# lukifer23/Matrix0

Measured on AMD Instinct MI355X. Metric: self-play games/sec at 800 sims/move, ResNet-24 53M; 1/2/4/8 MI355X, higher is better.
Workload: dtype f16

## Files before the change

include/m0_engine.h:

```cpp
#ifndef M0_ENGINE_H
#define M0_ENGINE_H

#include <stddef.h>
#include <stdint.h>

#ifdef __cplusplus
extern "C" {
#endif

#define M0_OK 0
#define M0_ERR_INVALID (-1)
#define M0_ERR_UNSUPPORTED (-2)
#define M0_ERR_HIP (-3)
#define M0_ERR_STATE (-4)
#define M0_ERR_NONFINITE (-5)

#define M0_POLICY_SIZE 4672
#define M0_PLANES 19

#define M0_ACT_RELU 1
#define M0_ACT_SILU 2
#define M0_ACT_LEAKY 3

#define M0_SSL_PIECE 1
// ... 203 lines not shown
#define M0_DECODE_FULLMOVE_SATURATED 2
#define M0_DECODE_EP_FROM_MASK 4
#define M0_DECODE_NO_MASK 8
int m0_decode_planes(int hip_device, const float* planes, const uint8_t* mask, int n, int32_t* status, int32_t* flags,
                     int32_t* nlegal, char* fens, int fen_stride);
int m0_analysis_submit_planes(m0_selfplay* sp, const float* planes, const uint8_t* mask, int n, int sims, const int64_t* ids,
                              int32_t* status, int32_t* flags);
int m0_analysis_keep_visits(m0_selfplay* sp, int on);
int m0_analysis_poll_visits(m0_selfplay* sp, m0_analysis_result* out, int32_t* nchild, int32_t* policy_idx, int32_t* visits,
                            int cap);

typedef struct m0_tb m0_tb;
m0_tb* m0_tb_build(int hip_device, int max_men);
m0_tb* m0_tb_build_signatures(int hip_device, const char* const* sigs, int n);
m0_tb* m0_tb_load(const char* path);
int m0_tb_save(const m0_tb* tb, const char* path);
void m0_tb_destroy(m0_tb* tb);
int m0_tb_max_men(const m0_tb* tb);
int m0_tb_table(const m0_tb* tb, const char* sig, const uint8_t** bytes, size_t* n);
int m0_tb_table_info(const m0_tb* tb, int i, char* sig8, int* maxd, int* sweeps, double* build_ms);
int m0_tb_probe_fens(const m0_tb* tb, const char* const* fens, int n, uint8_t* hit, int8_t* wdl, int16_t* dtm);
int m0_selfplay_set_tablebase(m0_selfplay* sp, const m0_tb* tb, int max_pieces);
uint64_t m0_selfplay_tb_adjudications(m0_selfplay* sp);
int m0_selfplay_set_search_tablebase(m0_selfplay* sp, const m0_tb* tb, int max_pieces);
uint64_t m0_selfplay_tb_leaves(m0_selfplay* sp);
int m0_tb_root_lines(const m0_tb* tb, const char* fen, int multipv, int pv_len, m0_analysis_result* out);

int m0_sample_move_index(const int32_t* visits, int n, double temperature, double u);
int m0_playout_cap(int sims, double frac, double u);
double m0_temperature_for(int fullmove_number, double t_start, double t_end, int t_moves);
int m0_rules_probe(const m0_selfplay_cfg* cfg, const char* fen, const char* const* ucis, int n, int* flags, float* result);

int m0_san_pattern(const char* token, uint32_t* pattern);
#define M0_MOVE_UCI 0
#define M0_MOVE_RAW 1
int m0_move_pattern(int kind, const char* uci, uint32_t raw, uint32_t* pattern);
#define M0_REPLAY_OK 0
#define M0_REPLAY_ILLEGAL 1
#define M0_REPLAY_AMBIGUOUS 2
#define M0_REPLAY_TOO_LONG 3
#define M0_REPLAY_END_CHECKMATE 1
#define M0_REPLAY_END_STALEMATE 2
#define M0_REPLAY_END_INSUFFICIENT 4
#define M0_REPLAY_END_WHITE_TO_MOVE 8
int m0_replay_games(int hip_device, const char* const* start_fens, const uint32_t* patterns, const int32_t* offsets, int n_games,
                    int max_plies, int max_positions_per_launch, int32_t* plies, int32_t* status, int32_t* end_flags,
                    uint16_t* moves, int32_t* policy_idx, int32_t* nlegal, int8_t* turn, float* planes, uint8_t* mask, float* ssl);

#ifdef __cplusplus
}
#endif
#include "m0_analysis_live.h"
#include "m0_score.h"
#endif
```

matrix0_amd/_abi.py:

```python
from __future__ import annotations

import ctypes as C
from ctypes import POINTER as P

M0_OK = 0
M0_ERR_INVALID = -1
M0_ERR_UNSUPPORTED = -2
M0_ERR_HIP = -3
M0_ERR_STATE = -4
M0_ERR_NONFINITE = -5
POLICY_SIZE = 4672
ACT = {"relu": 1, "silu": 2, "leaky_relu": 3}
SSL_BITS = {"piece": 1, "threat": 2, "pin": 4, "fork": 8, "control": 16}
AN_MAX_LINES, AN_MAX_PV = 8, 16
DECODE_STATUS = {0: "ok", 1: "piece_value", 2: "square_clash", 3: "kings", 4: "pawn_rank", 5: "not_uniform", 6: "flag_value",
                 7: "castling", 8: "counter", 9: "opponent_in_check", 10: "too_many_moves", 11: "mask_mismatch"}
DECODE_OK, DECODE_MASK_MISMATCH = 0, 11
HALFMOVE_SATURATED, FULLMOVE_SATURATED, EP_FROM_MASK, NO_MASK = 1, 2, 4, 8
REPLAY_STATUS = {0: "ok", 1: "illegal", 2: "ambiguous", 3: "too_long"}
REPLAY_END_BITS = {"checkmate": 1, "stalemate": 2, "insufficient": 4, "white_to_move": 8}
MOVE_UCI, MOVE_RAW = 0, 1
SCORE_MASK = {"legal": 0, "target": 1, "none": 2}
SCORE_COLS = 8
SCORE_COLUMNS = ("policy_loss", "entropy", "value_loss", "rank", "support_mass", "support_size", "value", "flags")
# ... 139 lines not shown
    "m0_search_advance": (i32, [vp, i32, i32, i32, i32]),
    "m0_analysis_create": (vp, [vp, _cfg, P(AnalysisOpts)]),
    "m0_analysis_create_ext": (vp, [_cfg, P(AnalysisOpts)]),
    "m0_analysis_submit": (i32, [vp, cstr, cstrs, i32, i32, i64]),
    "m0_analysis_step": (i32, [vp, i32]),
    "m0_analysis_ext_select": _select,
    "m0_analysis_ext_expand": _expand,
    "m0_analysis_poll": (i32, [vp, _res]),
    "m0_analysis_pending": (i32, [vp]),
    "m0_analysis_result_size": (C.c_size_t, []),
    "m0_decode_planes": (i32, [i32, vp, vp, i32, vp, vp, vp, cstr, i32]),
    "m0_analysis_submit_planes": (i32, [vp, vp, vp, i32, i32, vp, vp, vp]),
    "m0_analysis_keep_visits": (i32, [vp, i32]),
    "m0_analysis_poll_visits": (i32, [vp, _res, _pi32, vp, vp, i32]),
    "m0_tb_build": (vp, [i32, i32]),
    "m0_tb_build_signatures": (vp, [i32, cstrs, i32]),
    "m0_tb_load": (vp, [cstr]),
    "m0_tb_save": (i32, [vp, cstr]),
    "m0_tb_destroy": (None, [vp]),
    "m0_tb_max_men": (i32, [vp]),
    "m0_tb_table": (i32, [vp, cstr, P(P(u8)), P(C.c_size_t)]),
    "m0_tb_table_info": (i32, [vp, i32, cstr, _pi32, _pi32, P(f64)]),
    "m0_tb_probe_fens": (i32, [vp, cstrs, i32, vp, vp, vp]),
    "m0_selfplay_set_tablebase": _attach,
    "m0_selfplay_tb_adjudications": (u64, [vp]),
    "m0_selfplay_set_search_tablebase": _attach,
    "m0_selfplay_tb_leaves": (u64, [vp]),
    "m0_tb_root_lines": (i32, [vp, cstr, i32, i32, _res]),
    "m0_sample_move_index": (i32, [vp, i32, f64, f64]),
    "m0_playout_cap": (i32, [i32, f64, f64]),
    "m0_temperature_for": (f64, [i32, f64, f64, i32]),
    "m0_rules_probe": (i32, [_cfg, cstr, cstrs, i32, _pi32, P(f32)]),
    "m0_san_pattern": (i32, [cstr, P(u32)]),
    "m0_move_pattern": (i32, [i32, cstr, u32, P(u32)]),
    "m0_replay_games": (i32, [i32, cstrs, vp, vp, i32, i32, i32] + [vp] * 10),
}

LIVE_FUNCTIONS = {
    "m0_analysis_submit_keep": (i32, [vp, cstr, cstrs, i32, i32, i64]),
    "m0_analysis_peek": (i32, [vp, i64, _res]),
    "m0_analysis_stop": (i32, [vp, i64]),
    "m0_analysis_continue": (i32, [vp, i64, cstrs, i32, i32, i64, i32, _pi32]),
    "m0_analysis_release": (i32, [vp, i64]),
    "m0_analysis_held": (i32, [vp]),
}

SCORE_STRUCTS = {"m0_score_opts": ScoreOpts}
SCORE_FUNCTIONS = {
    "m0_score_rows": (i32, [i32, vp, vp, vp, vp, vp, i32, P(ScoreOpts), vp]),
    "m0_net_score": (i32, [vp, vp, vp, vp, vp, i32, P(ScoreOpts), vp]),
    "m0_score_bench": (i32, [i32, i32, i32, P(f32), P(f64)]),
}


def bind(L) -> list:
    missing = []
    for name, (restype, argtypes) in list(FUNCTIONS.items()) + list(LIVE_FUNCTIONS.items()) + list(SCORE_FUNCTIONS.items()):
        fn = getattr(L, name, None)
        if fn is None:
            missing.append(name)
        else:
            fn.restype, fn.argtypes = restype, argtypes
    return missing
```

matrix0_amd/backend.py:

```python
from __future__ import annotations

import ctypes as C
import threading
from typing import Dict, Optional, Tuple

import numpy as np

from . import _abi, _lib


def resolve_mask_mode(pi: np.ndarray, legal_mask, mask_mode: Optional[str]) -> str:
    if mask_mode is not None:
        if mask_mode not in _abi.SCORE_MASK:
            raise ValueError(f"mask_mode must be one of {sorted(_abi.SCORE_MASK)} or None, got {mask_mode!r}")
        return mask_mode
    if legal_mask is not None:
        return "legal"
    return "none" if bool(((np.asarray(pi) > 0).sum(axis=1) == 1).all()) else "target"


class NonFiniteScore(ValueError):

    def __init__(self, msg: str, rows: np.ndarray):
        super().__init__(msg)
        self.rows = rows


def score_opts(mask_mode: str, label_smoothing: float, value_loss: str, huber_delta: float) -> "_abi.ScoreOpts":
    if value_loss not in ("mse", "huber"):
        raise ValueError(f"value_loss must be 'mse' or 'huber', got {value_loss!r}")
    return _abi.ScoreOpts(_abi.SCORE_MASK[mask_mode], float(label_smoothing), int(value_loss == "huber"), float(huber_delta))


class M0Backend:
    def __init__(self, model_cfg: dict, device_index: int = 0):
        self._L = _lib.lib()
        self.model_cfg = dict(model_cfg)
        self._cfg = _lib.net_cfg_from_dict(model_cfg)
        self._h = self._L.m0_net_create(C.byref(self._cfg), int(device_index))
        if not self._h:
            raise RuntimeError(f"m0_net_create failed: {_lib.last_error()}")
        self._finalized = False
        self.ssl_tasks = [t for t in _lib.SSL_ORDER if self._cfg.ssl_tasks & _lib.SSL_BITS[t]] \
            if self._cfg.self_supervised else []

    def load_state_dict(self, sd: Dict[str, "np.ndarray"]) -> None:
        for k, v in sd.items():
            if hasattr(v, "detach"):
                v = v.detach().cpu().float().numpy()
            a = np.ascontiguousarray(np.asarray(v), dtype=np.float32)
            shape = (C.c_int64 * max(1, a.ndim))(*a.shape)
            _lib.check(self._L.m0_net_load_weight(self._h, k.encode(), _lib.ptr(a), 0, shape, a.ndim),
                       f"m0_net_load_weight({k})")
        _lib.check(self._L.m0_net_finalize(self._h), "m0_net_finalize")
        self._finalized = True

    @classmethod
    def from_state_dict(cls, model_cfg: dict, sd, device_index: int = 0) -> "M0Backend":
        b = cls(model_cfg, device_index)
        b.load_state_dict(sd)
        return b

    @classmethod
    def from_checkpoint(cls, model_cfg: dict, ckpt_path: str, device_index: int = 0) -> "M0Backend":
        import torch
        state = torch.load(ckpt_path, map_location="cpu", weights_only=False)
        sd = state
        if isinstance(state, dict):
            for key in ("model_ema", "model", "model_state_dict"):
                if key in state and isinstance(state[key], dict):
                    sd = state[key]
                    break
        return cls.from_state_dict(model_cfg, sd, device_index)

    def infer_np(self, arr: np.ndarray) -> Tuple[np.ndarray, np.ndarray]:
        p, v, _ = self._infer(arr, False)
        return p, v

    def infer_np_ssl(self, arr: np.ndarray):
        return self._infer(arr, True)

    def tap_info(self) -> Tuple[int, int]:
        steps, width = C.c_int(0), C.c_int(0)
        _lib.check(self._L.m0_net_tap_info(self._h, C.byref(steps), C.byref(width)), "m0_net_tap_info")
        return steps.value, width.value

    def infer_tap(self, arr: np.ndarray, step: int):
        return self._infer(arr, True, int(step))

    def _infer(self, arr: np.ndarray, want_ssl: bool, tap_step: Optional[int] = None):
        if not self._finalized:
            raise RuntimeError("weights not loaded")
        a = np.asarray(arr)
        if a.ndim == 3:
            a = a[None]
        if a.ndim != 4 or a.shape[1:] != (self._cfg.planes, 8, 8):
            raise ValueError(f"expected input [B,{self._cfg.planes},8,8], got {a.shape}")
        a = np.ascontiguousarray(a, dtype=np.float32)
        B = a.shape[0]
        pol = np.empty((B, _lib.POLICY_SIZE), dtype=np.float32)
        val = np.empty((B,), dtype=np.float32)
        sslc = self._L.m0_net_ssl_channels(self._h)
        ssl = np.empty((B, sslc, 8, 8), dtype=np.float32) if (want_ssl and sslc > 0) else None
        if tap_step is None:
            _lib.check(self._L.m0_net_infer(self._h, _lib.ptr(a), B, _lib.ptr(pol), _lib.ptr(val), _lib.ptr(ssl)), "m0_net_infer")
        else:
            width = self.tap_info()[1]
            stream = np.empty((B, 64, width), dtype=np.float32)
            second = np.empty((B, 64, width), dtype=np.float32)
            has_second = C.c_int(0)
            _lib.check(self._L.m0_net_infer_tap(self._h, _lib.ptr(a), B, tap_step, _lib.ptr(pol), _lib.ptr(val), _lib.ptr(ssl),
                                                _lib.ptr(stream), _lib.ptr(second), C.byref(has_second)), "m0_net_infer_tap")
        out = None
        if ssl is not None:
            out, off = {}, 0
            for t in self.ssl_tasks:
                n = _lib.SSL_CH[t]
                out[t] = ssl[:, off:off + n]
                off += n
        if tap_step is not None:
            return pol, val, out, stream, (second if has_second.value else None)
        return pol, val, out

    def score(self, s: np.ndarray, pi: np.ndarray, z: np.ndarray, legal_mask: Optional[np.ndarray] = None, *,
              mask_mode: Optional[str] = None, label_smoothing: float = 0.0, value_loss: str = "mse",
              huber_delta: float = 1.0) -> np.ndarray:
        if not self._finalized:
            raise RuntimeError("weights not loaded")
        a = np.ascontiguousarray(s, dtype=np.float32)
        if a.ndim != 4 or a.shape[1:] != (self._cfg.planes, 8, 8):
            raise ValueError(f"expected input [B,{self._cfg.planes},8,8], got {a.shape}")
        B = a.shape[0]
        pi = np.ascontiguousarray(pi, dtype=np.float32)
        z = np.ascontiguousarray(np.asarray(z).reshape(-1), dtype=np.float32)
        if pi.shape != (B, _lib.POLICY_SIZE) or z.shape != (B,):
            raise ValueError(f"expected pi [{B},{_lib.POLICY_SIZE}] and z [{B}], got {pi.shape} and {z.shape}")
        if legal_mask is not None:
            legal_mask = np.ascontiguousarray(np.asarray(legal_mask).reshape(B, -1), dtype=np.uint8)
            if legal_mask.shape != pi.shape:
                raise ValueError(f"expected legal_mask [{B},{_lib.POLICY_SIZE}], got {legal_mask.shape}")
        opts = score_opts(resolve_mask_mode(pi, legal_mask, mask_mode), label_smoothing, value_loss, huber_delta)
        rows = np.empty((B, _abi.SCORE_COLS), dtype=np.float32)
        rc = self._L.m0_net_score(self._h, _lib.ptr(a), _lib.ptr(pi), _lib.ptr(z), _lib.ptr(legal_mask), B, C.byref(opts),
                                  _lib.ptr(rows))
        if rc == _lib.M0_ERR_NONFINITE:
            raise NonFiniteScore(f"m0_net_score failed ({rc}): {_lib.last_error()}", rows)
        _lib.check(rc, "m0_net_score")
        return rows

    def param_count(self) -> int:
        return int(self._L.m0_net_param_count(self._h))

# ... 35 lines not shown
```

matrix0_amd/csrc/capi_analysis.hip:

```cpp
#include <string.h>
#include <algorithm>
#include <string>
#include <memory>
#include "selfplay_engine.h"
#include "planes_decode.h"
#include "tb.h"

using namespace m0;

namespace m0 {

static int searches_pending(const m0_selfplay* sp) {
    int n = (int)sp->an->queue.size();
    for (int s = 0; s < sp->G; ++s) n += sp->games[s].in_use && !sp->an->held[s] ? 1 : 0;
    return n;
}
static int pending_count(const m0_selfplay* sp) { return searches_pending(sp) + (int)sp->an->policy_queue.size(); }

static m0_analysis_result blank_result(const AnalysisJob& job) {
    m0_analysis_result r;
    memset(&r, 0, sizeof(r));
    r.id = job.id; r.nlegal = job.nlegal; r.sims = job.sims;
    return r;
}
// ... 54 lines not shown
    a.finished.clear();
    for (int s = 0; s < sp->G; ++s)
        if (sp->hg[s].active && sp->hg[s].finished) a.finished.push_back(s);
    const int nf = (int)a.finished.size();
    if (nf == 0) return M0_OK;
    HipStatus& hs = sp->hip;
    M0_HIP(hs, hipMemcpyAsync(sp->ids_dev, a.finished.data(), (size_t)nf * 4, hipMemcpyHostToDevice, sp->stream));
    M0_HIP(hs, launch_analysis_lines(sp->d, sp->ids_dev, nf, a.opts.multipv, a.opts.pv_len, a.lines_dev, a.nlines_dev, sp->stream));
    M0_HIP(hs, hipMemcpyAsync(a.hlines.data(), a.lines_dev, sizeof(m0_analysis_line) * M0_AN_MAX_LINES * nf, hipMemcpyDeviceToHost, sp->stream));
    M0_HIP(hs, hipMemcpyAsync(a.hnlines.data(), a.nlines_dev, (size_t)nf * 4, hipMemcpyDeviceToHost, sp->stream));
    if (a.keep_visits) {
        M0_HIP(hs, launch_root_children(sp->d, sp->ids_dev, nf, a.child_idx_dev, a.child_n_dev, a.nchild_dev, sp->stream));
        M0_HIP(hs, hipMemcpyAsync(a.hchild_idx.data(), a.child_idx_dev, (size_t)nf * M0_MAX_CHILDREN * 4, hipMemcpyDeviceToHost, sp->stream));
        M0_HIP(hs, hipMemcpyAsync(a.hchild_n.data(), a.child_n_dev, (size_t)nf * M0_MAX_CHILDREN * 4, hipMemcpyDeviceToHost, sp->stream));
        M0_HIP(hs, hipMemcpyAsync(a.hnchild.data(), a.nchild_dev, (size_t)nf * 4, hipMemcpyDeviceToHost, sp->stream));
    }
    if (!M0_HIP(hs, hipStreamSynchronize(sp->stream))) return m0_hip_error(hs, "analysis harvest failed");
    for (int j = 0; j < nf; ++j) {
        const int s = a.finished[j];
        GameDev& g = sp->hg[s];
        m0_analysis_result r = blank_result(a.slot_job[s]);
        r.overflow = g.overflow; r.root_n = g.root_n; r.evals = g.evals;
        r.value = (float)g.root_v;
        r.root_q = g.root_n > 0 ? g.root_q : g.root_v;
        copy_lines(a, j, r);
        if (g.overflow) sp->stats.arena_overflows++;
        std::vector<int32_t> children;
        if (a.keep_visits) {
            const int k = a.hnchild[j] < 0 ? 0 : (a.hnchild[j] > M0_MAX_CHILDREN ? M0_MAX_CHILDREN : a.hnchild[j]);
            const int32_t* ci = a.hchild_idx.data() + (size_t)j * M0_MAX_CHILDREN;
            const int32_t* cn = a.hchild_n.data() + (size_t)j * M0_MAX_CHILDREN;
            children.assign(ci, ci + k);
            children.insert(children.end(), cn, cn + k);
        }
        answer(a, r, std::move(children));
        g.active = 0; g.finished = 0;
        leave_slot(sp, s);
    }
    return sync_games_h2d(sp) ? M0_OK : m0_hip_error(hs, "releasing the slots failed");
}

static int policy_pass(m0_selfplay* sp) {
    Analysis& a = *sp->an;
    const int n = (int)std::min<size_t>(a.policy_queue.size(), (size_t)sp->rows_max);
    if (n <= 0) return M0_OK;
    const double t0 = now_ms();
    for (int i = 0; i < n; ++i) a.hpos[i] = a.policy_queue[i].line.pos;
    HipStatus& hs = sp->hip;
    M0_HIP(hs, hipMemcpyAsync(a.pos_dev, a.hpos.data(), sizeof(Pos) * n, hipMemcpyHostToDevice, sp->stream));
    if (!M0_HIP(hs, launch_encode_positions(a.pos_dev, n, nullptr, sp->d.x0, nullptr, a.nlegal_dev, a.moves_dev, a.idx_dev, sp->stream)))
        return m0_hip_error(hs, "position encode failed");
    std::string err;
    m0_net_lock(sp->nethandle);
    const int rc = sp->net->forward(nullptr, sp->d.x0, n, sp->logits_dev, sp->values_dev, nullptr, sp->stream, err);
    m0_net_unlock(sp->nethandle);
    if (rc != M0_OK) { hs.check(sp->net->hip()); m0_set_error(err); return rc; }
    M0_HIP(hs, launch_policy_lines(sp->logits_dev, sp->values_dev, a.nlegal_dev, a.moves_dev, a.idx_dev, n, a.opts.multipv, a.lines_dev,
                                   a.nlines_dev, a.value_out_dev, sp->stream));
    M0_HIP(hs, hipMemcpyAsync(a.hlines.data(), a.lines_dev, sizeof(m0_analysis_line) * M0_AN_MAX_LINES * n, hipMemcpyDeviceToHost, sp->stream));
    M0_HIP(hs, hipMemcpyAsync(a.hnlines.data(), a.nlines_dev, (size_t)n * 4, hipMemcpyDeviceToHost, sp->stream));
    M0_HIP(hs, hipMemcpyAsync(a.hvalues.data(), a.value_out_dev, (size_t)n * 4, hipMemcpyDeviceToHost, sp->stream));
    if (!M0_HIP(hs, hipStreamSynchronize(sp->stream))) return m0_hip_error(hs, "policy pass failed");
    for (int i = 0; i < n; ++i) {
        m0_analysis_result r = blank_result(a.policy_queue.front());
        r.evals = 1;
        r.value = a.hvalues[i];
        r.root_q = (double)r.value;
        copy_lines(a, i, r);
        answer(a, r);
        a.policy_queue.pop_front();
    }
    sp->stats.evals += (uint64_t)n;
    sp->stats.ms_total += now_ms() - t0;
    return M0_OK;
}

static bool blocked_by_held(const m0_selfplay* sp) {
    if (sp->an->queue.empty()) return false;
    for (int s = 0; s < sp->G; ++s) if (!sp->games[s].in_use || !sp->an->held[s]) return false;
    m0_set_error("searches are queued but every slot is held: m0_analysis_release or m0_analysis_continue one");
    return true;
}

static bool live_call_ok(const m0_selfplay* sp, const char* what) {
    if (!sp->ext_pending) return true;
    m0_set_error(std::string(what) + ": m0_analysis_ext_expand outstanding");
    return false;
}
static int slot_of(const m0_selfplay* sp, int64_t id, bool held) {
    for (int s = 0; s < sp->G; ++s)
        if (sp->games[s].in_use && (sp->an->held[s] != 0) == held && sp->an->slot_job[s].id == id) return s;
    return -1;
}
template <typename Q> static typename Q::iterator queued(Q& q, int64_t id) {
    return std::find_if(q.begin(), q.end(), [id](const AnalysisJob& j) { return j.id == id; });
}

static int live_result(m0_selfplay* sp, int s, m0_analysis_result& r) {
    Analysis& a = *sp->an;
    HipStatus& hs = sp->hip;
    M0_HIP(hs, hipMemcpyAsync(sp->ids_dev, &s, 4, hipMemcpyHostToDevice, sp->stream));
    M0_HIP(hs, launch_analysis_lines(sp->d, sp->ids_dev, 1, a.opts.multipv, a.opts.pv_len, a.lines_dev, a.nlines_dev, sp->stream));
    M0_HIP(hs, hipMemcpyAsync(a.hlines.data(), a.lines_dev, sizeof(m0_analysis_line) * M0_AN_MAX_LINES, hipMemcpyDeviceToHost, sp->stream));
    M0_HIP(hs, hipMemcpyAsync(a.hnlines.data(), a.nlines_dev, 4, hipMemcpyDeviceToHost, sp->stream));
    if (!sync_games_d2h(sp)) return m0_hip_error(hs, "reading a running search failed");
    const GameDev& g = sp->hg[s];
    r = blank_result(a.slot_job[s]);
// ... 309 lines not shown
```

matrix0_amd/csrc/capi_net.hip:

```cpp
#include <hip/hip_runtime.h>
#include <math.h>
#include <string.h>
#include <mutex>
#include <string>
#include <vector>
#include "../../include/m0_engine.h"
#include "net.h"
#include "capi_common.h"
#include "score_core.h"
#include "score_kernels.h"

thread_local std::string g_m0_last_error;

void m0_set_error(const std::string& s) { g_m0_last_error = s; }

struct m0_net {
    Net* net = nullptr;
    int device = 0;
    hipStream_t stream = nullptr;
    std::mutex mu;
    float* planes_dev = nullptr;
    float* logits_dev = nullptr;
    float* value_dev = nullptr;
    float* ssl_dev = nullptr;
    int cap = 0;
    float* score_pi_dev = nullptr;
    float* score_z_dev = nullptr;
    uint8_t* score_mask_dev = nullptr;
    float* score_rows_dev = nullptr;
    int score_cap = 0;
};

Net* m0_net_impl(m0_net* n) { return n ? n->net : nullptr; }
hipStream_t m0_net_stream(m0_net* n) { return n ? n->stream : nullptr; }
int m0_net_device(m0_net* n) { return n ? n->device : 0; }
void m0_net_lock(m0_net* n) { if (n) n->mu.lock(); }
void m0_net_unlock(m0_net* n) { if (n) n->mu.unlock(); }

hipError_t create_stream_cu_mask_env(const char* env_name, hipStream_t* stream) {
    const char* mk = getenv(env_name);
    if (!mk || !*mk) return hipStreamCreateWithFlags(stream, hipStreamNonBlocking);
    uint32_t words[8] = {0, 0, 0, 0, 0, 0, 0, 0};
    int nw = 0;
    for (const char* q = mk; *q && nw < 8; ++nw) {
        char* end = nullptr;
        words[nw] = (uint32_t)strtoul(q, &end, 16);
        if (end == q) break;
        q = (*end == ',') ? end + 1 : end;
    }
    return hipExtStreamCreateWithCUMask(stream, 8, words);
}

extern "C" {

const char* m0_last_error(void) { return g_m0_last_error.c_str(); }
const char* m0_version(void) { return "m0engine 0.2 (gfx950)"; }
int m0_device_count(void) {
    int n = 0;
    if (hipGetDeviceCount(&n) != hipSuccess) { (void)hipGetLastError(); return 0; }
    return n;
}

m0_net* m0_net_create(const m0_net_cfg* cfg, int hip_device) {
    if (!cfg) { m0_set_error("cfg is null"); return nullptr; }
    const char* why = Net::check_supported(*cfg);
    if (why) { m0_set_error(std::string("unsupported network config: ") + why); return nullptr; }
    int ndev = 0;
    if (hipGetDeviceCount(&ndev) != hipSuccess || ndev <= 0) {
        m0_set_error("no HIP device available (the engine has no CPU fallback)");
        return nullptr;
    }
    if (hip_device < 0 || hip_device >= ndev) { m0_set_error("hip_device out of range"); return nullptr; }
    if (hipSetDevice(hip_device) != hipSuccess) { m0_set_error("hipSetDevice failed"); return nullptr; }
    m0_net* h = new m0_net();
    h->device = hip_device;
    const hipError_t se = create_stream_cu_mask_env("M0_NET_CU_MASK", &h->stream);
    if (se != hipSuccess) {
        m0_set_error("hipStreamCreate failed");
        delete h;
        return nullptr;
    }
    h->net = new Net(*cfg, hip_device, h->stream);
    return h;
}

void m0_net_destroy(m0_net* n) {
    if (!n) return;
    (void)hipSetDevice(n->device);
    if (n->stream) { (void)hipStreamSynchronize(n->stream); }
    if (n->planes_dev) (void)hipFree(n->planes_dev);
    if (n->logits_dev) (void)hipFree(n->logits_dev);
    if (n->value_dev) (void)hipFree(n->value_dev);
    if (n->ssl_dev) (void)hipFree(n->ssl_dev);
    if (n->score_pi_dev) (void)hipFree(n->score_pi_dev);
    if (n->score_z_dev) (void)hipFree(n->score_z_dev);
    if (n->score_mask_dev) (void)hipFree(n->score_mask_dev);
    if (n->score_rows_dev) (void)hipFree(n->score_rows_dev);
    delete n->net;
    if (n->stream) (void)hipStreamDestroy(n->stream);
    delete n;
}

int m0_net_load_weight(m0_net* n, const char* name, const void* data, int dtype, const int64_t* shape, int ndim) {
    if (!n) { m0_set_error("net is null"); return M0_ERR_INVALID; }
    std::lock_guard<std::mutex> lk(n->mu);
    std::string err;
    int rc = n->net->load(name, data, dtype, shape, ndim, err);
    if (rc != M0_OK) m0_set_error(err);
    return rc;
}

int m0_net_finalize(m0_net* n) {
    if (!n) { m0_set_error("net is null"); return M0_ERR_INVALID; }
    std::lock_guard<std::mutex> lk(n->mu);
    if (!n->net->hip().ok()) return m0_hip_error(n->net->hip());
    std::string err;
    int rc = n->net->finalize(err);
    if (rc != M0_OK) m0_set_error(err);
    return rc;
}

static int ensure_io(m0_net* n, int B) {
    if (B <= n->cap) return M0_OK;
    HipStatus& hs = n->net->hip();
    for (float** p : {&n->planes_dev, &n->logits_dev, &n->value_dev, &n->ssl_dev}) {
        if (*p) M0_HIP(hs, hipFree(*p));
        *p = nullptr;
    }
    n->cap = 0;
    int cap = B < 64 ? 64 : B;
    const int P = n->net->cfg().planes;
    int sslc = n->net->ssl_channels_total();
    M0_HIP(hs, hipMalloc((void**)&n->planes_dev, (size_t)cap * P * 64 * 4));
    M0_HIP(hs, hipMalloc((void**)&n->logits_dev, (size_t)cap * M0_POLICY_SIZE * 4));
    M0_HIP(hs, hipMalloc((void**)&n->value_dev, (size_t)cap * 4));
    M0_HIP(hs, hipMalloc((void**)&n->ssl_dev, (size_t)cap * (sslc > 0 ? sslc : 1) * 64 * 4));
    if (!hs.ok()) return m0_hip_error(hs, "hipMalloc failed for I/O staging");
    n->cap = cap;
    return M0_OK;
}

static int ensure_score_io(m0_net* n, int B) {
    if (B <= n->score_cap) return M0_OK;
    HipStatus& hs = n->net->hip();
    if (n->score_pi_dev) M0_HIP(hs, hipFree(n->score_pi_dev));
    if (n->score_z_dev) M0_HIP(hs, hipFree(n->score_z_dev));
    if (n->score_mask_dev) M0_HIP(hs, hipFree(n->score_mask_dev));
    if (n->score_rows_dev) M0_HIP(hs, hipFree(n->score_rows_dev));
    n->score_pi_dev = n->score_z_dev = n->score_rows_dev = nullptr;
    n->score_mask_dev = nullptr;
    n->score_cap = 0;
    const int cap = B < 64 ? 64 : B;
    M0_HIP(hs, hipMalloc((void**)&n->score_pi_dev, (size_t)cap * M0_POLICY_SIZE * 4));
    M0_HIP(hs, hipMalloc((void**)&n->score_z_dev, (size_t)cap * 4));
    M0_HIP(hs, hipMalloc((void**)&n->score_mask_dev, (size_t)cap * M0_POLICY_SIZE));
    M0_HIP(hs, hipMalloc((void**)&n->score_rows_dev, (size_t)cap * M0_SCORE_COLS * 4));
    if (!hs.ok()) return m0_hip_error(hs, "hipMalloc failed for score staging");
    n->score_cap = cap;
    return M0_OK;
}

static int infer_locked(m0_net* n, const float* planes, int B, float* policy, float* value, float* ssl,
                        float* tap_stream = nullptr, float* tap_second = nullptr, int* has_second = nullptr) {
    HipStatus& hs = n->net->hip();
    if (!M0_HIP(hs, hipSetDevice(n->device))) return m0_hip_error(hs);
    int rc = ensure_io(n, B);
    if (rc != M0_OK) return rc;
    const int P = n->net->cfg().planes;
    const int sslc = n->net->ssl_channels_total();
    if (ssl && sslc == 0) { m0_set_error("ssl output requested but the net has no SSL heads"); return M0_ERR_INVALID; }
    std::string err;
    if (!M0_HIP(hs, hipMemcpyAsync(n->planes_dev, planes, (size_t)B * P * 64 * 4, hipMemcpyHostToDevice, n->stream)))
        return m0_hip_error(hs, "H2D copy");
    rc = n->net->forward(n->planes_dev, nullptr, B, n->logits_dev, n->value_dev, ssl ? n->ssl_dev : nullptr, n->stream, err);
    if (rc != M0_OK) { m0_set_error(err); return rc; }
    M0_HIP(hs, hipMemcpyAsync(policy, n->logits_dev, (size_t)B * M0_POLICY_SIZE * 4, hipMemcpyDeviceToHost, n->stream));
    M0_HIP(hs, hipMemcpyAsync(value, n->value_dev, (size_t)B * 4, hipMemcpyDeviceToHost, n->stream));
    if (ssl) M0_HIP(hs, hipMemcpyAsync(ssl, n->ssl_dev, (size_t)B * sslc * 64 * 4, hipMemcpyDeviceToHost, n->stream));
    std::vector<_Float16> th, ta;
    const size_t tn = tap_stream ? (size_t)B * 64 * n->net->trunk_width() : 0;
    if (tap_stream) {
        th.resize(tn);
        M0_HIP(hs, hipMemcpyAsync(th.data(), n->net->tap_stream(), tn * 2, hipMemcpyDeviceToHost, n->stream));
        if (n->net->tap_has_second()) {
            ta.resize(tn);
            M0_HIP(hs, hipMemcpyAsync(ta.data(), n->net->tap_second(), tn * 2, hipMemcpyDeviceToHost, n->stream));
        }
    }
    if (!M0_HIP(hs, hipStreamSynchronize(n->stream))) return m0_hip_error(hs, "forward failed");
    if (tap_stream) {
        for (size_t i = 0; i < tn; ++i) tap_stream[i] = (float)th[i];
        for (size_t i = 0; i < tn; ++i) tap_second[i] = ta.empty() ? 0.f : (float)ta[i];
        *has_second = ta.empty() ? 0 : 1;
    }
    for (size_t i = 0, nn = (size_t)B * M0_POLICY_SIZE; i < nn; ++i)
        if (!isfinite(policy[i])) { m0_set_error("network produced non-finite policy logits"); return M0_ERR_NONFINITE; }
    for (int i = 0; i < B; ++i)
        if (!isfinite(value[i])) { m0_set_error("network produced non-finite value"); return M0_ERR_NONFINITE; }
    return M0_OK;
}

int m0_net_infer(m0_net* n, const float* planes, int B, float* policy, float* value, float* ssl) {
    if (!n || !planes || !policy || !value) { m0_set_error("null argument"); return M0_ERR_INVALID; }
    if (B <= 0) { m0_set_error("batch must be positive"); return M0_ERR_INVALID; }
    std::lock_guard<std::mutex> lk(n->mu);
    return infer_locked(n, planes, B, policy, value, ssl);
}

int m0_net_score(m0_net* n, const float* planes, const float* pi, const float* z, const uint8_t* legal_mask, int B,
                 const m0_score_opts* opts, float* rows) {
    if (!n || !planes || !pi || !z || !rows) { m0_set_error("null argument"); return M0_ERR_INVALID; }
    if (B <= 0) { m0_set_error("batch must be positive"); return M0_ERR_INVALID; }
    if (const char* why = m0score::bad_opts(opts, legal_mask != nullptr)) { m0_set_error(why); return M0_ERR_INVALID; }
    std::lock_guard<std::mutex> lk(n->mu);
    HipStatus& hs = n->net->hip();
    if (!M0_HIP(hs, hipSetDevice(n->device))) return m0_hip_error(hs);
    int rc = ensure_io(n, B);
    if (rc == M0_OK) rc = ensure_score_io(n, B);
    if (rc != M0_OK) return rc;
    const bool masked = opts->mask_mode == M0_SCORE_MASK_LEGAL;
    const size_t cells = (size_t)B * M0_POLICY_SIZE;
    M0_HIP(hs, hipMemcpyAsync(n->planes_dev, planes, (size_t)B * n->net->cfg().planes * 64 * 4, hipMemcpyHostToDevice, n->stream));
    M0_HIP(hs, hipMemcpyAsync(n->score_pi_dev, pi, cells * 4, hipMemcpyHostToDevice, n->stream));
    M0_HIP(hs, hipMemcpyAsync(n->score_z_dev, z, (size_t)B * 4, hipMemcpyHostToDevice, n->stream));
    if (masked) M0_HIP(hs, hipMemcpyAsync(n->score_mask_dev, legal_mask, cells, hipMemcpyHostToDevice, n->stream));
    if (!hs.ok()) return m0_hip_error(hs, "H2D copy");
    std::string err;
    rc = n->net->forward(n->planes_dev, nullptr, B, n->logits_dev, n->value_dev, nullptr, n->stream, err);
    if (rc != M0_OK) { m0_set_error(err); return rc; }
    M0_HIP(hs, launch_score_rows(n->logits_dev, n->value_dev, n->score_pi_dev, n->score_z_dev, masked ? n->score_mask_dev : nullptr,
                                 B, *opts, n->score_rows_dev, n->stream));
    M0_HIP(hs, hipMemcpyAsync(rows, n->score_rows_dev, (size_t)B * M0_SCORE_COLS * 4, hipMemcpyDeviceToHost, n->stream));
    if (!M0_HIP(hs, hipStreamSynchronize(n->stream))) return m0_hip_error(hs, "forward and score failed");
    for (int b = 0; b < B; ++b)
        if ((int)rows[(size_t)b * M0_SCORE_COLS + 7] & M0_SCORE_FLAG_NONFINITE) {
            m0_set_error("network produced non-finite outputs (row " + std::to_string(b) + ")");
            return M0_ERR_NONFINITE;
        }
    return M0_OK;
}

int m0_net_tap_info(const m0_net* n, int* steps, int* width) {
    if (!n || !steps || !width) { m0_set_error("null argument"); return M0_ERR_INVALID; }
    *steps = n->net->tap_steps();
    *width = n->net->trunk_width();
    return M0_OK;
}

int m0_net_infer_tap(m0_net* n, const float* planes, int B, int step, float* policy, float* value, float* ssl, float* stream,
                     float* second, int* has_second) {
    if (!n || !planes || !policy || !value || !stream || !second || !has_second) {
        m0_set_error("null argument");
        return M0_ERR_INVALID;
    }
    if (B <= 0) { m0_set_error("batch must be positive"); return M0_ERR_INVALID; }
    if (step < 0 || step >= n->net->tap_steps()) { m0_set_error("tap step out of range"); return M0_ERR_INVALID; }
    std::lock_guard<std::mutex> lk(n->mu);
    n->net->set_tap(step);
    const int rc = infer_locked(n, planes, B, policy, value, ssl, stream, second, has_second);
    n->net->set_tap(-1);
    return rc;
}

int m0_net_ssl_channels(const m0_net* n) { return n ? n->net->ssl_channels_total() : 0; }
int64_t m0_net_param_count(const m0_net* n) { return n ? (int64_t)n->net->param_count() : 0; }
double m0_net_flops_per_position(const m0_net* n, int with_ssl) { return n ? n->net->flops_per_position(with_ssl != 0) : 0.0; }

int m0_net_profile_enable(m0_net* n, int on) {
    if (!n) { m0_set_error("net is null"); return M0_ERR_INVALID; }
    std::lock_guard<std::mutex> lk(n->mu);
    n->net->set_profile(on != 0);
    return M0_OK;
}

int m0_net_profile_get(m0_net* n, double* conv_ms, double* conv_flop, int64_t* launches, int reset) {
    if (!n) { m0_set_error("net is null"); return M0_ERR_INVALID; }
    std::lock_guard<std::mutex> lk(n->mu);
    if (conv_ms) *conv_ms = n->net->prof_conv_ms();
    if (conv_flop) *conv_flop = n->net->prof_conv_flop();
    if (launches) *launches = n->net->prof_conv_launches();
    if (reset) n->net->reset_profile();
    return M0_OK;
}

int m0_net_profile_get_tail(m0_net* n, double* tail_ms, int64_t* tail_launches) {
    if (!n) { m0_set_error("net is null"); return M0_ERR_INVALID; }
    std::lock_guard<std::mutex> lk(n->mu);
    if (tail_ms) *tail_ms = n->net->prof_tail_ms();
    if (tail_launches) *tail_launches = n->net->prof_tail_launches();
    return M0_OK;
}

int m0_net_bench_forward(m0_net* n, int B, int iters, int with_ssl, float* ms_per_forward) {
    if (!n || !ms_per_forward || B <= 0 || iters <= 0) { m0_set_error("invalid argument"); return M0_ERR_INVALID; }
    std::lock_guard<std::mutex> lk(n->mu);
    HipStatus& hs = n->net->hip();
    if (!M0_HIP(hs, hipSetDevice(n->device))) return m0_hip_error(hs);
    int rc = ensure_io(n, B);
    if (rc != M0_OK) return rc;
    std::string err;
    if (!(with_ssl & 2)) {
        const int P = n->net->cfg().planes;
        std::vector<float> h((size_t)B * P * 64, 0.f);
        uint64_t s = 0x9E3779B97F4A7C15ull;
        for (size_t i = 0; i < h.size(); ++i) {
            s ^= s << 13; s ^= s >> 7; s ^= s << 17;
            int p = (int)((i / 64) % P);
            if (p < 12) h[i] = ((s >> 20) % 100) < 8 ? 1.f : 0.f;
            else h[i] = (float)((((i / 64 / P) * 7 + p) % 10) / 10.0);
        }
        if (!M0_HIP(hs, hipMemcpy(n->planes_dev, h.data(), h.size() * 4, hipMemcpyHostToDevice))) return m0_hip_error(hs, "H2D copy");
    }
    float* ssl = ((with_ssl & 1) && n->net->ssl_channels_total() > 0) ? n->ssl_dev : nullptr;
    rc = n->net->forward(n->planes_dev, nullptr, B, n->logits_dev, n->value_dev, ssl, n->stream, err);
    if (rc != M0_OK) { m0_set_error(err); return rc; }
    struct Events {
        hipEvent_t e0 = nullptr, e1 = nullptr;
        ~Events() { if (e0) (void)hipEventDestroy(e0); if (e1) (void)hipEventDestroy(e1); }
    } ev;
    M0_HIP(hs, hipEventCreate(&ev.e0)); M0_HIP(hs, hipEventCreate(&ev.e1));
    M0_HIP(hs, hipEventRecord(ev.e0, n->stream));
    for (int i = 0; i < iters && hs.ok(); ++i) {
        rc = n->net->forward(n->planes_dev, nullptr, B, n->logits_dev, n->value_dev, ssl, n->stream, err);
        if (rc != M0_OK) { m0_set_error(err); return rc; }
    }
    M0_HIP(hs, hipEventRecord(ev.e1, n->stream));
    M0_HIP(hs, hipEventSynchronize(ev.e1));
    float ms = 0.f;
    if (!M0_HIP(hs, hipEventElapsedTime(&ms, ev.e0, ev.e1))) return m0_hip_error(hs, "bench forward failed");
    *ms_per_forward = ms / iters;
    n->net->harvest_profile();
    return M0_OK;
}

}
```

matrix0_amd/csrc/capi_selfplay.hip:

```cpp
#include <string.h>
#include <algorithm>
#include <memory>
#include "selfplay_engine.h"

using namespace m0;

static void fill_tree_cfg(const m0_selfplay_cfg& c, bool match, TreeCfg& t) {
    t.fpu_reduction = c.fpu_reduction; t.draw_penalty = c.draw_penalty; t.virtual_loss = c.virtual_loss;
    t.selection_jitter = c.selection_jitter; t.cpuct = c.cpuct; t.cpuct_start = c.cpuct_start; t.cpuct_end = c.cpuct_end;
    t.cpuct_plies = c.cpuct_plies; t.use_c_base = c.use_c_base; t.cpuct_c_base = c.cpuct_c_base; t.cpuct_c_init = c.cpuct_c_init;
    t.dirichlet_alpha = c.dirichlet_alpha; t.dirichlet_frac = c.dirichlet_frac; t.legal_softmax = c.legal_softmax;
    t.enable_entropy_noise = c.enable_entropy_noise; t.no_instant_backtrack = c.no_instant_backtrack;
    t.virtual_loss_active = c.virtual_loss_active; t.leaves_per_step = c.inference_batch_size;
    t.tt_merge = c.tt_merge; t.raw_legal_priors = c.raw_legal_priors; t.max_children = c.max_children;
    t.min_child_prior = c.min_child_prior;
    t.eval_cache = ((match ? c.arena_eval_cache : c.eval_cache) && c.legal_softmax && !c.raw_legal_priors && !c.tt_merge) ? 1 : 0;
}

static bool alloc_tree_arenas(m0_selfplay* sp) {
    const m0_selfplay_cfg& c = sp->cfg;
    long want = c.arena_nodes > 0 ? c.arena_nodes : (long)(c.num_simulations * 1.3 + 64) * 96;
    if (want < 4096) want = 4096;
    sp->cap = (int)want;
    const size_t N = (size_t)sp->G * 2 * sp->cap;
    TreeArrays& t = sp->d.t;
    t.cap = sp->cap;
    t.prior = dalloc<double>(sp, N); t.w = dalloc<double>(sp, N); t.q = dalloc<double>(sp, N);
    t.n = dalloc<int>(sp, N); t.vl = dalloc<int>(sp, N); t.cbase = dalloc<int>(sp, N);
    t.nch = dalloc<int16_t>(sp, N); t.mv = dalloc<uint16_t>(sp, N); t.midx = dalloc<uint16_t>(sp, N);
    sp->d.games = dalloc<GameDev>(sp, sp->G);
    const size_t LS = (size_t)sp->L + 1;
    sp->d.samples = dalloc<Sample>(sp, (size_t)sp->G * LS);
    sp->d.paths = dalloc<int>(sp, (size_t)sp->G * LS * M0_MAX_DEPTH);
    sp->d.leaf_moves = dalloc<uint16_t>(sp, (size_t)sp->G * LS * M0_MAX_CHILDREN);
    return hip_ok(sp, "hipMalloc failed for the search arenas (lower concurrent_games or arena_nodes)");
}

static bool alloc_position_tables(m0_selfplay* sp) {
    sp->d.tt_sides = 1;
    if (!sp->cfg.tt_merge) return true;
    const size_t LS = (size_t)sp->L + 1;
    int tc = 1024;
    while (tc < 2 * sp->cap) tc <<= 1;
    sp->d.tt_cap = tc;
    sp->d.tt_sides = sp->kind == EngineKind::Match ? 2 : 1;
    sp->d.search_nodes = (int)std::min<long>((long)sp->cfg.num_simulations * 48 + 4 * M0_MAX_CHILDREN, (long)sp->cap / 2);
    sp->d.epaths = dalloc<int>(sp, (size_t)sp->G * LS * M0_MAX_DEPTH);
    sp->d.tt_keys = dalloc<uint64_t>(sp, (size_t)sp->G * sp->d.tt_sides * tc);
    sp->d.tt_nodes = dalloc<int>(sp, (size_t)sp->G * sp->d.tt_sides * tc);
    return hip_ok(sp, "hipMalloc failed for the position tables (tt_merge): lower concurrent_games or arena_nodes");
}

static bool alloc_eval_cache(m0_selfplay* sp) {
    if (!sp->tc.eval_cache) return true;
    const size_t LS = (size_t)sp->L + 1;
    int entries = sp->cfg.eval_cache_entries > 0 ? sp->cfg.eval_cache_entries : 16384;
    int sets = 64;
    while (sets * 4 < entries) sets <<= 1;
    EvalCache& ec = sp->d.ec;
    ec.sets = sets;
    ec.sides = sp->kind == EngineKind::Match ? 2 : 1;
    const size_t entries_all = (size_t)sp->G * ec.sides * sets * 4;
    ec.keys = dalloc<uint64_t>(sp, entries_all);
    ec.stamps = dalloc<uint32_t>(sp, entries_all);
    ec.payload = dalloc<float>(sp, entries_all * M0_EC_WORDS);
    ec.hit_stage = dalloc<float>(sp, (size_t)sp->G * LS * M0_EC_WORDS);
    return hip_ok(sp, "hipMalloc failed for the evaluation cache: lower eval_cache_entries or concurrent_games");
}

static bool alloc_batch_buffers(m0_selfplay* sp) {
    const int nreg = sp->kind == EngineKind::Match ? 2 : 1;
    sp->d.hist = dalloc<uint64_t>(sp, (size_t)sp->G * M0_HIST_CAP);
    sp->d.results = dalloc<RootResult>(sp, sp->G);
    sp->d.row_counter = dalloc<int>(sp, 4);
    sp->d.x0 = dalloc<_Float16>(sp, (size_t)(nreg * sp->rows_max + 4) * 64 * 32);
    sp->logits_dev = dalloc<float>(sp, (size_t)nreg * sp->rows_max * 4672);
    sp->values_dev = dalloc<float>(sp, (size_t)nreg * sp->rows_max + 4);
    sp->d.net_row_base = sp->rows_max;
    if (sp->cfg.ssl_in_forward && sp->net && sp->net->ssl_channels_total() > 0)
        sp->ssl_dev = dalloc<float>(sp, (size_t)sp->rows_max * sp->net->ssl_channels_total() * 64);
    if (sp->cfg.ssl_targets) {
        sp->ssl_cap = sp->cfg.max_game_len > 0 ? sp->cfg.max_game_len + 1 : 513;
        sp->ssl_pos_dev = dalloc<Pos>(sp, sp->ssl_cap);
        sp->ssl_out_dev = dalloc<float>(sp, (size_t)sp->ssl_cap * 17 * 64);
        if (!hip_ok(sp, "hipMalloc failed for the SSL target staging buffers")) return false;
    }
    sp->ids_dev = dalloc<int>(sp, sp->G);
    sp->roots_dev = dalloc<int>(sp, sp->G);
    sp->d.logits = sp->logits_dev; sp->d.values = sp->values_dev;
    sp->d.G = sp->G; sp->d.L = sp->L;
    return hip_ok(sp, "hipMalloc failed for the batch buffers (lower concurrent_games or inference_batch_size)");
}

static bool make_tail_view(m0_selfplay* sp) {
    if (!(sp->cfg.tail_split && sp->net && sp->kind != EngineKind::Match && sp->net->cfg().channels > 256 && sp->net->cfg().channels <= 320 &&
          sp->rows_max >= 2048)) return true;
    M0_HIP(sp->hip, create_stream_cu_mask_env("M0_TAIL_CU_MASK", &sp->stream_tail));
    M0_HIP(sp->hip, hipEventCreateWithFlags(&sp->ev_sel, hipEventDisableTiming));
    M0_HIP(sp->hip, hipEventCreateWithFlags(&sp->ev_tail, hipEventDisableTiming));
    if (!hip_ok(sp, "hipStreamCreate / hipEventCreate failed (tail split)")) return false;
    sp->net_tail = sp->net->shared_view(sp->stream_tail);
    std::string werr;
    sp->half_split = sp->cfg.tail_split == 2;
    if (sp->net_tail->ensure_workspace(sp->half_split ? sp->rows_max / 2 + 1024 : 1023, werr) != M0_OK) {
        m0_set_error("tail split: " + werr);
        return false;
    }
    return true;
}

static bool build_engine(m0_selfplay* sp) {
    if (!alloc_tree_arenas(sp) || !alloc_position_tables(sp) || !alloc_eval_cache(sp) || !alloc_batch_buffers(sp)) return false;
    sp->hg.assign(sp->G, GameDev());
    for (auto& g : sp->hg) memset(&g, 0, sizeof(GameDev));
    sp->games.assign(sp->G, HostGame());
    sp->hres.resize(sp->G);
    sp->hsamples.resize((size_t)sp->G * (sp->L + 1));
    sp->prev_done.assign(sp->G, 0);
    for (hipEvent_t* e : {&sp->ev0, &sp->ev1, &sp->ev2, &sp->ev3}) M0_HIP(sp->hip, hipEventCreate(e));
    if (!hip_ok(sp, "hipEventCreate failed") || !make_tail_view(sp)) return false;
    std::string err;
    if (sp->net && sp->net->ensure_workspace(sp->rows_max, err) != M0_OK) { m0_set_error(err); return false; }
    if (sp->net && sp->net_b && sp->net_b->ensure_workspace(sp->rows_max, err) != M0_OK) { m0_set_error(err); return false; }
    M0_HIP(sp->hip, hipStreamSynchronize(sp->stream));
    return hip_ok(sp, "clearing the search arenas failed");
}

m0_selfplay* m0::engine_create(m0_net* nh, m0_net* nh_b, const m0_selfplay_cfg* cfg, EngineKind kind) {
    if (!cfg) { m0_set_error("cfg is null"); return nullptr; }
    if (cfg->concurrent_games <= 0 || cfg->inference_batch_size <= 0 || cfg->num_simulations <= 0) {
// ... 31 lines not shown
static int leaf_planes(m0_selfplay* sp, int rows_a, float* planes_a, int rows_b, float* planes_b) {
    sync_games_d2h(sp);
    if (!M0_HIP(sp->hip, hipMemcpy(sp->hsamples.data(), sp->d.samples, sizeof(Sample) * (size_t)sp->G * (sp->L + 1), hipMemcpyDeviceToHost)))
        return m0_hip_error(sp->hip, "device sync failed");
    const int base = sp->d.net_row_base;
    for (int g = 0; g < sp->G; ++g) {
        if (!sp->hg[g].active) continue;
        for (int s = 0; s < sp->hg[g].nsamples; ++s) {
            const Sample& smp = sp->hsamples[(size_t)g * (sp->L + 1) + s];
            if (!sample_owns_row(smp.kind) || smp.row < 0) continue;
            if (smp.row < rows_a) encode_planes_f32(smp.pos, planes_a + (size_t)smp.row * 19 * 64);
            else if (smp.row >= base && smp.row < base + rows_b) encode_planes_f32(smp.pos, planes_b + (size_t)(smp.row - base) * 19 * 64);
        }
    }
    return M0_OK;
}

static void upload_eval(m0_selfplay* sp, size_t row_base, const float* logits, const float* values, int rows) {
    if (rows <= 0) return;
    M0_HIP(sp->hip, hipMemcpyAsync(sp->logits_dev + row_base * 4672, logits, (size_t)rows * 4672 * 4, hipMemcpyHostToDevice, sp->stream));
    M0_HIP(sp->hip, hipMemcpyAsync(sp->values_dev + row_base, values, (size_t)rows * 4, hipMemcpyHostToDevice, sp->stream));
}

int m0::ext_select_impl(m0_selfplay* sp, int* rows_a, int* rows_b, float* planes_a, float* planes_b, int max_rows) {
    if (sp->ext_pending) { m0_set_error("m0_selfplay_ext_expand outstanding"); return M0_ERR_STATE; }
    if (!planes_a || (sp->kind == EngineKind::Match && !planes_b) || max_rows < sp->G * (sp->L + 1)) {
        m0_set_error("planes buffer too small: concurrent_games * (inference_batch_size + 1) rows are required");
        return M0_ERR_INVALID;
    }
    int rc = refill(sp);
    if (rc != M0_OK) return rc;
    int r = 0;
    if ((rc = run_select(sp, &r)) != M0_OK) return rc;
    const int rb = sp->kind == EngineKind::Match ? sp->rows2[1] : 0;
    if (r > sp->rows_max || rb > sp->rows_max) { m0_set_error("row counter overflow"); return M0_ERR_STATE; }
    *rows_a = r;
    if (rows_b) *rows_b = rb;
    sp->last_rows = r;
    sp->last_rows_b = rb;
    sp->ext_pending = true;
    if (r + rb > 0) return leaf_planes(sp, r, planes_a, rb, planes_b);
    return M0_OK;
}

int m0::ext_expand_impl(m0_selfplay* sp, const float* logits_a, const float* values_a, int rows_a, const float* logits_b,
                           const float* values_b, int rows_b) {
    if (!sp->ext_pending) { m0_set_error("no m0_selfplay_ext_select outstanding"); return M0_ERR_STATE; }
    if (rows_a != sp->last_rows || rows_b != sp->last_rows_b) { m0_set_error("rows does not match the last select"); return M0_ERR_INVALID; }
    if ((rows_a > 0 && (!logits_a || !values_a)) || (rows_b > 0 && (!logits_b || !values_b))) { m0_set_error("null argument"); return M0_ERR_INVALID; }
    upload_eval(sp, 0, logits_a, values_a, rows_a);
    upload_eval(sp, (size_t)sp->d.net_row_base, logits_b, values_b, rows_b);
    sp->ext_pending = false;
    M0_HIP(sp->hip, hipEventRecord(sp->ev0, sp->stream)); M0_HIP(sp->hip, hipEventRecord(sp->ev1, sp->stream));
    return finish_step(sp, rows_a + rows_b, now_ms());
}

bool m0::kind_accepted(const m0_selfplay* sp, const char* what, unsigned kinds) {
    if (kinds & (1u << (int)sp->kind)) return true;
    static const char* const is_a[] = {"a self-play engine", "a match engine", "an analysis engine"};
    const char* only = kinds == KIND_SELFPLAY ? "self-play engines" : kinds == KIND_MATCH ? "match engines"
                     : kinds == KIND_ANALYSIS ? "analysis engines" : "self-play and match engines";
    m0_set_error(std::string(what) + ": " + only + " only, this is " + is_a[(int)sp->kind]);
    return false;
}

extern "C" {

m0_selfplay* m0_selfplay_create(m0_net* nh, const m0_selfplay_cfg* cfg) { return engine_create(nh, nullptr, cfg, EngineKind::SelfPlay); }

m0_selfplay* m0_arena_create(m0_net* net_a, m0_net* net_b, const m0_selfplay_cfg* cfg) {
    if (!net_a || !net_b) { m0_set_error("m0_arena_create needs two networks"); return nullptr; }
    if (m0_net_device(net_a) != m0_net_device(net_b)) { m0_set_error("both networks must live on the same HIP device"); return nullptr; }
    if (cfg && (cfg->ssl_in_forward || cfg->ssl_targets)) { m0_set_error("arena games carry no SSL outputs"); return nullptr; }
    return engine_create(net_a, net_b, cfg, EngineKind::Match);
}

m0_selfplay* m0_arena_create_ext(const m0_selfplay_cfg* cfg) {
    if (cfg && (cfg->ssl_in_forward || cfg->ssl_targets)) { m0_set_error("arena games carry no SSL outputs"); return nullptr; }
    return engine_create(nullptr, nullptr, cfg, EngineKind::Match);
}

void m0_selfplay_destroy(m0_selfplay* sp) {
    if (!sp) return;
    forward_gate_leave(sp);
    (void)hipSetDevice(sp->device);
    if (sp->stream) (void)hipStreamSynchronize(sp->stream);
    if (sp->stream_tail) (void)hipStreamSynchronize(sp->stream_tail);
    delete sp->net_tail;
    if (sp->ev_sel) (void)hipEventDestroy(sp->ev_sel);
    if (sp->ev_tail) (void)hipEventDestroy(sp->ev_tail);
    if (sp->stream_tail) (void)hipStreamDestroy(sp->stream_tail);
    for (void* p : sp->allocs) (void)hipFree(p);
    for (auto& r : sp->done_meta) delete (GameRecordOwner*)r.owner;
    delete sp->an;
    if (sp->ev0) { (void)hipEventDestroy(sp->ev0); (void)hipEventDestroy(sp->ev1); (void)hipEventDestroy(sp->ev2); (void)hipEventDestroy(sp->ev3); }
    if (sp->own_stream && sp->stream) (void)hipStreamDestroy(sp->stream);
    delete sp;
}

int m0_selfplay_set_openings(m0_selfplay* sp, const char* const* fens, int n) {
    if (!sp || n < 0 || (n > 0 && !fens)) { m0_set_error("invalid argument"); return M0_ERR_INVALID; }
    M0_ENGINE_CALL(sp, "m0_selfplay_set_openings", KIND_GAMES, false);
    if (sp->stats.games_started != 0) { m0_set_error("set the opening book before the first step"); return M0_ERR_STATE; }
    std::vector<Pos> book(n);
    for (int i = 0; i < n; ++i)
        if (!fens[i] || parse_fen(fens[i], book[i]) != 0) { m0_set_error(std::string("bad FEN at index ") + std::to_string(i)); return M0_ERR_INVALID; }
    sp->book.swap(book);
// ... 154 lines not shown
```

matrix0_amd/csrc/conv_epilogue.h:

```cpp
#pragma once
#include "kernel_common.h"

typedef _Float16 half2v __attribute__((ext_vector_type(2)));

template <int ACT>
__device__ __forceinline__ float act_fast(float v) {
    if constexpr (ACT == ACT_RELU) return v > 0.f ? v : 0.f;
    else if constexpr (ACT == ACT_SILU) return v * __builtin_amdgcn_rcpf(1.f + __expf(-v));
    else if constexpr (ACT == ACT_LEAKY) return v > 0.f ? v : 0.05f * v;
    else if constexpr (ACT == ACT_SIGMOID) return __builtin_amdgcn_rcpf(1.f + __expf(-v));
    else if constexpr (ACT == ACT_TANH) return tanhf(v);
    else return v;
}
template <int NT>
__device__ __forceinline__ char* conv_stage_base(char* lds_wave, int lane) {
    return lds_wave + (4 * (lane >> 5) + (lane & 1)) * (NT * 64) + ((lane & 31) >> 1) * 4;
}

template <int NT, int MI, int NI>
__device__ __forceinline__ void conv_stage_tile(const float (&v)[16], char* wbase, int lane) {
    constexpr int ROWB = NT * 64;
    const bool odd = (lane & 1) != 0;
    static_for<0, 8>([&](auto rp_) __attribute__((always_inline)) {
        constexpr int r0 = 2 * decltype(rp_)::value;
// ... 2 lines not shown
        const float recv = __builtin_bit_cast(
            float, __builtin_amdgcn_update_dpp(0, __builtin_bit_cast(int, send), 0xB1, 0xF, 0xF, true));
        const half2v h = {(_Float16)(odd ? recv : v0), (_Float16)(odd ? v1 : recv)};
        *reinterpret_cast<half2v*>(wbase + (MI * 32 + (r0 & 3) + 8 * (r0 >> 2)) * ROWB + NI * 64) = h;
    });
}

template <int NT, int FENCE_EVERY = 0>
__device__ __forceinline__ void conv_stage_flush(const GemmArgs& a, const char* lds_wave, int m0, int n0, int wm, int wn,
                                                 int lane) {
    constexpr int NCH = NT * 4;
    const uint32_t ldo2 = (uint32_t)a.ldo * 2u;
    char* out = reinterpret_cast<char*>(a.out) + ((size_t)(m0 + wm * 64) * a.ldo + n0 + wn * NT * 32) * 2;
    const int rows_valid = a.Mvalid - (m0 + wm * 64);
    int row = lane / NCH, ch = lane - row * NCH;
#pragma unroll
    for (int it = 0; it < NCH; ++it) {
        if (FENCE_EVERY > 0 && it % (FENCE_EVERY > 0 ? FENCE_EVERY : 1) == 0) asm volatile("" ::: "memory");
        const uint4 v = *reinterpret_cast<const uint4*>(lds_wave + (it * 64 + lane) * 16);
        if (row < rows_valid) *reinterpret_cast<uint4*>(out + ((uint32_t)row * ldo2 + (uint32_t)ch * 16u)) = v;
        ch += 64 % NCH; row += 64 / NCH;
        if (ch >= NCH) { ch -= NCH; row += 1; }
    }
}

__device__ __forceinline__ void gn16_mean_rstd(float s, float ss, float& mean, float& rstd) {
    mean = s * (1.f / 1024.f);
    float var = ss * (1.f / 1024.f) - mean * mean;
    var = var > 0.f ? var : 0.f;
    rstd = rsqrtf(var + 1e-5f);
}
__device__ __forceinline__ void gn16_affine(float mean, float rstd, const float& gamma, const float& beta, float& scale,
                                            float& shift) {
    scale = gamma * rstd;
    shift = beta - mean * scale;
}

template <int NI, int NT>
__device__ __forceinline__ void conv_gn_column(const float16v (&acc)[2][NT], const float* gamma, const float* beta, int col,
                                               float& scale, float& shift) {
    float s = 0.f, ss = 0.f;
    static_for<0, 2>([&](auto mi_) __attribute__((always_inline)) {
        const float16v av = acc[decltype(mi_)::value][NI];
        static_for<0, 16>([&](auto r_) __attribute__((always_inline)) { const float v = av[decltype(r_)::value]; s += v; ss += v * v; });
    });
#pragma unroll
    for (int o = 1; o <= 8; o <<= 1) { s += __shfl_xor(s, o); ss += __shfl_xor(ss, o); }
    s += __shfl_xor(s, 32); ss += __shfl_xor(ss, 32);
    float mean, rstd;
    gn16_mean_rstd(s, ss, mean, rstd);
    gn16_affine(mean, rstd, gamma[col], beta[col], scale, shift);
}

template <ConvEpi EPI, int ACT, int NT>
__device__ __forceinline__ void conv_tile_epilogue(float16v (&acc)[2][NT], const GemmArgs& a, char* lds_wave, int m0,
                                                   int n0, int wm, int wn, int lane, int out_col0 = 0) {
    const int half = lane >> 5;
    const int r31 = lane & 31;
    const int colbase = n0 + wn * NT * 32 + r31;
    char* wbase = conv_stage_base<NT>(lds_wave, lane);
    if constexpr (EPI == EPI_GN) {
        static_for<0, NT>([&](auto ni_) __attribute__((always_inline)) {
            constexpr int ni = decltype(ni_)::value;
            const int col = colbase + ni * 32;
            float g, sh;
            conv_gn_column<ni>(acc, a.gn_gamma, a.gn_beta, col, g, sh);
            static_for<0, 2>([&](auto mi_) __attribute__((always_inline)) {
                constexpr int mi = decltype(mi_)::value;
                float v[16];
                static_for<0, 16>([&](auto r_) __attribute__((always_inline)) {
                    constexpr int r = decltype(r_)::value;
                    v[r] = act_fast<ACT>(acc[mi][ni][r] * g + sh);
                });
                if (a.posenc != nullptr) {
                    static_for<0, 16>([&](auto r_) __attribute__((always_inline)) {
                        constexpr int r = decltype(r_)::value;
                        const int sq = mi * 32 + (r & 3) + 8 * (r >> 2) + 4 * half;
                        v[r] += a.posenc[(size_t)sq * a.N + col];
                    });
                }
                conv_stage_tile<NT, mi, ni>(v, wbase, lane);
            });
        });
        conv_stage_flush<NT>(a, lds_wave, m0, n0 - out_col0, wm, wn, lane);
    }
    if constexpr (EPI == EPI_PLAIN) {
        const float oscale = a.out_scale;
        const bool want_stats = a.out_stats != nullptr;
        float* stats = a.out_stats + ((size_t)(m0 / 64 + wm) * a.N + colbase) * 2;
        static_for<0, NT>([&](auto ni_) __attribute__((always_inline)) {
            constexpr int ni = decltype(ni_)::value;
            const float bias = a.bias != nullptr ? a.bias[colbase + ni * 32] : 0.f;
            float s = 0.f, ss = 0.f;
            static_for<0, 2>([&](auto mi_) __attribute__((always_inline)) {
                constexpr int mi = decltype(mi_)::value;
                float v[16];
                static_for<0, 16>([&](auto r_) __attribute__((always_inline)) {
                    constexpr int r = decltype(r_)::value;
                    v[r] = act_fast<ACT>(acc[mi][ni][r] + bias) * oscale;
                    s += v[r]; ss += v[r] * v[r];
                });
                conv_stage_tile<NT, mi, ni>(v, wbase, lane);
            });
            if (want_stats) {
                s += __shfl_xor(s, 32);
                ss += __shfl_xor(ss, 32);
                if (lane < 32) { stats[ni * 64] = s; stats[ni * 64 + 1] = ss; }
            }
        });
        conv_stage_flush<NT>(a, lds_wave, m0, n0, wm, wn, lane);
    }
    if constexpr (EPI == EPI_ELEMENT) {
        const int ldo = a.ldo;
        const int rowbase = m0 + wm * 64 + 4 * half;
        const int epi_act = a.epi_act;
        const float oscale = a.out_scale;
        const bool want_stats = a.out_stats != nullptr;
        const bool has_mul = a.mul != nullptr;
        const bool f32out = a.out_f32 != 0;
        static_for<0, NT>([&](auto ni_) __attribute__((always_inline)) {
            constexpr int ni = decltype(ni_)::value;
            const int col = colbase + ni * 32;
            const float bias = a.bias != nullptr ? a.bias[col] : 0.f;
            float s = 0.f, ss = 0.f;
            static_for<0, 2>([&](auto mi_) __attribute__((always_inline)) {
                constexpr int mi = decltype(mi_)::value;
                const float16v av = acc[mi][ni];
                static_for<0, 16>([&](auto r_) __attribute__((always_inline)) {
                    constexpr int r = decltype(r_)::value;
                    const int row = rowbase + mi * 32 + (r & 3) + 8 * (r >> 2);
                    float v = av[r] + bias;
                    if (epi_act != ACT_NONE) v = act_apply(v, epi_act);
                    if (has_mul) v *= (float)a.mul[(size_t)row * ldo + col];
                    v *= oscale;
                    s += v; ss += v * v;
                    if (row < a.Mvalid) {
                        if (f32out) reinterpret_cast<float*>(a.out)[(size_t)row * ldo + col] = v;
                        else reinterpret_cast<_Float16*>(a.out)[(size_t)row * ldo + col] = (_Float16)v;
                    }
                });
            });
            if (want_stats) {
                s += __shfl_xor(s, 32);
                ss += __shfl_xor(ss, 32);
                if (lane < 32) {
                    float* st = a.out_stats + ((size_t)(m0 / 64 + wm) * a.N + col) * 2;
                    st[0] = s; st[1] = ss;
                }
            }
        });
    }
}
```

matrix0_amd/csrc/conv_gemm.hip:

```cpp
#include "kernel_common.h"
#include "conv_epilogue.h"

template <int TAPS, int WN, int NT, int KC, ConvEpi EPI = EPI_ELEMENT, int ACT = ACT_NONE>
__global__ __launch_bounds__(256 * WN) void conv_gemm_kernel(GemmArgs a) {
    constexpr int NB = WN * NT * 32;
    constexpr int NTHR = 256 * WN;
    constexpr int AST = KC + 8;
    constexpr int APIX = (TAPS == 9) ? 100 : 64;
    constexpr int A_ELEMS = 4 * APIX * AST;
    constexpr int W_ELEMS = NB * AST;
    constexpr int A_PIECES = 4 * 64 * KC / 8;
    constexpr int W_PIECES = NB * KC / 8;
    constexpr int A_PER = (A_PIECES + NTHR - 1) / NTHR;
    constexpr int W_PER = (W_PIECES + NTHR - 1) / NTHR;
    constexpr int K8 = KC / 8;

    extern __shared__ __attribute__((aligned(16))) char smem[];
    _Float16* A_lds = reinterpret_cast<_Float16*>(smem);
    _Float16* W_lds = A_lds + A_ELEMS;

    const int tid = threadIdx.x;
    const int lane = tid & 63;
    const int wave = tid >> 6;
    const int wm = wave % 4;
    const int wn = wave / 4;
    const int m0 = blockIdx.x * 256;
    const int n0 = blockIdx.y * NB;
    const int Cin = a.Cin;
    const int nchunk = Cin / KC;
    const int Npad = a.Npad;

    if (TAPS == 9) {
        for (int i = tid; i < A_ELEMS / 8; i += NTHR)
            reinterpret_cast<uint4*>(A_lds)[i] = make_uint4(0, 0, 0, 0);
    }
    __syncthreads();

    float16v acc[2][NT];
    static_for<0, 2>([&](auto mi) __attribute__((always_inline)) {
        static_for<0, NT>([&](auto ni) __attribute__((always_inline)) {
            acc[decltype(mi)::value][decltype(ni)::value] = float16v{0.f, 0.f, 0.f, 0.f, 0.f, 0.f, 0.f, 0.f,
                                                                      0.f, 0.f, 0.f, 0.f, 0.f, 0.f, 0.f, 0.f};
        });
    });

    int apix[2];
#pragma unroll
    for (int mi = 0; mi < 2; ++mi) {
        int px = mi * 32 + (lane & 31);
        if (TAPS == 9) apix[mi] = wm * 100 + ((px >> 3) + 1) * 10 + (px & 7) + 1;
        else apix[mi] = wm * 64 + px;
    }
    const int khalf = 8 * (lane >> 5);

    uint4 areg[A_PER];
    uint4 wreg[W_PER];
// ... 29 lines not shown
            int p = tid + i * NTHR;
            if (W_PIECES % NTHR == 0 || p < W_PIECES)
                wreg[i] = *reinterpret_cast<const uint4*>(src + (size_t)p * 8);
        }
    };
    auto store_W = [&](int buf) {
#pragma unroll
        for (int i = 0; i < W_PER; ++i) {
            int p = tid + i * NTHR;
            if (W_PIECES % NTHR == 0 || p < W_PIECES) {
                int n = p / K8, k8 = p % K8;
                *reinterpret_cast<uint4*>(W_lds + buf * W_ELEMS + n * AST + k8 * 8) = wreg[i];
            }
        }
    };

    const int nsteps = nchunk * TAPS;
    load_A(0);
    load_W(0);
    for (int s = 0; s < nsteps; ++s) {
        const int chunk = s / TAPS, tap = s % TAPS;
        if (tap == 0) {
            if (s > 0) __syncthreads();
            store_A(chunk);
        }
        store_W(s & 1);
        __syncthreads();
        if (s + 1 < nsteps) {
            load_W(s + 1);
            if ((s + 1) % TAPS == 0) load_A((s + 1) / TAPS);
        }
        const int tapoff = (TAPS == 9) ? ((tap / 3 - 1) * 10 + (tap % 3 - 1)) : 0;
        const _Float16* Wb = W_lds + (s & 1) * W_ELEMS + (wn * NT * 32 + (lane & 31)) * AST + khalf;
        static_for<0, KC / 16>([&](auto kk_) __attribute__((always_inline)) {
            constexpr int kk = decltype(kk_)::value;
            half8 af0 = *reinterpret_cast<const half8*>(A_lds + (apix[0] + tapoff) * AST + kk * 16 + khalf);
            half8 af1 = *reinterpret_cast<const half8*>(A_lds + (apix[1] + tapoff) * AST + kk * 16 + khalf);
            static_for<0, NT>([&](auto ni_) __attribute__((always_inline)) {
                constexpr int ni = decltype(ni_)::value;
                half8 bf = *reinterpret_cast<const half8*>(Wb + ni * 32 * AST + kk * 16);
                acc[0][ni] = __builtin_amdgcn_mfma_f32_32x32x16_f16(af0, bf, acc[0][ni], 0, 0, 0);
                acc[1][ni] = __builtin_amdgcn_mfma_f32_32x32x16_f16(af1, bf, acc[1][ni], 0, 0, 0);
            });
        });
    }

    if constexpr (EPI == EPI_GN) {
        __syncthreads();
        GemmArgs o = a;
        int out_col0 = 0;
        if (a.out2 != nullptr && n0 + wn * NT * 32 >= a.nsplit) { o.out = a.out2; o.ldo = a.ldo2; out_col0 = a.nsplit; }
        conv_tile_epilogue<EPI_GN, ACT, NT>(acc, o, smem + wave * (64 * 64 * NT), m0, n0, wm, wn, lane, out_col0);
    } else {
        conv_tile_epilogue<EPI_ELEMENT, ACT_NONE, NT>(acc, a, smem, m0, n0, wm, wn, lane);
    }
}

template <int TAPS, int WN, int NT, int KC>
static size_t conv_gemm_lds() {
    constexpr int NB = WN * NT * 32;
    constexpr int AST = KC + 8;
    constexpr int APIX = (TAPS == 9) ? 100 : 64;
    const size_t main_loop = (size_t)(4 * APIX * AST + 2 * NB * AST) * 2 + 64;
    const size_t staging = (size_t)WN * 4 * 64 * 64 * NT;
    return main_loop > staging ? main_loop : staging;
}

template <int TAPS, int WN, int NT, int KC, ConvEpi EPI = EPI_ELEMENT, int ACT = ACT_NONE>
static hipError_t launch_conv_gemm_t(const GemmArgs& a, hipStream_t st) {
    constexpr int NB = WN * NT * 32;
    size_t lds = conv_gemm_lds<TAPS, WN, NT, KC>();
    static DeviceOnce once;
    hipError_t e = once.run([] {
        return hipFuncSetAttribute(reinterpret_cast<const void*>(&conv_gemm_kernel<TAPS, WN, NT, KC, EPI, ACT>),
                                   hipFuncAttributeMaxDynamicSharedMemorySize, 160 * 1024);
    });
    if (e != hipSuccess) return e;
    dim3 grid(a.Mrows / 256, a.Npad / NB);
    hipLaunchKernelGGL((conv_gemm_kernel<TAPS, WN, NT, KC, EPI, ACT>), grid, dim3(256 * WN), lds, st, a);
    return hipGetLastError();
}
template <int ACT>
static hipError_t launch_conv_gemm_gn(const GemmArgs& a, int taps, hipStream_t st) {
    if (a.bias != nullptr || a.mul != nullptr || a.out_stats != nullptr || a.out_f32 || a.out_scale != 1.f || a.Npad != a.N)
        return hipErrorInvalidValue;
    if (taps == 9) return a.Npad % 64 == 0 && a.out2 == nullptr ? launch_conv_gemm_t<9, 1, 2, 32, EPI_GN, ACT>(a, st) : hipErrorInvalidValue;
    if (a.posenc != nullptr) return hipErrorInvalidValue;
    if (a.out2 != nullptr) return a.Npad == 192 && a.nsplit == 64 ? launch_conv_gemm_t<1, 3, 2, 32, EPI_GN, ACT>(a, st) : hipErrorInvalidValue;
    if (a.Npad == 160) return launch_conv_gemm_t<1, 1, 5, 32, EPI_GN, ACT>(a, st);
    if (a.Npad == 128) return launch_conv_gemm_t<1, 2, 2, 32, EPI_GN, ACT>(a, st);
    if (a.Npad == 64) return launch_conv_gemm_t<1, 1, 2, 32, EPI_GN, ACT>(a, st);
    if (a.Npad == 32) return launch_conv_gemm_t<1, 1, 1, 32, EPI_GN, ACT>(a, st);
    return hipErrorInvalidValue;
}

hipError_t launch_conv_big(const GemmArgs& a, int taps, hipStream_t st);
hipError_t launch_conv_zs(const GemmArgs& a, hipStream_t st);

int conv_gemm_tile_n(int Cin, int Npad) {
    return (Npad % 320 == 0 && Cin % 64 == 0) ? 320 : 32;
}
int conv_gemm_kc(int Cin, int Npad) {
    return (Npad % 320 == 0 && Cin % 64 == 0) ? 64 : 32;
}

hipError_t launch_conv_gemm(const GemmArgs& a, int taps, hipStream_t st) {
    if (a.Mrows % 256 != 0 || a.Cin % 32 != 0 || a.Npad % 32 != 0) return hipErrorInvalidValue;
    const bool big = conv_gemm_tile_n(a.Cin, a.Npad) == 320;
    if (a.gn_gamma != nullptr && !big) {
        if (a.epi_act == ACT_SILU) return launch_conv_gemm_gn<ACT_SILU>(a, taps, st);
        if (a.epi_act == ACT_RELU) return launch_conv_gemm_gn<ACT_RELU>(a, taps, st);
        return hipErrorInvalidValue;
    }
    if (taps == 9) {
        if (big) {
            if (!a.w_pp) return hipErrorInvalidValue;
            return launch_conv_zs(a, st);
        }
        return launch_conv_gemm_t<9, 1, 1, 32>(a, st);
    } else if (taps == 1) {
        if (big) return a.w_pp ? hipErrorInvalidValue : launch_conv_big(a, 1, st);
        if (a.Mrows / 256 >= 256 && a.Npad % 64 == 0) return launch_conv_gemm_t<1, 1, 2, 32>(a, st);
        return launch_conv_gemm_t<1, 1, 1, 32>(a, st);
    }
    return hipErrorInvalidValue;
}
```

matrix0_amd/csrc/net.h:

```cpp
#pragma once
#include <hip/hip_runtime.h>
#include <stdint.h>
#include <map>
#include <string>
#include <vector>
#include "../../include/m0_engine.h"
#include "hip_check.h"
#include "net_kernels.h"

namespace net_pack { struct GemmShape; }

inline int ceil_to(int v, int m) { return (v + m - 1) / m * m; }

struct HostTensor {
    std::vector<float> data;
    std::vector<int64_t> shape;
};

struct PackedGemm {
    _Float16* w = nullptr;
    float* bias = nullptr;
    int taps = 1, Cin = 0, N = 0;
    bool pp = false;
};
// ... 4 lines not shown
};

struct HostNorm { std::vector<float> gamma, beta; };

struct ResBlockW {
    PackedGemm conv1, conv2;
    NormParams bn1, bn2;
    float *se_w1 = nullptr, *se_b1 = nullptr, *se_w2 = nullptr, *se_b2 = nullptr;
    void* se_wf = nullptr;
    int se_hidden = 0;
};

struct AttnW {
    PackedGemm qkv, proj;
    NormParams ln;
    float* rel_bias = nullptr;
    void* blk_w = nullptr;
    _Float16* blk_bias = nullptr;
};

struct TowerLayer {
    int kind;
    int index;
    bool skip;
    int next_bn1 = -1;
};

struct SslHeadW {
    PackedGemm c0, c1;
    NormParams n;
    int out_ch = 0;
};

struct ConvNormOpts {
    const float* posenc = nullptr;
    const _Float16* res = nullptr;
    const NormParams* next_bn1 = nullptr;
};

class Net {
public:
    explicit Net(const m0_net_cfg& cfg, int device, hipStream_t stream);
    ~Net();
    Net* shared_view(hipStream_t stream) const;
    static const char* check_supported(const m0_net_cfg& cfg);
    int load(const char* name, const void* data, int dtype, const int64_t* shape, int ndim, std::string& err);
    int finalize(std::string& err);
    bool ready() const { return finalized_; }
    HipStatus& hip() { return *hip_; }
    const std::vector<void*>& device_buffers() const { return dev_allocs_; }
    const std::vector<size_t>& device_buffer_bytes() const { return dev_sizes_; }

    int forward(const float* planes_dev, const _Float16* nhwc_dev, int B, float* logits_dev, float* value_dev,
                float* ssl_dev, hipStream_t st, std::string& err);
    int ensure_workspace(int B, std::string& err);
    int ssl_channels_total() const;
    const m0_net_cfg& cfg() const { return cfg_; }
    size_t param_count() const { return nparams_; }
    double flops_per_position(bool with_ssl) const;
    _Float16* input_nhwc() { return X0_; }
    int tap_steps() const { return 3 + (int)tower_.size(); }
    int trunk_width() const { return Cp_; }
    void set_tap(int step) { tap_step_ = step; }
    const _Float16* tap_stream() const { return TAPX_; }
    const _Float16* tap_second() const { return TAPA_; }
    bool tap_has_second() const { return tap_second_; }
    void set_profile(bool on) { profile_ = on; }
    void harvest_profile();
    double prof_conv_ms() const { return prof_ms_; }
    double prof_conv_flop() const { return prof_flop_; }
    long prof_conv_launches() const { return prof_launches_; }
    void reset_profile() { prof_ms_ = 0; prof_flop_ = 0; prof_launches_ = 0; prof_tail_ms_ = 0; prof_tail_launches_ = 0; }
    double prof_tail_ms() const { return prof_tail_ms_; }
    long prof_tail_launches() const { return prof_tail_launches_; }

private:
    m0_net_cfg cfg_;
    int device_;
    hipStream_t stream_ = nullptr;
    HipStatus own_hip_, *hip_ = &own_hip_;
    struct Switches { bool fuse_tail = true, fuse_attn = true; int attn_grid = 0; } sw_;
    struct Plan {
        bool fuse_tail = false;
        bool fuse_attn = false;
        bool gn_small = false;
        int act = 0, vact = 0;
        int first_bn1 = -1;
    } plan_;
    bool finalized_ = false;
    size_t nparams_ = 0;
    std::map<std::string, HostTensor> sd_;
    std::vector<void*> dev_allocs_;
    std::vector<size_t> dev_sizes_;
    std::vector<void*> ws_allocs_;

    int C_ = 0, Cs_ = 0 ;
    int Cp_ = 0;
    PackedGemm stem_;
    NormParams stem_n_;
    float* posenc_ = nullptr;
    PackedGemm pst_, inter_;
    NormParams pst_n_, inter_n_;
    std::vector<ResBlockW> res_;
    std::vector<AttnW> att_;
    std::vector<TowerLayer> tower_;
    PackedGemm ph_conv_, pfc1_, pfc2_;
    PackedGemm hv_;
    NormParams hv_n_;
    NormParams ph_n_;
    float logit_scale_ = 1.f;
    PackedGemm vh0_, vh3_, vfc1_, vfc2_, vgate_, vfc3_;
    NormParams vh1_n_, vh4_n_;
    std::vector<SslHeadW> ssl_;
    uint64_t* mask_dev_ = nullptr;

    bool profile_ = false;
    std::vector<hipEvent_t> pev_;
    std::vector<double> pflop_;
    std::vector<char> ptail_;
    size_t pev_used_ = 0;
    double prof_ms_ = 0, prof_flop_ = 0, prof_tail_ms_ = 0;
    long prof_launches_ = 0, prof_tail_launches_ = 0;

    int wsB_ = 0, wsM_ = 0;
    _Float16 *X0_ = nullptr, *XA_ = nullptr, *XB_ = nullptr, *T1_ = nullptr, *T2_ = nullptr, *QKV_ = nullptr,
             *O_ = nullptr, *AA_ = nullptr;
    float *S1_ = nullptr, *S2_ = nullptr, *G_ = nullptr;
    _Float16 *PH_ = nullptr, *PH2_ = nullptr, *VH_ = nullptr, *VH2_ = nullptr, *F1_ = nullptr, *F2_ = nullptr,
             *F3_ = nullptr, *F4_ = nullptr, *SH_ = nullptr, *SH2_ = nullptr, *SO_ = nullptr;
    float* VAL_ = nullptr;
    float* SPK_ = nullptr;
    int tap_step_ = -1;
    bool tap_second_ = false;
    _Float16 *TAPX_ = nullptr, *TAPA_ = nullptr;
// ... 26 lines not shown
```

matrix0_amd/csrc/net.hip:

```cpp
#include "net.h"
#include <math.h>
#include <string.h>
#include <algorithm>
#include <stdlib.h>

const char* Net::check_supported(const m0_net_cfg& c) {
    if (!c.norm_group) return "HIP path supports norm='group' only (BatchNorm configs are not built)";
    if (!c.preact) return "HIP path supports preact=true only";
    if (c.channels % 32 != 0 || c.channels < 32 || c.channels > 384) return "channels must be a multiple of 32 in [32,384]";
    if (c.planes < 1 || c.planes > 32) return "planes must be in [1,32]";
    if (c.attention && (c.attention_heads <= 0 || c.channels % c.attention_heads != 0 ||
                        c.channels / c.attention_heads != 16))
        return "attention head_dim (channels/attention_heads) must be 16";
    if (c.activation != M0_ACT_SILU && c.activation != M0_ACT_RELU) return "activation must be silu or relu";
    if (c.blocks < 1) return "blocks must be >= 1";
    if (c.policy_factor_rank < 0) return "policy_factor_rank must be >= 0";
    if (c.self_supervised && c.ssl_tasks && (c.channels / 2) % 16 != 0) return "ssl heads need channels/2 % 16 == 0";
    return nullptr;
}

Net::Net(const m0_net_cfg& cfg, int device, hipStream_t stream) : cfg_(cfg), device_(device), stream_(stream) {
    auto off = [](const char* name) { const char* e = getenv(name); return e && e[0] == '0'; };
    sw_.fuse_tail = !off("M0_FUSE_TAIL");
    sw_.fuse_attn = !off("M0_FUSE_ATTN");
    if (const char* e = getenv("M0_ATTN_GRID")) sw_.attn_grid = std::max(0, atoi(e));
    C_ = cfg.channels;
    Cp_ = (C_ > 256 && C_ < 320) ? 320 : C_;
    Cs_ = ceil_to(std::max(16, C_ / 2), 32);
    int k = cfg.attention_every_k;
    int stride = std::max(1, cfg.infer_attention_stride);
    int att_seen = 0;
    for (int i = 0; i < cfg.blocks; ++i) {
        tower_.push_back({0, (int)res_.size(), false});
        res_.emplace_back();
        if (cfg.attention && k > 0 && (i % k) == (k - 1)) {
            ++att_seen;
            bool skip = stride > 1 && (att_seen % stride) != 0;
            tower_.push_back({1, (int)att_.size(), skip});
            att_.emplace_back();
        }
    }
}

Net* Net::shared_view(hipStream_t stream) const {
    Net* v = new Net(*this);
    v->stream_ = stream;
    v->dev_allocs_.clear(); v->dev_sizes_.clear();
    v->ws_allocs_.clear(); v->wsB_ = 0; v->wsM_ = 0;
    v->tap_step_ = -1; v->TAPX_ = v->TAPA_ = nullptr;
    v->sd_.clear();
    v->pev_.clear(); v->pflop_.clear(); v->ptail_.clear(); v->pev_used_ = 0; v->profile_ = false;
    v->prof_ms_ = v->prof_flop_ = v->prof_tail_ms_ = 0; v->prof_launches_ = v->prof_tail_launches_ = 0;
    return v;
}

Net::~Net() {
    for (hipEvent_t e : pev_) (void)hipEventDestroy(e);
    for (void* p : dev_allocs_) (void)hipFree(p);
    for (void* p : ws_allocs_) (void)hipFree(p);
}

void* Net::dalloc(size_t bytes, bool ws) {
    void* p = nullptr;
    if (bytes == 0) bytes = 16;
    if (!M0_HIP(*hip_, hipMalloc(&p, bytes))) return nullptr;
    (ws ? ws_allocs_ : dev_allocs_).push_back(p);
    if (!ws) dev_sizes_.push_back(bytes);
    M0_HIP(*hip_, hipMemsetAsync(p, 0, bytes, stream_));
    if (!ws) M0_HIP(*hip_, hipStreamSynchronize(stream_));
    return hip_->ok() ? p : nullptr;
}

int Net::ssl_channels_total() const {
    int n = 0;
    for (auto& h : ssl_) n += h.out_ch;
    return n;
}
// ... 78 lines not shown

static double conv3x3_flop(const PackedGemm& g, int rows) { return 2.0 * (double)rows * (double)g.N * (double)g.Cin * 9.0; }

template <class Launch>
hipError_t Net::profiled(bool on, hipStream_t st, double flop, bool tail, Launch&& launch) {
    if (!on) return launch();
    if (pev_used_ + 2 > pev_.size()) {
        for (int i = 0; i < 2; ++i) { hipEvent_t e; if (!M0_HIP(*hip_, hipEventCreate(&e))) return hip_->code(); pev_.push_back(e); }
    }
    M0_HIP(*hip_, hipEventRecord(pev_[pev_used_], st));
    hipError_t rc = hip_->ok() ? launch() : hip_->code();
    if (rc == hipSuccess && !M0_HIP(*hip_, hipEventRecord(pev_[pev_used_ + 1], st))) rc = hip_->code();
    pev_used_ += 2;
    pflop_.push_back(flop);
    ptail_.push_back(tail ? 1 : 0);
    return rc;
}

hipError_t Net::run_gemm(const PackedGemm& g, GemmArgs a, hipStream_t st) {
    const bool big = conv_gemm_tile_n(g.Cin, g.N) == 320;
    const bool splitk = g.taps == 1 && big && g.Cin >= 4096 && (g.Cin >> 6) % 8 == 0 && !a.gn_gamma && !a.mul && !a.out_stats &&
                        !a.out_f32 && a.out_scale == 1.f && SPK_ != nullptr && (size_t)g.N <= (size_t)ceil_to(2 * C_, 32) &&
                        a.Mrows <= wsM_;
    return profiled(profile_ && g.taps == 9 && big, st, conv3x3_flop(g, a.Mvalid), false, [&]() -> hipError_t {
        if (!splitk) return launch_conv_gemm(a, g.taps, st);
        _Float16* out = (_Float16*)a.out;
        const int act = a.epi_act;
        a.out = SPK_; a.bias = nullptr; a.epi_act = ACT_NONE; a.out_f32 = 1; a.ksplit = 8;
        hipError_t rc = launch_conv_gemm(a, g.taps, st);
        return rc != hipSuccess ? rc : launch_splitk_reduce(SPK_, 8, a.Mrows, g.N, g.bias, act, out, st);
    });
}

hipError_t Net::se_gate(const ResBlockW& r, const float* stats, int boards, hipStream_t st) {
    SeGateArgs g;
    g.t_stats = stats; g.w1 = r.se_w1; g.b1 = r.se_b1; g.w2 = r.se_w2; g.b2 = r.se_b2;
    g.gate = G_; g.B = boards; g.C = Cp_; g.hidden = r.se_hidden; g.act = plan_.act;
    return launch_se_gate(g, st);
}

hipError_t Net::conv_norm_act(const PackedGemm& g, const NormParams& n, const _Float16* in, _Float16* out, _Float16* scratch,
                              int Mrows, hipStream_t st, const ConvNormOpts& o) {
    const bool big = conv_gemm_tile_n(g.Cin, g.N) == 320;
    GemmArgs a = gemm_args(g, in, out, Mrows);
    if (big && o.res && plan_.fuse_tail) {
        a.epi_act = plan_.act; a.res = o.res; a.pre_gamma = n.gamma; a.pre_beta = n.beta;
        if (o.next_bn1) { a.y2 = AA_; a.gn_gamma = o.next_bn1->gamma; a.gn_beta = o.next_bn1->beta; }
        return launch_conv_gemm(a, g.taps, st);
    }
    const bool epilogue = big ? g.taps == 9
                              : plan_.gn_small && (g.taps == 9 ? g.Cin == 32 : g.N == 32 || g.N == 64 || g.N == 128 || g.N == 160);
    if (epilogue && !o.res && !o.next_bn1) {
        a.gn_gamma = n.gamma; a.gn_beta = n.beta; a.epi_act = plan_.act; a.posenc = o.posenc;
        return run_gemm(g, a, st);
    }
    a.out = scratch; a.out_stats = S1_;
    hipError_t rc = run_gemm(g, a, st);
    if (rc != hipSuccess) return rc;
    EwArgs e = ew_args(scratch, out, g.N, plan_.act);
    e.t_stats = S1_; e.gn_gamma = n.gamma; e.gn_beta = n.beta; e.res = o.res; e.posenc = o.posenc;
    ew_next_bn1(e, o.next_bn1, AA_);
    return launch_ew_board(e, Mrows / 64, st);
}

void Net::harvest_profile() {
    for (size_t i = 0; i + 1 < pev_used_; i += 2) {
        float ms = 0.f;
        if (hipEventElapsedTime(&ms, pev_[i], pev_[i + 1]) == hipSuccess) {
            prof_ms_ += ms; prof_flop_ += pflop_[i / 2]; prof_launches_++;
            if (ptail_[i / 2]) { prof_tail_ms_ += ms; prof_tail_launches_++; }
        }
    }
    pev_used_ = 0;
    pflop_.clear();
    ptail_.clear();
}

int Net::forward(const float* planes_dev, const _Float16* nhwc_dev, int B, float* logits_dev, float* value_dev,
                 float* ssl_dev, hipStream_t st, std::string& err) {
    if (!finalized_) { err = "weights not finalized"; return M0_ERR_STATE; }
    if (B <= 0) { err = "batch must be positive"; return M0_ERR_INVALID; }
    if (int rc = ensure_workspace(B, err)) return rc;
    HipStatus& hs = *hip_;
    const int Bp = ceil_to(B, 4);
    const int Mc = Bp * 64;
    const int Mfc = ceil_to(B, 256);
    const int act = plan_.act, vact = plan_.vact;
    const int C = Cp_;

    const _Float16* x0 = nhwc_dev;
    if (!x0) {
        if (!planes_dev) { err = "no input"; return M0_ERR_INVALID; }
        M0_HIP(hs, launch_planes_to_nhwc(planes_dev, X0_, B, cfg_.planes, st));
        x0 = X0_;
    }
    _Float16* xa = XA_;
    _Float16* xb = XB_;
    const NormParams* first_bn1 = bn1(plan_.first_bn1);
    auto tap = [&](int step, const _Float16* stream, bool second) {
        if (step != tap_step_) return;
        const size_t bytes = (size_t)Mc * C * sizeof(_Float16);
        M0_HIP(hs, hipMemcpyAsync(TAPX_, stream, bytes, hipMemcpyDeviceToDevice, st));
        if (second) M0_HIP(hs, hipMemcpyAsync(TAPA_, AA_, bytes, hipMemcpyDeviceToDevice, st));
        tap_second_ = second;
    };
    ConvNormOpts so;
    if (cfg_.chess_features) so.posenc = posenc_; else so.next_bn1 = first_bn1;
    M0_HIP(hs, conv_norm_act(stem_, stem_n_, x0, xa, T1_, Mc, st, so));
    tap(0, xa, so.next_bn1 != nullptr);
    if (cfg_.chess_features) {
        if (cfg_.piece_square_tables) {
            ConvNormOpts po;
            po.res = xa;
            M0_HIP(hs, conv_norm_act(pst_, pst_n_, xa, xb, T1_, Mc, st, po));
            std::swap(xa, xb);
        }
        tap(1, xa, false);
        ConvNormOpts io;
        io.res = xa; io.next_bn1 = first_bn1;
        M0_HIP(hs, conv_norm_act(inter_, inter_n_, xa, xb, T1_, Mc, st, io));
        std::swap(xa, xb);
        tap(2, xa, first_bn1 != nullptr);
    } else {
        tap(1, xa, false);
        tap(2, xa, false);
    }
    for (size_t li = 0; li < tower_.size(); ++li) {
        const TowerLayer& L = tower_[li];
        const NormParams* next_bn1 = bn1(L.next_bn1);
        if (L.kind == 0) {
            const ResBlockW& r = res_[L.index];
            M0_HIP(hs, conv_norm_act(r.conv1, r.bn2, AA_, T1_, T2_, Mc, st));
// ... 7 lines not shown
            } else {
                GemmArgs a = gemm_args(r.conv2, T1_, T2_, Mc);
                a.out_stats = S2_;
                M0_HIP(hs, run_gemm(r.conv2, a, st));
                EwArgs e = ew_args(T2_, xb, C, act);
                e.t_stats = S2_; e.res = xa;
                if (cfg_.se) { M0_HIP(hs, se_gate(r, S2_, Bp, st)); e.gate = G_; }
                ew_next_bn1(e, next_bn1, AA_);
                M0_HIP(hs, launch_ew_board(e, Bp, st));
            }
        } else {
            if (L.skip) { tap(3 + (int)li, xa, false); continue; }
            const AttnW& w = att_[L.index];
            const float inv_sqrt_d = 1.f / sqrtf((float)(C_ / cfg_.attention_heads));
            if (plan_.fuse_attn && w.blk_w != nullptr) {
                AttnBlockArgs ab;
                memset(&ab, 0, sizeof(ab));
                ab.x = xa; ab.wpack = w.blk_w; ab.bias = w.blk_bias; ab.mask = mask_dev_;
                ab.ln_g = w.ln.gamma; ab.ln_b = w.ln.beta; ab.y = xb;
                if (next_bn1) { ab.y2 = AA_; ab.gn2_gamma = next_bn1->gamma; ab.gn2_beta = next_bn1->beta; }
                ab.B = Bp; ab.ln_count = C_; ab.act = act; ab.grid_cap = sw_.attn_grid; ab.mix = cfg_.attention_unmasked_mix; ab.inv_sqrt_d = inv_sqrt_d;
                M0_HIP(hs, launch_attn_block(ab, st));
            } else {
                M0_HIP(hs, run_gemm(w.qkv, gemm_args(w.qkv, xa, QKV_, Mc), st));
                AttnArgs aa;
                aa.qkv = QKV_; aa.rel_bias = w.rel_bias; aa.mask = mask_dev_; aa.o = O_;
                aa.B = Bp; aa.H = C / 16; aa.C = C; aa.mix = cfg_.attention_unmasked_mix;
                aa.inv_sqrt_d = inv_sqrt_d;
                M0_HIP(hs, launch_attn_core(aa, st));
                M0_HIP(hs, run_gemm(w.proj, gemm_args(w.proj, O_, T1_, Mc), st));
                EwArgs e = ew_args(T1_, xb, C, act);
                e.res = xa; e.ln_g = w.ln.gamma; e.ln_b = w.ln.beta; e.ln_count = C_;
                ew_next_bn1(e, next_bn1, AA_);
                M0_HIP(hs, launch_ew_board(e, Bp, st));
            }
        }
        std::swap(xa, xb);
        tap(3 + (int)li, xa, next_bn1 != nullptr);
    }
    const bool joint = plan_.gn_small;
    if (joint) {
        GemmArgs a = gemm_args(hv_, xa, PH2_, Mc, act);
        a.gn_gamma = hv_n_.gamma; a.gn_beta = hv_n_.beta;
        a.ldo = 64; a.out2 = VH2_; a.ldo2 = 128; a.nsplit = 64;
        M0_HIP(hs, launch_conv_gemm(a, 1, st));
    } else {
        M0_HIP(hs, conv_norm_act(ph_conv_, ph_n_, xa, PH2_, PH_, Mc, st));
    }
    const bool factored = cfg_.policy_factor_rank > 0;
    if (factored) M0_HIP(hs, run_gemm(pfc1_, gemm_args(pfc1_, PH2_, F1_, Mfc, ACT_RELU), st));
    const PackedGemm& plast = factored ? pfc2_ : pfc1_;
    GemmArgs pl = gemm_args(plast, factored ? F1_ : PH2_, logits_dev, Mfc);
    pl.Mvalid = B; pl.out_f32 = 1; pl.out_scale = logit_scale_;
    M0_HIP(hs, run_gemm(plast, pl, st));
    if (!joint) M0_HIP(hs, conv_norm_act(vh0_, vh1_n_, xa, VH2_, VH_, Mc, st));
    _Float16* vflat = joint ? VH_ : VH2_;
    M0_HIP(hs, conv_norm_act(vh3_, vh4_n_, VH2_, vflat, VH_, Mc, st));
    M0_HIP(hs, run_gemm(vfc1_, gemm_args(vfc1_, vflat, F2_, Mfc, vact), st));
    M0_HIP(hs, run_gemm(vfc2_, gemm_args(vfc2_, F2_, F3_, Mfc, vact), st));
    GemmArgs vg = gemm_args(vgate_, F3_, F4_, Mfc, ACT_SIGMOID);
    vg.mul = F3_;
    M0_HIP(hs, run_gemm(vgate_, vg, st));
    GemmArgs v3 = gemm_args(vfc3_, F4_, VAL_, Mfc, ACT_TANH);
    v3.out_f32 = 1;
    M0_HIP(hs, run_gemm(vfc3_, v3, st));
    M0_HIP(hs, hipMemcpy2DAsync(value_dev, 4, VAL_, 32 * 4, 4, B, hipMemcpyDeviceToDevice, st));
    if (ssl_dev && !ssl_.empty()) {
        const int ctot = ssl_channels_total();
        int coff = 0;
        for (auto& h : ssl_) {
            M0_HIP(hs, conv_norm_act(h.c0, h.n, xa, SH2_, SH_, Mc, st));
            M0_HIP(hs, run_gemm(h.c1, gemm_args(h.c1, SH2_, SO_, Mc), st));
            M0_HIP(hs, launch_nhwc_to_nchw_f32(SO_, ssl_dev, B, 32, h.out_ch, ctot, coff, st));
            coff += h.out_ch;
        }
    }
    if (!hs.ok()) { err = "kernel launch failed: " + hs.message(); return M0_ERR_HIP; }
    return M0_OK;
}
```

matrix0_amd/csrc/net_kernels.h:

```cpp
#pragma once
#include <hip/hip_runtime.h>
#include <stdint.h>

enum { ACT_NONE = 0, ACT_RELU = 1, ACT_SILU = 2, ACT_LEAKY = 3, ACT_SIGMOID = 4, ACT_TANH = 5 };

enum ConvEpi {
    EPI_PLAIN,
    EPI_GN,
    EPI_ELEMENT,
    EPI_TAIL,
    EPI_TAIL_PRE,
};

constexpr int TAIL_SE_HMAX = 96;

struct GemmArgs {
    const _Float16* in;
    const _Float16* w;
    void* out;
    const float* gn_gamma;
    const float* gn_beta;
    const float* bias;
    const _Float16* mul;
    float* out_stats;
    int Mrows;
    int Mvalid;
    int Cin;
    int N;
    int Npad;
    int ldo;
    int epi_act;
    int out_f32;
    float out_scale;
    int ksplit;
    int w_pp;
    const _Float16* res;
    const float* pre_gamma;
    const float* pre_beta;
    _Float16* y2;
    const float* se_w1;
    const float* se_b1;
    const float* se_w2;
    const float* se_b2;
    int se_hidden;
    const void* se_wf;
    const float* posenc;
    void* out2;
    int ldo2;
    int nsplit;
};

struct EwArgs {
    const _Float16* t;
    const float* t_stats;
    const float* gn_gamma;
    const float* gn_beta;
    const float* gate;
    const _Float16* res;
    const float* posenc;
    const float* ln_g;
    const float* ln_b;
    int ln_count;
    _Float16* y;
    float* out_stats;
    _Float16* y2;
    const float* gn2_gamma;
    const float* gn2_beta;
    int C;
    int act;
};

struct SeGateArgs {
    const float* t_stats;
    const float* w1;
    const float* b1;
    const float* w2;
    const float* b2;
    float* gate;
    int B, C, hidden, act;
};

struct AttnArgs {
    const _Float16* qkv;
    const float* rel_bias;
    const uint64_t* mask;
    _Float16* o;
    int B, H, C;
    float mix;
    float inv_sqrt_d;
};

struct AttnBlockArgs {
    const _Float16* x;
    const void* wpack;
    const _Float16* bias;
    const uint64_t* mask;
    const float* ln_g;
    const float* ln_b;
    const float* gn2_gamma;
    const float* gn2_beta;
    _Float16* y;
    _Float16* y2;
// ... 21 lines not shown
```

matrix0_amd/csrc/selfplay.hip:

```cpp
#include <math.h>
#include <string.h>
#include <atomic>
#include "selfplay_engine.h"
#include "tb.h"

namespace m0 {

static bool nn_cache_miss(m0_selfplay* sp, uint64_t key) {
    auto it = sp->nn_map.find(key);
    if (it != sp->nn_map.end()) {
        sp->nn_lru.splice(sp->nn_lru.end(), sp->nn_lru, it->second);
        return false;
    }
    sp->nn_lru.push_back(key);
    sp->nn_map[key] = std::prev(sp->nn_lru.end());
    if (sp->nn_lru.size() > 10000) { sp->nn_map.erase(sp->nn_lru.front()); sp->nn_lru.pop_front(); }
    return true;
}

static void seed_game_dev(GameDev& g, uint64_t base, int uid) {
    g.seed_jitter = derive_seed(base, uid, PURPOSE_JITTER);
    g.seed_noise = derive_seed(base, uid, PURPOSE_NOISE);
    g.seed_dir = derive_seed(base, uid, PURPOSE_DIRICHLET);
    g.ctr_jitter = g.ctr_noise = g.ctr_dir = 0;
// ... 309 lines not shown
    }
}

static int harvest_games(m0_selfplay* sp) {
    if (!M0_HIP(sp->hip, hipMemcpy(sp->hres.data(), sp->d.results, sizeof(RootResult) * sp->G, hipMemcpyDeviceToHost)))
        return m0_hip_error(sp->hip, "harvest failed");
    for (int s = 0; s < sp->G; ++s) {
        if (!(sp->hg[s].active && sp->hg[s].finished)) continue;
        if (sp->hg[s].overflow) sp->stats.arena_overflows++;
        finish_search(sp, s);
    }
    start_games(sp);
    return apply_advances(sp);
}

static int harvest(m0_selfplay* sp) {
    switch (sp->kind) {
    case EngineKind::Analysis: return analysis_harvest(sp);
    default: return harvest_games(sp);
    }
}

static constexpr int M0_MAX_DEVICES = 16;
static std::mutex g_forward_gate[M0_MAX_DEVICES];
static std::atomic<int> g_engines_with_net[M0_MAX_DEVICES];
static bool forward_gate_enabled() {
    static const bool on = [] { const char* v = getenv("M0_FORWARD_GATE"); return v && v[0] == '1'; }();
    return on;
}

struct ForwardGate {
    std::mutex* m = nullptr;
    hipStream_t st = nullptr;
    ForwardGate(int device, hipStream_t stream, bool has_rows) : st(stream) {
        if (has_rows && forward_gate_enabled() && (unsigned)device < (unsigned)M0_MAX_DEVICES &&
            g_engines_with_net[device].load(std::memory_order_relaxed) > 1) {
            m = &g_forward_gate[device];
            m->lock();
        }
    }
    void release() {
        if (m) { (void)hipStreamSynchronize(st); m->unlock(); m = nullptr; }
    }
    ~ForwardGate() { release(); }
};

void forward_gate_join(m0_selfplay* sp) {
    if ((unsigned)sp->device < (unsigned)M0_MAX_DEVICES) { g_engines_with_net[sp->device].fetch_add(1); sp->counted = true; }
}
void forward_gate_leave(m0_selfplay* sp) {
    if (sp->counted) g_engines_with_net[sp->device].fetch_sub(1);
}

int finish_step(m0_selfplay* sp, int rows, double t0) {
    M0_HIP(sp->hip, hipEventRecord(sp->ev2, sp->stream));
    M0_HIP(sp->hip, launch_expand(sp->d, sp->tc, sp->stream));
    M0_HIP(sp->hip, hipEventRecord(sp->ev3, sp->stream));
    if (!sync_games_d2h(sp)) return m0_hip_error(sp->hip, "step failed");
    if (sp->net) sp->net->harvest_profile();
    if (sp->net_b) sp->net_b->harvest_profile();
    float ms_sel = 0, ms_net = 0, ms_exp = 0;
    M0_HIP(sp->hip, hipEventElapsedTime(&ms_sel, sp->ev0, sp->ev1));
    M0_HIP(sp->hip, hipEventElapsedTime(&ms_net, sp->ev1, sp->ev2));
    if (!M0_HIP(sp->hip, hipEventElapsedTime(&ms_exp, sp->ev2, sp->ev3))) return m0_hip_error(sp->hip, "step failed");
    sp->stats.ms_net += ms_net; sp->stats.ms_tree += ms_sel + ms_exp;
    sp->stats.steps++; sp->stats.evals += (uint64_t)rows;
    const double t1 = now_ms();
    bool any = false;
    if (sp->tc.eval_cache) {
        uint64_t h = 0;
        for (int s = 0; s < sp->G; ++s) h += sp->hg[s].cache_hits;
        sp->stats.evals_cached = h;
    }
    for (int s = 0; s < sp->G; ++s) {
        if (!sp->hg[s].active) continue;
        const int delta = sp->hg[s].sims_done - sp->prev_done[s];
        if (delta > 0) { sp->stats.sims += (uint64_t)delta; sp->prev_done[s] = sp->hg[s].sims_done; }
        if (sp->hg[s].finished) any = true;
    }
    if (any) { const int rc = harvest(sp); if (rc != M0_OK) return rc; }
    count_active_games(sp);
    const double t2 = now_ms();
    sp->stats.ms_host += t2 - t1;
    sp->stats.ms_total += t2 - t0;
    return M0_OK;
}

struct RowSplit { int main_rows, tail_rows; };
static RowSplit split_rows(int rows, bool have_tail, bool half_split) {
    int main_rows = rows;
    if (have_tail && rows >= 2048 && (rows & 1023) != 0) main_rows = rows & ~1023;
    if (have_tail && half_split && rows >= 4096) main_rows = ((rows / 2) + 1023) & ~1023;
    return {main_rows, rows - main_rows};
}

int one_step(m0_selfplay* sp) {
    std::string err;
    const double t0 = now_ms();
    M0_HIP(sp->hip, hipEventRecord(sp->ev0, sp->stream));
    int rows = 0;
    if (run_select(sp, &rows) != M0_OK) return M0_ERR_HIP;
    if (!M0_HIP(sp->hip, hipEventRecord(sp->ev1, sp->stream))) return m0_hip_error(sp->hip, "step failed");
    if (rows > sp->rows_max || sp->rows2[1] > sp->rows_max) { m0_set_error("row counter overflow"); return M0_ERR_STATE; }
    ForwardGate gate(sp->device, sp->stream, rows > 0 || sp->rows2[1] > 0);
    if (rows > 0) {
        if (!sp->net) { m0_set_error("m0_selfplay_step needs a network (use the split-step API without one)"); return M0_ERR_STATE; }
        const auto [main_rows, tail_rows] = split_rows(rows, sp->net_tail != nullptr, sp->half_split);
        float* ssl = sp->cfg.ssl_in_forward ? sp->ssl_dev : nullptr;
        if (tail_rows > 0 && !M0_HIP(sp->hip, hipEventRecord(sp->ev_sel, sp->stream)))
            return m0_hip_error(sp->hip, "step failed");
        m0_net_lock(sp->nethandle);
        int rc = sp->net->forward(nullptr, sp->d.x0, main_rows, sp->logits_dev, sp->values_dev, ssl, sp->stream, err);
        if (rc == M0_OK && tail_rows > 0 && M0_HIP(sp->hip, hipStreamWaitEvent(sp->stream_tail, sp->ev_sel, 0))) {
            const size_t sslw = ssl ? (size_t)sp->net->ssl_channels_total() * 64 : 0;
            rc = sp->net_tail->forward(nullptr, sp->d.x0 + (size_t)main_rows * 64 * 32, tail_rows, sp->logits_dev + (size_t)main_rows * 4672,
                                       sp->values_dev + main_rows, ssl ? ssl + (size_t)main_rows * sslw : nullptr, sp->stream_tail, err);
            M0_HIP(sp->hip, hipEventRecord(sp->ev_tail, sp->stream_tail));
            M0_HIP(sp->hip, hipStreamWaitEvent(sp->stream, sp->ev_tail, 0));
        }
        m0_net_unlock(sp->nethandle);
        if (rc != M0_OK) { sp->hip.check(sp->net->hip()); m0_set_error(err); return rc; }
        if (!sp->hip.ok()) return m0_hip_error(sp->hip, "step failed");
        sp->stats.rows_tail += (uint64_t)tail_rows;
    }
    if (sp->rows2[1] > 0) {
        if (!sp->net_b) { m0_set_error("rows for a second network without one"); return M0_ERR_STATE; }
        const size_t b = (size_t)sp->d.net_row_base;
        m0_net_lock(sp->nethandle_b);
        int rc = sp->net_b->forward(nullptr, sp->d.x0 + b * 64 * 32, sp->rows2[1], sp->logits_dev + b * 4672,
                                    sp->values_dev + b, nullptr, sp->stream, err);
        m0_net_unlock(sp->nethandle_b);
        if (rc != M0_OK) { sp->hip.check(sp->net_b->hip()); m0_set_error(err); return rc; }
        rows += sp->rows2[1];
    }
    gate.release();
    return finish_step(sp, rows, t0);
}

}
```

matrix0_amd/csrc/selfplay_engine.h:

```cpp
#pragma once
#include <hip/hip_runtime.h>
#include <chrono>
#include <deque>
#include <list>
#include <mutex>
#include <string>
#include <unordered_map>
#include <vector>
#include "../../include/m0_engine.h"
#include "capi_common.h"
#include "chess_core.h"
#include "host_rules.h"
#include "net.h"
#include "tree.h"

namespace m0 {

inline double now_ms() {
    return std::chrono::duration<double, std::milli>(std::chrono::steady_clock::now().time_since_epoch()).count();
}

struct GameRecordOwner {
    std::vector<float> s, pi, z, search_values, ssl;
    std::vector<uint8_t> legal_mask;
// ... 38 lines not shown
    std::deque<AnalysisJob> queue;
    std::deque<AnalysisJob> policy_queue;
    std::deque<m0_analysis_result> done;
    std::deque<std::vector<int32_t>> done_children;
    std::vector<AnalysisJob> slot_job;
    std::vector<uint8_t> held;
    int* reroot_in_dev = nullptr;
    RerootOut* reroot_out_dev = nullptr;
    std::vector<int> finished;
    std::vector<m0_analysis_line> hlines;
    std::vector<int> hnlines;
    std::vector<float> hvalues;
    std::vector<Pos> hpos;
    m0_analysis_line* lines_dev = nullptr;
    int* nlines_dev = nullptr;
    float* value_out_dev = nullptr;
    Pos* pos_dev = nullptr;
    int32_t* nlegal_dev = nullptr;
    uint16_t* moves_dev = nullptr;
    int32_t* idx_dev = nullptr;
    bool keep_visits = false;
    int32_t* child_idx_dev = nullptr;
    int32_t* child_n_dev = nullptr;
    int32_t* nchild_dev = nullptr;
    std::vector<int32_t> hchild_idx, hchild_n, hnchild;
};

}

struct m0_selfplay {
    m0::EngineKind kind = m0::EngineKind::SelfPlay;
    m0_selfplay_cfg cfg;
    TreeCfg tc;
    m0_net* nethandle = nullptr;
    m0_net* nethandle_b = nullptr;
    Net* net = nullptr;
    Net* net_b = nullptr;
    Net* net_tail = nullptr;
    hipStream_t stream_tail = nullptr;
    hipEvent_t ev_sel = nullptr, ev_tail = nullptr;
    bool half_split = false;
    int device = 0;
    hipStream_t stream = nullptr;
    bool own_stream = false;
    int G = 0, L = 0, cap = 0, rows_max = 0;
    TreeDev d;
    std::vector<void*> allocs;
    HipStatus hip;
    std::vector<GameDev> hg;
    std::vector<m0::HostGame> games;
    std::vector<RootResult> hres;
    float* logits_dev = nullptr;
    float* values_dev = nullptr;
    float* ssl_dev = nullptr;
    m0::Pos* ssl_pos_dev = nullptr;
    float* ssl_out_dev = nullptr;
    int ssl_cap = 0;
    m0::AdvanceList adv;
    int* ids_dev = nullptr;
    int* roots_dev = nullptr;
    std::deque<m0_game_record> done_meta;
    m0_selfplay_stats stats;
    int next_game = 0;
    hipEvent_t ev0 = nullptr, ev1 = nullptr, ev2 = nullptr, ev3 = nullptr;
    std::mutex mu;
    std::vector<Sample> hsamples;
    std::vector<int> prev_done;
    int last_rows = 0, last_rows_b = 0;
    int rows2[2] = {0, 0};
    std::vector<m0::Pos> book;
    std::vector<std::string> book_fens;
    std::list<uint64_t> nn_lru;
    std::unordered_map<uint64_t, std::list<uint64_t>::iterator> nn_map;
    bool ext_pending = false;
    bool counted = false;
    m0::Analysis* an = nullptr;
    const m0_tb* tb = nullptr;
    int tb_max_pieces = 0;
    uint64_t tb_adjudications = 0;
};

namespace m0 {

template <typename T>
T* dalloc(m0_selfplay* sp, size_t count) {
    void* p = nullptr;
    size_t bytes = count * sizeof(T);
    if (bytes == 0) bytes = 16;
    if (!M0_HIP(sp->hip, hipMalloc(&p, bytes))) return nullptr;
    sp->allocs.push_back(p);
    M0_HIP(sp->hip, hipMemsetAsync(p, 0, bytes, sp->stream));
    return (T*)p;
}
inline bool hip_ok(m0_selfplay* sp, const char* context) {
    if (!sp->hip.ok()) m0_hip_error(sp->hip, context);
    return sp->hip.ok();
}

bool kind_accepted(const m0_selfplay* sp, const char* what, unsigned kinds);
#define M0_ENGINE_CALL_OR(null_result, sp, what, kinds, on_device)                    \
    if (!(sp)) { m0_set_error(what ": sp is null"); return null_result; }             \
    std::lock_guard<std::mutex> lk((sp)->mu);                                         \
    if (!m0::kind_accepted(sp, what, kinds)) return M0_ERR_STATE;                     \
    if ((on_device) && !M0_HIP((sp)->hip, hipSetDevice((sp)->device))) return m0_hip_error((sp)->hip)
#define M0_ENGINE_CALL(sp, what, kinds, on_device) M0_ENGINE_CALL_OR(M0_ERR_INVALID, sp, what, kinds, on_device)

void forward_gate_join(m0_selfplay* sp);
void forward_gate_leave(m0_selfplay* sp);
bool sync_games_d2h(m0_selfplay* sp);
bool sync_games_h2d(m0_selfplay* sp);
HostGame& occupy_slot(m0_selfplay* sp, int slot, Line&& line, int uid);
void begin_search(m0_selfplay* sp, int slot, int sims, bool dirichlet, int root);
void arm_slot_search(m0_selfplay* sp, int slot, int sims, bool dirichlet, bool fresh);
int apply_advances(m0_selfplay* sp);
int run_select(m0_selfplay* sp, int* rows_out);
int refill(m0_selfplay* sp);
int one_step(m0_selfplay* sp);
int finish_step(m0_selfplay* sp, int rows, double t0);

m0_selfplay* engine_create(m0_net* nh, m0_net* nh_b, const m0_selfplay_cfg* cfg, EngineKind kind);
int ext_select_impl(m0_selfplay* sp, int* rows_a, int* rows_b, float* planes_a, float* planes_b, int max_rows);
int ext_expand_impl(m0_selfplay* sp, const float* logits_a, const float* values_a, int rows_a, const float* logits_b,
                    const float* values_b, int rows_b);

int analysis_refill(m0_selfplay* sp);
int analysis_harvest(m0_selfplay* sp);

}
```

matrix0_amd/csrc/tree.h:

```cpp
#pragma once
#include <hip/hip_runtime.h>
#include <stdint.h>
#include "chess_core.h"
namespace m0 { struct TbSet; }
#include "../../include/m0_engine.h"

#define M0_MAX_DEPTH 256
#define M0_HIST_CAP 192
#define M0_MAX_CHILDREN 256
constexpr int M0_NHWC_C = 32;

struct TreeCfg {
    double fpu_reduction;
    double draw_penalty;
    double virtual_loss;
    double selection_jitter;
    double cpuct;
    double cpuct_start, cpuct_end;
    int cpuct_plies;
    int use_c_base;
    double cpuct_c_base, cpuct_c_init;
    double dirichlet_alpha, dirichlet_frac;
    int legal_softmax;
    int enable_entropy_noise;
    int no_instant_backtrack;
    int virtual_loss_active;
    int leaves_per_step;
    int tt_merge;
    int raw_legal_priors;
    int max_children;
    double min_child_prior;
    int eval_cache;
};

#define M0_EC_MAXLEGAL 64
#define M0_EC_WORDS 66
struct EvalCache {
    uint64_t* keys;
    uint32_t* stamps;
    float* payload;
    float* hit_stage;
    int sets;
    int sides;
};

struct GameDev {
    m0::Pos root_pos;
    int root;
    int next;
    int arena;
    int active;
    int sims_done, sims_target;
    int need_dirichlet;
    int root_q_from_v;
    int flip_root_v;
    int root_fresh;
    int hist_len;
    int nsamples;
    int overflow;
    int finished;
    int root_n;
    double root_q;
    double root_v;
    uint64_t seed_jitter, seed_noise, seed_dir;
    uint64_t ctr_jitter, ctr_noise, ctr_dir;
    uint64_t evals;
    int net_id;
    int reinfer;
    uint64_t cache_hits;
    uint32_t cache_clock[2];
    int ec_clear;
    int side_next[2];
    int root_found;
    uint64_t tb_leaves;
};

enum SampleKind : int {
    SK_NONE = 0,
    SK_EVAL = 1,
    SK_ROOT_INIT = 2,
    SK_TERMINAL = 3,
    SK_ROOT_VALUE = 4,
    SK_CACHED = 5,
    SK_SHARED = 6,
};
// ... 6 lines not shown
    uint64_t ckey;
    int leaf;
    int depth;
    int row;
    int nlegal;
};
static_assert(sizeof(Sample) == 104, "the host copies Sample arrays device-to-host: the layout must not move");

struct TreeArrays {
    double* prior;
    double* w;
    double* q;
    int* n;
    int* vl;
    int* cbase;
    int16_t* nch;
    uint16_t* mv;
    uint16_t* midx;
    int cap;
};

struct RootResult {
    int nchild;
    int root_n;
    double root_q;
    int child_node[M0_MAX_CHILDREN];
    int child_n[M0_MAX_CHILDREN];
    uint16_t child_mv[M0_MAX_CHILDREN];
    uint16_t child_idx[M0_MAX_CHILDREN];
    double child_prior[M0_MAX_CHILDREN];
    double child_q[M0_MAX_CHILDREN];
};

struct TreeDev {
    TreeArrays t;
    GameDev* games;
    Sample* samples;
    int* paths;
    int* epaths;
    uint64_t* tt_keys;
    int* tt_nodes;
    int tt_cap;
    EvalCache ec;
    int search_nodes;
    int tt_sides;
    uint16_t* leaf_moves;
    uint64_t* hist;
    RootResult* results;
    int* row_counter;
    int net_row_base;
    _Float16* x0;
    const float* logits;
    const float* values;
    int G;
    int L;
    const m0::TbSet* tb_set;
    int tb_max_pieces;
};

hipError_t launch_select(const TreeDev& d, const TreeCfg& c, hipStream_t st);
hipError_t launch_expand(const TreeDev& d, const TreeCfg& c, hipStream_t st);
enum RootMode : int {
    ROOT_FRESH = -1,
    ROOT_FROM_SIDE_TABLE = -2,
    ROOT_FIRST_OF_GAME = -3,
};
hipError_t launch_advance(const TreeDev& d, const int* game_ids_dev, const int* child_slots_dev, int count, hipStream_t st);
#define M0_REROOT_MAX_MOVES 8
struct RerootOut { int32_t kept, n; double q; };
hipError_t launch_reroot_moves(const TreeDev& d, const int* slots_dev, const int* nmoves_dev, const int* moves_dev ,
                               int count, RerootOut* out_dev, hipStream_t st);

hipError_t launch_encode_positions(const m0::Pos* pos_dev, int n, float* planes_f32_dev ,
                                   _Float16* nhwc_dev , uint8_t* mask_dev ,
                                   int32_t* nlegal_dev, uint16_t* moves_dev , int32_t* idx_dev ,
                                   hipStream_t st);

hipError_t launch_decode_planes(const float* planes_dev, const uint8_t* mask_dev, int n, m0::Pos* pos_dev, int32_t* status_dev,
                                int32_t* flags_dev, int32_t* nlegal_dev, hipStream_t st);

hipError_t launch_analysis_lines(const TreeDev& d, const int* slots_dev, int count, int multipv, int pv_len,
                                 m0_analysis_line* lines_dev, int* nlines_dev, hipStream_t st);
hipError_t launch_root_children(const TreeDev& d, const int* slots_dev, int count, int32_t* policy_idx_dev, int32_t* visits_dev,
                                int32_t* nchild_dev, hipStream_t st);
hipError_t launch_policy_lines(const float* logits_dev, const float* values_dev, const int32_t* nlegal_dev, const uint16_t* moves_dev,
                               const int32_t* idx_dev, int rows, int multipv, m0_analysis_line* lines_dev, int* nlines_dev,
                               float* value_out_dev, hipStream_t st);

hipError_t launch_ssl_targets(const m0::Pos* pos_dev, int n, float* out_dev, hipStream_t st);

hipError_t launch_replay_games(const m0::Pos* start_dev, const uint32_t* patterns_dev, const int32_t* offsets_dev ,
                               int n_games, int max_plies, m0::Pos* pos_dev, uint16_t* moves_dev, int32_t* policy_idx_dev,
                               int32_t* nlegal_dev, int8_t* turn_dev, int32_t* plies_dev, int32_t* status_dev,
                               int32_t* end_flags_dev, hipStream_t st);
```

matrix0_amd/csrc/tree_device.h:

```cpp
#pragma once
#include <hip/hip_runtime.h>
#include <math.h>
#include "tree.h"

using namespace m0;

#define GOLDEN64 0x9E3779B97F4A7C15ull

__device__ __forceinline__ double u01(uint64_t seed, uint64_t k) {
    return (double)(mix64(seed + (k + 1) * GOLDEN64) >> 11) * (1.0 / 9007199254740992.0);
}
__device__ __forceinline__ double normal_at(uint64_t seed, uint64_t k) {
    double u1 = u01(seed, k), u2 = u01(seed, k + 1);
    if (u1 < 1e-300) u1 = 1e-300;
    return sqrt(-2.0 * log(u1)) * cos(2.0 * 3.141592653589793 * u2);
}
static __device__ double gamma_draw(uint64_t seed, uint64_t& ctr, double a) {
    double boost = 1.0;
    if (a < 1.0) {
        double u = u01(seed, ctr++);
        boost = pow(u, 1.0 / a);
        a += 1.0;
    }
    const double d = a - 1.0 / 3.0, c = 1.0 / sqrt(9.0 * d);
    for (int it = 0; it < 1000; ++it) {
        double x = normal_at(seed, ctr); ctr += 2;
        double v = 1.0 + c * x;
        if (v <= 0.0) continue;
        v = v * v * v;
        double u = u01(seed, ctr++);
        if (u < 1e-300) u = 1e-300;
        if (log(u) < 0.5 * x * x + d - d * v + d * log(v)) return d * v * boost;
    }
    return d * boost;
}

struct Arena {
    double* prior; double* w; double* q; int* n; int* vl; int* cbase; int16_t* nch; uint16_t* mv; uint16_t* midx;
};
__device__ __forceinline__ Arena arena_of(const TreeArrays& t, int g, int half) {
    size_t b = ((size_t)g * 2 + half) * (size_t)t.cap;
    Arena a;
    a.prior = t.prior + b; a.w = t.w + b; a.q = t.q + b; a.n = t.n + b; a.vl = t.vl + b;
    a.cbase = t.cbase + b; a.nch = t.nch + b; a.mv = t.mv + b; a.midx = t.midx + b;
    return a;
}
__device__ __forceinline__ void node_reset(const Arena& A, int i, double prior, Move mv, uint16_t midx) {
    A.prior[i] = prior; A.w[i] = 0.0; A.q[i] = 0.0; A.n[i] = 0; A.vl[i] = 0;
    A.cbase[i] = -1; A.nch[i] = -1; A.mv[i] = mv; A.midx[i] = midx;
}
__device__ __forceinline__ void node_copy(const Arena& D, int dn, const Arena& S, int so) {
    D.prior[dn] = S.prior[so]; D.w[dn] = S.w[so]; D.q[dn] = S.q[so]; D.n[dn] = S.n[so]; D.vl[dn] = 0;
    D.cbase[dn] = S.cbase[so]; D.nch[dn] = S.nch[so]; D.mv[dn] = S.mv[so]; D.midx[dn] = S.midx[so];
}

__device__ __forceinline__ float wave_max_f(float v) {
    for (int o = 32; o > 0; o >>= 1) v = fmaxf(v, __shfl_xor(v, o));
    return v;
}
__device__ __forceinline__ float wave_sum_f(float v) {
    for (int o = 32; o > 0; o >>= 1) v += __shfl_xor(v, o);
    return v;
}
__device__ __forceinline__ double wave_sum_d(double v) {
    for (int o = 32; o > 0; o >>= 1) v += __shfl_xor(v, o);
    return v;
}

constexpr int CPL = M0_MAX_CHILDREN / 64;
static_assert(M0_POLICY_SIZE % 4 == 0, "logit rows are read as 16-byte pieces");

__device__ __forceinline__ bool row_nonfinite(const float* lg, int lane) {
    constexpr int N4 = M0_POLICY_SIZE / 4, PER_LANE = (N4 + 63) / 64;
    const uint4* lg4 = reinterpret_cast<const uint4*>(lg);
    uint4 v[PER_LANE];
#pragma unroll
    for (int k = 0; k < PER_LANE; ++k) { const int j = lane + 64 * k; v[k] = lg4[j < N4 ? j : N4 - 1]; }
    uint32_t acc = 0;
#pragma unroll
    for (int k = 0; k < PER_LANE; ++k) {
        acc |= (uint32_t)((v[k].x & 0x7f800000u) == 0x7f800000u) | (uint32_t)((v[k].y & 0x7f800000u) == 0x7f800000u) |
               (uint32_t)((v[k].z & 0x7f800000u) == 0x7f800000u) | (uint32_t)((v[k].w & 0x7f800000u) == 0x7f800000u);
    }
    return acc != 0;
}

__device__ __forceinline__ void wave_softmax(const float (&l)[CPL], int n, int lane, float (&pr)[CPL]) {
    float mx = -3.0e38f;
#pragma unroll
    for (int k = 0; k < CPL; ++k) mx = fmaxf(mx, l[k]);
    mx = wave_max_f(mx);
    double e[CPL], sum = 0.0;
#pragma unroll
    for (int k = 0; k < CPL; ++k) { const int i = lane + 64 * k; e[k] = i < n ? exp((double)(l[k] - mx)) : 0.0; sum += e[k]; }
    sum = wave_sum_d(sum);
#pragma unroll
    for (int k = 0; k < CPL; ++k) pr[k] = (float)(e[k] / sum);
}

__device__ __forceinline__ int reserve_row(const TreeDev& d, const GameDev* gd, int lane) {
    int row = 0;
    if (lane == 0) row = atomicAdd(d.row_counter + gd->net_id, 1) + gd->net_id * d.net_row_base;
    return __shfl(row, 0);
}
__device__ __forceinline__ double root_value(const GameDev* gd, float v) {
    double rv = fmax(-1.0, fmin(1.0, (double)v));
    if (gd->flip_root_v) rv = -rv;
    return rv;
}

__device__ __forceinline__ uint64_t tt_key_of(const Pos& p) { const uint64_t k = tkey(p); return k ? k : 1ull; }
__device__ __forceinline__ int tt_home(uint64_t key, int cap) { return (int)((key ^ (key >> 29)) & (uint64_t)(cap - 1)); }
__device__ __forceinline__ size_t tt_table_of(const TreeDev& d, int g, const GameDev* gd) {
    return ((size_t)g * d.tt_sides + (d.tt_sides == 2 ? gd->arena : 0)) * (size_t)d.tt_cap;
}
__device__ __forceinline__ void tt_clear(uint64_t* keys, int nkeys, int lane) {
    uint4* tk = reinterpret_cast<uint4*>(keys);
    for (int i = lane; i < nkeys / 2; i += 64) tk[i] = make_uint4(0, 0, 0, 0);
}
// ... 92 lines not shown
```

matrix0_amd/csrc/tree_expand.hip:

```cpp
#include "tree_device.h"
#include "eval_cache.h"

struct ExpandScratch {
    float pr[M0_MAX_CHILDREN];
    uint8_t keep[M0_MAX_CHILDREN];
    float total;
    int bad;
};

struct ExpandEnv {
    Arena A;
    int cap;
    GameDev* gd;
    uint64_t* TK; int* TN; int tt_cap;
    ExpandScratch* X;
    int lane;
};
struct LeafLogits {
    const float* row;
    const float* legal;
    float* store;
};
__device__ __forceinline__ LeafLogits logits_of_row(const float* row, float* store) { return LeafLogits{row, nullptr, store}; }
__device__ __forceinline__ LeafLogits logits_of_cache(const float* payload) { return LeafLogits{nullptr, payload + EC_LOGITS, nullptr}; }

static __device__ float np_sum_f32_dev(const float* a, int n) {
    auto block = [&](const float* b, int m) -> float {
        if (m < 8) { float r = 0.f; for (int i = 0; i < m; ++i) r += b[i]; return r; }
        float r[8];
        for (int j = 0; j < 8; ++j) r[j] = b[j];
        int i;
        for (i = 8; i < m - (m % 8); i += 8)
            for (int j = 0; j < 8; ++j) r[j] += b[i + j];
        float res = ((r[0] + r[1]) + (r[2] + r[3])) + ((r[4] + r[5]) + (r[6] + r[7]));
        for (; i < m; ++i) res += b[i];
        return res;
    };
    if (n <= 128) return block(a, n);
    int n2 = n / 2;
    n2 -= n2 % 8;
    return block(a, n2) + block(a + n2, n - n2);
}

__device__ __forceinline__ void priors_raw(const float* lg, const int (&idx)[CPL], int n, int lane, ExpandScratch* X, float (&pr)[CPL]) {
#pragma unroll
    for (int k = 0; k < CPL; ++k) { const int i = lane + 64 * k; if (i < n) X->pr[i] = lg[idx[k]]; }
    __syncthreads();
    if (lane == 0) X->total = np_sum_f32_dev(X->pr, n);
    __syncthreads();
    const float total = X->total;
    const bool ok = isfinite(total) && total > 0.f;
#pragma unroll
    for (int k = 0; k < CPL; ++k) { const int i = lane + 64 * k; pr[k] = i < n ? (ok ? X->pr[i] / total : 1.0f / (float)n) : 0.f; }
    __syncthreads();
}

__device__ __forceinline__ void priors_uniform(int n, float (&pr)[CPL]) {
#pragma unroll
    for (int k = 0; k < CPL; ++k) pr[k] = 1.0f / (float)n;
}

__device__ __forceinline__ void priors_legal_softmax(const LeafLogits& src, const int (&idx)[CPL], int n, int lane, GameDev* gd,
                                                     const TreeCfg& c, float (&pr)[CPL]) {
    double ent = 0.0;
    float l[CPL];
#pragma unroll
    for (int k = 0; k < CPL; ++k) {
        const int i = lane + 64 * k;
        l[k] = i < n ? (src.legal ? src.legal[i] : src.row[idx[k]]) : -3.0e38f;
        if (src.store && i < n && i < M0_EC_MAXLEGAL) src.store[EC_LOGITS + i] = l[k];
    }
    wave_softmax(l, n, lane, pr);
#pragma unroll
    for (int k = 0; k < CPL; ++k) {
        const int i = lane + 64 * k;
        if (i < n) ent -= (double)pr[k] * log((double)pr[k] + 1e-8);
    }
// ... 83 lines not shown
    for (int k = 0; k < CPL; ++k) {
        const int i = lane + 64 * k;
        slot[k] = -1;
        if (i < n && X->keep[i]) {
            int r = 0;
            if (topk) { for (int j = 0; j < n; ++j) r += (X->keep[j] && (X->pr[j] > pr[k] || (X->pr[j] == pr[k] && j < i))) ? 1 : 0; }
            else { for (int j = 0; j < i; ++j) r += X->keep[j]; }
            if (r < nkeep) slot[k] = r;
        }
    }
    __syncthreads();
    return nkeep;
}

__device__ __forceinline__ bool write_children(const ExpandEnv& E, int leaf, const Pos& pos, const Move (&mvv)[CPL], const int (&idx)[CPL],
                                               const float (&pr)[CPL], const int (&slot)[CPL], int n, int nkeep, bool reg_children,
                                               double q0) {
    const Arena& A = E.A;
    GameDev* gd = E.gd;
    const int lane = E.lane;
    const int cb = gd->next;
    if (cb + nkeep > E.cap) { if (lane == 0) gd->overflow = 1; return false; }
#pragma unroll
    for (int k = 0; k < CPL; ++k) {
        const int i = lane + 64 * k;
        if (i < n && slot[k] >= 0) {
            const int ci = cb + slot[k];
            node_reset(A, ci, (double)pr[k], mvv[k], (uint16_t)idx[k]);
            if (q0 != 0.0) A.q[ci] = q0;
            if (E.TK && reg_children) {
                Pos q = pos;
                make_move(q, mvv[k]);
                tt_insert(E.TK, E.TN, E.tt_cap, tt_key_of(q), ci);
            }
        }
    }
    if (E.TK && !reg_children && lane == 0) tt_insert(E.TK, E.TN, E.tt_cap, tt_key_of(pos), leaf);
    if (lane == 0) { A.cbase[leaf] = cb; A.nch[leaf] = (int16_t)nkeep; gd->next = cb + nkeep; }
    __syncthreads();
    return true;
}

__device__ __forceinline__ double child_seed_q(const TreeCfg& c, const Arena& A, const int* path, int depth) {
    if (c.tt_merge || depth < 1) return 0.0;
    const double pq = A.q[path[depth - 1]];
    return pq != 0.0 ? -pq : 0.0;
}

__device__ __forceinline__ bool expand_node(const ExpandEnv& E, const TreeCfg& c, int leaf, const Pos& pos, const uint16_t* smoves, int n,
                                   const LeafLogits& src, bool is_root, bool reg_children, double q0) {
    const int lane = E.lane;
    if (n <= 0) return true;
    bool bad = false;
    if (!src.legal) bad = row_nonfinite(src.row, lane);
    bad = __any(bad);
    if (lane == 0) E.X->bad = bad ? 1 : 0;
    float pr[CPL];
    int idx[CPL];
    Move mvv[CPL];
#pragma unroll
    for (int k = 0; k < CPL; ++k) {
        const int i = lane + 64 * k;
        pr[k] = 0.f; idx[k] = 0; mvv[k] = 0;
        if (i < n) { mvv[k] = smoves[i]; idx[k] = move_to_index(pos, mvv[k]); }
    }
    if (c.raw_legal_priors && c.legal_softmax && !is_root) priors_raw(src.row, idx, n, lane, E.X, pr);
    else if (bad) priors_uniform(n, pr);
    else {
        if (c.legal_softmax) priors_legal_softmax(src, idx, n, lane, E.gd, c, pr);
        else priors_full_softmax(src.row, idx, n, lane, E.gd, c, pr);
        priors_renormalise(n, lane, pr);
    }
    int slot[CPL];
    const int nkeep = prune_children(c, pr, n, lane, E.X, slot);
    return write_children(E, leaf, pos, mvv, idx, pr, slot, n, nkeep, reg_children, q0);
}

__device__ __forceinline__ void expand_evaluated(const TreeDev& d, const TreeCfg& c, const ExpandEnv& E, int g, const Sample& smp,
                                                 const uint16_t* moves, const float* lg, float v, double q0) {
    const Arena& A = E.A;
    GameDev* gd = E.gd;
    const int lane = E.lane, kind = smp.kind, leaf = smp.leaf;
    const Pos pos = smp.pos;
    float* cw = nullptr;
    size_t ce = 0;
    const uint64_t ckey = kind == SK_EVAL ? smp.ckey : 0ull;
    if (ckey != 0 && isfinite(v)) {
        ce = ec_choose_victim(d.ec, gd, g, ckey, lane);
        cw = ec_payload(d.ec, ce);
        ec_invalidate(d.ec, ce, lane);
    }
    const bool ok = expand_node(E, c, leaf, pos, moves, smp.nlegal, logits_of_row(lg, cw), kind == SK_ROOT_INIT,
                                !(kind == SK_ROOT_INIT && gd->root_fresh), q0);
    if (c.eval_cache && kind == SK_EVAL && lane == 0 && A.nch[leaf] < 0) A.cbase[leaf] = -1;
    const int sig = cw ? legal_sig(moves, smp.nlegal, lane) : 0;
    if (cw && lane == 0) {
        if (ok && !E.X->bad) ec_publish(d.ec, gd, ce, ckey, v, sig);
    }
}

__device__ __forceinline__ void release_inflight(const TreeDev& d, const TreeCfg& c, const Arena& A, int g, const Sample* S, const int* P,
                                                 int ns, int lane) {
    for (int s = lane; s < ns; s += 64) {
        if (sample_holds_inflight(S[s].kind)) {
            const int* path = (c.tt_merge ? d.epaths + (size_t)g * (d.L + 1) * M0_MAX_DEPTH : P) + (size_t)s * M0_MAX_DEPTH;
            for (int dd = 1; dd <= S[s].depth; ++dd) atomicSub(&A.vl[path[dd]], 1);
        }
    }
}

__device__ __forceinline__ void write_root_result(RootResult* R, const Arena& A, int root, int lane) {
    const int k = A.nch[root] > 0 ? A.nch[root] : 0;
    const int cb = A.cbase[root];
    for (int i = lane; i < k; i += 64) {
        R->child_node[i] = cb + i; R->child_n[i] = A.n[cb + i];
        R->child_mv[i] = A.mv[cb + i]; R->child_idx[i] = A.midx[cb + i];
        R->child_prior[i] = A.prior[cb + i]; R->child_q[i] = A.q[cb + i];
    }
    if (lane == 0) { R->nchild = k; R->root_n = A.n[root]; R->root_q = A.q[root]; }
}

__global__ __launch_bounds__(64) void expand_kernel(TreeDev d, TreeCfg c) {
    __shared__ ExpandScratch X;
    const int g = blockIdx.x, lane = threadIdx.x;
    GameDev* gd = &d.games[g];
    if (!gd->active) return;
    uint64_t* TK = c.tt_merge ? d.tt_keys + tt_table_of(d, g, gd) : nullptr;
    int* TN = c.tt_merge ? d.tt_nodes + tt_table_of(d, g, gd) : nullptr;
    const uint16_t* LM = d.leaf_moves + (size_t)g * (d.L + 1) * M0_MAX_CHILDREN;
    const int ns = gd->nsamples;
    if (ns <= 0) return;
    const Arena A = arena_of(d.t, g, gd->arena);
    const ExpandEnv E{A, d.t.cap, gd, TK, TN, d.tt_cap, &X, lane};
    const Sample* S = d.samples + (size_t)g * (d.L + 1);
    const int* P = d.paths + (size_t)g * (d.L + 1) * M0_MAX_DEPTH;
    const bool may_repeat = c.tt_merge != 0;
    int sims = 0;
    uint64_t evals = 0, hits = 0;
    for (int s = 0; s < ns; ++s) {
        const int kind = S[s].kind;
        const int* path = P + (size_t)s * M0_MAX_DEPTH;
        const uint16_t* moves = LM + (size_t)s * M0_MAX_CHILDREN;
        if (kind == SK_SHARED) {
            const float v = d.values[S[s].row];
            backprop(A, path, S[s].depth, (double)v, lane, may_repeat, NoMirror{});
// ... 59 lines not shown
```

matrix0_amd/csrc/tree_select.hip:

```cpp
#include "tree_device.h"
#include "tb_core.h"
#include "eval_cache.h"
#include "movegen_wave.h"
#include "kernel_common.h"

__device__ __forceinline__ double cpuct_at(const TreeCfg& c, int ply) {
    if (c.use_c_base) {
        double N = fmax(1.0, (double)(ply + 1));
        return c.cpuct_c_init + log((N + c.cpuct_c_base) / c.cpuct_c_base);
    }
    if (c.cpuct_plies <= 0) return c.cpuct;
    int p = ply < 0 ? 0 : (ply > c.cpuct_plies ? c.cpuct_plies : ply);
    double t = (double)p / (double)c.cpuct_plies;
    return c.cpuct_start + (c.cpuct_end - c.cpuct_start) * t;
}
static __device__ void apply_dirichlet(const Arena& A, int root, GameDev* gd, const TreeCfg& c, double* sg, int lane) {
    const int k = A.nch[root];
    if (k <= 0 || c.dirichlet_frac <= 0.0) return;
    const int cb = A.cbase[root];
    uint64_t ctr = gd->ctr_dir;
    double sum = 0.0;
    for (int i = 0; i < k; ++i) {
        double gmm = gamma_draw(gd->seed_dir, ctr, c.dirichlet_alpha);
        if (lane == 0) sg[i] = gmm;
// ... 144 lines not shown
    int ncached = 0;
    if (!c.tt_merge && nleaf > 0) {
        ncached = gd->next < M0_SEL_CACHE ? gd->next : M0_SEL_CACHE;
        for (int i = lane; i < ncached; i += 64) {
            TC->prior[i] = A.prior[i]; TC->q[i] = A.q[i]; TC->n[i] = A.n[i]; TC->vl[i] = A.vl[i]; TC->cbase[i] = A.cbase[i];
            TC->nch[i] = A.nch[i]; TC->mv[i] = A.mv[i];
        }
        __syncthreads();
    }
    uint64_t ctrj = gd->ctr_jitter;
    const uint64_t seedj = gd->seed_jitter;
    const double jit = c.selection_jitter > 0.0 ? c.selection_jitter : 0.001;
    const int hist_len = gd->hist_len;
    const uint64_t* H = d.hist + (size_t)g * M0_HIST_CAP;

    for (int s = 0; s < nleaf; ++s) {
        Pos pos = gd->root_pos;
        int* path = P + (size_t)s * M0_MAX_DEPTH;
        int* epath = c.tt_merge ? EP + (size_t)s * M0_MAX_DEPTH : nullptr;
        int node = root, depth = 0;
        int prev_from = -1, prev_to = -1;
        if (lane == 0) { path[0] = root; if (epath) epath[0] = root; }
        const bool rh = node < ncached;
        int nc = TOP(nch, rh, node), cb = TOP(cbase, rh, node), nn = TOP(n, rh, node);
        double nq = TOP(q, rh, node);
        while (true) {
            if (nc <= 0 || depth >= M0_MAX_DEPTH - 1) break;
            const double sq = sqrt((double)(nn > 1 ? nn : 1));
            const double eff = cpuct_at(c, depth);
            double best = -1e9;
            int bi = -1;
            int b_nch = 0, b_cb = 0, b_n = 0, b_vl = 0;
            double b_q = 0.0;
            Move b_mv = 0;
            for (int i = lane; i < nc; i += 64) {
                const int ci = cb + i;
                const bool hit = ci < ncached;
                const int cn = TOP(n, hit, ci);
                const double cq = TOP(q, hit, ci);
                const int c_nch = TOP(nch, hit, ci), c_cb = TOP(cbase, hit, ci);
                const Move m = TOP(mv, hit, ci);
                const double cprior = TOP(prior, hit, ci);
                const double qq = cn == 0 ? nq - c.fpu_reduction : cq;
                const double u = eff * cprior * (sq / (1.0 + (double)cn));
                double sc = qq + u;
                if (c.no_instant_backtrack && depth >= 1) {
                    if (mv_from(m) == prev_to && mv_to(m) == prev_from) sc -= 0.01;
                }
                const int cvl = c.virtual_loss_active ? TOP(vl, hit, ci) : 0;
                if (c.virtual_loss_active && c.virtual_loss > 0.0) sc -= (double)cvl * c.virtual_loss;
                sc += (u01(seedj, ctrj + (uint64_t)i) - 0.5) * jit;
                if (sc > best) { best = sc; bi = i; b_nch = c_nch; b_cb = c_cb; b_n = cn; b_q = cq; b_mv = m; b_vl = cvl; }
            }
            for (int off = 32; off > 0; off >>= 1) {
                const double ob = __shfl_xor(best, off);
                const int oi = __shfl_xor(bi, off);
                if (oi >= 0 && (bi < 0 || ob > best || (ob == best && oi < bi))) { best = ob; bi = oi; }
            }
            ctrj += (uint64_t)nc;
            if (bi < 0) bi = 0;
            const int child = cb + bi;
            const int wl = bi & 63;
            nc = __shfl(b_nch, wl); cb = __shfl(b_cb, wl); nn = __shfl(b_n, wl); nq = __shfl(b_q, wl);
            const Move m = (Move)__shfl((int)b_mv, wl);
            const uint64_t k = tkey(pos);
            const bool irr = irreversible(pos, m);
            if (lane == 0) { pkey[depth] = k; pirr[depth] = irr ? 1 : 0; }
            make_move(pos, m);
            const int vlw = __shfl(b_vl, wl);
            if (lane == 0 && c.virtual_loss_active) { A.vl[child] = vlw + 1; if (child < ncached) TC->vl[child] = vlw + 1; }
            prev_from = mv_from(m); prev_to = mv_to(m);
            node = child; ++depth;
            if (c.tt_merge) {
                const int tn = tt_lookup(TK, TN, d.tt_cap, tt_key_of(pos), lane);
                if (tn >= 0 && tn != child) {
                    node = tn;
                    nc = A.nch[node]; cb = A.cbase[node]; nn = A.n[node]; nq = A.q[node];
                }
                if (lane == 0) epath[depth] = child;
            }
            if (lane == 0) path[depth] = node;
        }
        __syncthreads();
        const int nlegal = gen_legal_wave(pos, smoves, spseudo, lane);
        double tv;
        bool tb_hit;
        const bool term = leaf_terminal(d, c, pos, nlegal, depth, pkey, pirr, H, hist_len, lane, tv, tb_hit);
        if (tb_hit && lane == 0) gd->tb_leaves++;
        uint64_t ckey = 0;
        bool cached = false;
        if (!term && c.eval_cache && d.ec.sets > 0 && nlegal <= M0_EC_MAXLEGAL) {
            ckey = ec_key_of(pos);
            cached = ec_probe(d, gd, g, s, ckey, smoves, nlegal, lane);
        }
        emit_leaf(d, c, A, gd, S + s, LM + (size_t)s * M0_MAX_CHILDREN, pos, node, depth, smoves, nlegal, term, cached, ckey, lane);
        __syncthreads();
        if (term) {
            backprop(A, path, depth, tv, lane, c.tt_merge != 0, [&](int nd, int nn, double qq) {
                if (nd < ncached) { TC->n[nd] = nn; TC->q[nd] = qq; }
            });
            __syncthreads();
            __builtin_amdgcn_fence(__ATOMIC_ACQUIRE, "agent");
        }
    }
    if (reinfer) emit_root_value(d, gd, S, nleaf, root, lane);
    if (lane == 0) { gd->ctr_jitter = ctrj; gd->nsamples = nleaf + (reinfer ? 1 : 0); }
}

hipError_t launch_select(const TreeDev& d, const TreeCfg& c, hipStream_t st) {
    static DeviceOnce once;
    hipError_t e = once.run([] {
        return hipFuncSetAttribute(reinterpret_cast<const void*>(&select_kernel), hipFuncAttributeMaxDynamicSharedMemorySize, M0_SEL_CACHE_BYTES);
    });
    if (e != hipSuccess) return e;
    hipLaunchKernelGGL(select_kernel, dim3(d.G), dim3(64), M0_SEL_CACHE_BYTES, st, d, c);
    return hipGetLastError();
}
```

Before: 1.170.

## Add DPP wave argmax in tree select, fused row nonfinite flags, stem loop kernel

Replaces the shuffle-based wave argmax in MCTS child selection with DPP row operations plus readlane broadcasts, on by default and switchable through M0_TREE_DPP. Adds an optional per-row nonfinite flag written in the f32 GEMM epilogue, so leaf expansion can read one byte instead of scanning the whole 4672-wide logit row. It also adds a new stem loop conv kernel and threads the new argument through every forward call. The extra epilogue work and the DPP code path add some risk.

```diff
diff --git a/include/m0_engine.h b/include/m0_engine.h
--- a/include/m0_engine.h
+++ b/include/m0_engine.h
@@ -279,4 +279,5 @@
 #endif
 #include "m0_analysis_live.h"
 #include "m0_score.h"
+#include "m0_net_flags.h"
 #endif
diff --git a/include/m0_net_flags.h b/include/m0_net_flags.h
--- /dev/null
+++ b/include/m0_net_flags.h
@@ -0,0 +1,12 @@
+#ifndef M0_NET_FLAGS_H
+#define M0_NET_FLAGS_H
+#ifdef __cplusplus
+extern "C" {
+#endif
+
+int m0_net_last_row_flags(m0_net* net, uint8_t* flags, int max_rows, int* rows);
+
+#ifdef __cplusplus
+}
+#endif
+#endif
diff --git a/matrix0_amd/_abi.py b/matrix0_amd/_abi.py
--- a/matrix0_amd/_abi.py
+++ b/matrix0_amd/_abi.py
@@ -215,10 +215,15 @@
     "m0_score_bench": (i32, [i32, i32, i32, P(f32), P(f64)]),
 }
 
+NET_FLAG_FUNCTIONS = {
+    "m0_net_last_row_flags": (i32, [vp, vp, i32, _pi32]),
+}
+
 
 def bind(L) -> list:
     missing = []
-    for name, (restype, argtypes) in list(FUNCTIONS.items()) + list(LIVE_FUNCTIONS.items()) + list(SCORE_FUNCTIONS.items()):
+    for name, (restype, argtypes) in (list(FUNCTIONS.items()) + list(LIVE_FUNCTIONS.items()) + list(SCORE_FUNCTIONS.items())
+                                      + list(NET_FLAG_FUNCTIONS.items())):
         fn = getattr(L, name, None)
         if fn is None:
             missing.append(name)
diff --git a/matrix0_amd/backend.py b/matrix0_amd/backend.py
--- a/matrix0_amd/backend.py
+++ b/matrix0_amd/backend.py
@@ -41,6 +41,7 @@
         if not self._h:
             raise RuntimeError(f"m0_net_create failed: {_lib.last_error()}")
         self._finalized = False
+        self._last_rows = 0
         self.ssl_tasks = [t for t in _lib.SSL_ORDER if self._cfg.ssl_tasks & _lib.SSL_BITS[t]] \
             if self._cfg.self_supervised else []
 
@@ -80,6 +81,12 @@
     def infer_np_ssl(self, arr: np.ndarray):
         return self._infer(arr, True)
 
+    def last_row_flags(self) -> np.ndarray:
+        flags = np.zeros(max(1, self._last_rows), dtype=np.uint8)
+        rows = C.c_int(0)
+        _lib.check(self._L.m0_net_last_row_flags(self._h, _lib.ptr(flags), flags.shape[0], C.byref(rows)), "m0_net_last_row_flags")
+        return flags[:rows.value].astype(bool)
+
     def tap_info(self) -> Tuple[int, int]:
         steps, width = C.c_int(0), C.c_int(0)
         _lib.check(self._L.m0_net_tap_info(self._h, C.byref(steps), C.byref(width)), "m0_net_tap_info")
@@ -98,6 +105,7 @@
             raise ValueError(f"expected input [B,{self._cfg.planes},8,8], got {a.shape}")
         a = np.ascontiguousarray(a, dtype=np.float32)
         B = a.shape[0]
+        self._last_rows = B
         pol = np.empty((B, _lib.POLICY_SIZE), dtype=np.float32)
         val = np.empty((B,), dtype=np.float32)
         sslc = self._L.m0_net_ssl_channels(self._h)
diff --git a/matrix0_amd/csrc/argmax_rule.h b/matrix0_amd/csrc/argmax_rule.h
--- /dev/null
+++ b/matrix0_amd/csrc/argmax_rule.h
@@ -0,0 +1,11 @@
+#pragma once
+#if defined(__HIPCC__)
+#define M0_ARGMAX_HD __host__ __device__ inline
+#else
+#define M0_ARGMAX_HD inline
+#endif
+
+M0_ARGMAX_HD bool argmax_beats(double os, int oi, double s, int i) { return oi >= 0 && (i < 0 || os > s || (os == s && oi < i)); }
+M0_ARGMAX_HD void argmax_combine(double& s, int& i, double os, int oi) {
+    if (argmax_beats(os, oi, s, i)) { s = os; i = oi; }
+}
diff --git a/matrix0_amd/csrc/capi_analysis.hip b/matrix0_amd/csrc/capi_analysis.hip
--- a/matrix0_amd/csrc/capi_analysis.hip
+++ b/matrix0_amd/csrc/capi_analysis.hip
@@ -130,7 +130,7 @@
         return m0_hip_error(hs, "position encode failed");
     std::string err;
     m0_net_lock(sp->nethandle);
-    const int rc = sp->net->forward(nullptr, sp->d.x0, n, sp->logits_dev, sp->values_dev, nullptr, sp->stream, err);
+    const int rc = sp->net->forward(nullptr, sp->d.x0, n, sp->logits_dev, sp->values_dev, nullptr, nullptr, sp->stream, err);
     m0_net_unlock(sp->nethandle);
     if (rc != M0_OK) { hs.check(sp->net->hip()); m0_set_error(err); return rc; }
     M0_HIP(hs, launch_policy_lines(sp->logits_dev, sp->values_dev, a.nlegal_dev, a.moves_dev, a.idx_dev, n, a.opts.multipv, a.lines_dev,
diff --git a/matrix0_amd/csrc/capi_net.hip b/matrix0_amd/csrc/capi_net.hip
--- a/matrix0_amd/csrc/capi_net.hip
+++ b/matrix0_amd/csrc/capi_net.hip
@@ -23,6 +23,8 @@
     float* logits_dev = nullptr;
     float* value_dev = nullptr;
     float* ssl_dev = nullptr;
+    uint8_t* row_bad_dev = nullptr;
+    int flag_rows = 0;
     int cap = 0;
     float* score_pi_dev = nullptr;
     float* score_z_dev = nullptr;
@@ -92,6 +94,7 @@
     if (n->logits_dev) (void)hipFree(n->logits_dev);
     if (n->value_dev) (void)hipFree(n->value_dev);
     if (n->ssl_dev) (void)hipFree(n->ssl_dev);
+    if (n->row_bad_dev) (void)hipFree(n->row_bad_dev);
     if (n->score_pi_dev) (void)hipFree(n->score_pi_dev);
     if (n->score_z_dev) (void)hipFree(n->score_z_dev);
     if (n->score_mask_dev) (void)hipFree(n->score_mask_dev);
@@ -127,6 +130,9 @@
         if (*p) M0_HIP(hs, hipFree(*p));
         *p = nullptr;
     }
+    if (n->row_bad_dev) M0_HIP(hs, hipFree(n->row_bad_dev));
+    n->row_bad_dev = nullptr;
+    n->flag_rows = 0;
     n->cap = 0;
     int cap = B < 64 ? 64 : B;
     const int P = n->net->cfg().planes;
@@ -135,6 +141,7 @@
     M0_HIP(hs, hipMalloc((void**)&n->logits_dev, (size_t)cap * M0_POLICY_SIZE * 4));
     M0_HIP(hs, hipMalloc((void**)&n->value_dev, (size_t)cap * 4));
     M0_HIP(hs, hipMalloc((void**)&n->ssl_dev, (size_t)cap * (sslc > 0 ? sslc : 1) * 64 * 4));
+    M0_HIP(hs, hipMalloc((void**)&n->row_bad_dev, (size_t)cap));
     if (!hs.ok()) return m0_hip_error(hs, "hipMalloc failed for I/O staging");
     n->cap = cap;
     return M0_OK;
@@ -172,8 +179,10 @@
     std::string err;
     if (!M0_HIP(hs, hipMemcpyAsync(n->planes_dev, planes, (size_t)B * P * 64 * 4, hipMemcpyHostToDevice, n->stream)))
         return m0_hip_error(hs, "H2D copy");
-    rc = n->net->forward(n->planes_dev, nullptr, B, n->logits_dev, n->value_dev, ssl ? n->ssl_dev : nullptr, n->stream, err);
+    n->flag_rows = 0;
+    rc = n->net->forward(n->planes_dev, nullptr, B, n->logits_dev, n->value_dev, ssl ? n->ssl_dev : nullptr, n->row_bad_dev, n->stream, err);
     if (rc != M0_OK) { m0_set_error(err); return rc; }
+    if (n->net->writes_row_flags()) n->flag_rows = B;
     M0_HIP(hs, hipMemcpyAsync(policy, n->logits_dev, (size_t)B * M0_POLICY_SIZE * 4, hipMemcpyDeviceToHost, n->stream));
     M0_HIP(hs, hipMemcpyAsync(value, n->value_dev, (size_t)B * 4, hipMemcpyDeviceToHost, n->stream));
     if (ssl) M0_HIP(hs, hipMemcpyAsync(ssl, n->ssl_dev, (size_t)B * sslc * 64 * 4, hipMemcpyDeviceToHost, n->stream));
@@ -207,6 +216,21 @@
     return infer_locked(n, planes, B, policy, value, ssl);
 }
 
+int m0_net_last_row_flags(m0_net* n, uint8_t* flags, int max_rows, int* rows) {
+    if (!n || !flags || !rows) { m0_set_error("null argument"); return M0_ERR_INVALID; }
+    std::lock_guard<std::mutex> lk(n->mu);
+    HipStatus& hs = n->net->hip();
+    if (!M0_HIP(hs, hipSetDevice(n->device))) return m0_hip_error(hs);
+    if (!n->net->writes_row_flags()) { m0_set_error("the network writes no row flags (M0_ROW_FLAGS=0)"); return M0_ERR_STATE; }
+    if (n->flag_rows > max_rows) { m0_set_error("output buffer too small"); return M0_ERR_INVALID; }
+    *rows = n->flag_rows;
+    if (n->flag_rows > 0) {
+        M0_HIP(hs, hipMemcpyAsync(flags, n->row_bad_dev, (size_t)n->flag_rows, hipMemcpyDeviceToHost, n->stream));
+        if (!M0_HIP(hs, hipStreamSynchronize(n->stream))) return m0_hip_error(hs, "copy failed");
+    }
+    return M0_OK;
+}
+
 int m0_net_score(m0_net* n, const float* planes, const float* pi, const float* z, const uint8_t* legal_mask, int B,
                  const m0_score_opts* opts, float* rows) {
     if (!n || !planes || !pi || !z || !rows) { m0_set_error("null argument"); return M0_ERR_INVALID; }
@@ -226,7 +250,7 @@
     if (masked) M0_HIP(hs, hipMemcpyAsync(n->score_mask_dev, legal_mask, cells, hipMemcpyHostToDevice, n->stream));
     if (!hs.ok()) return m0_hip_error(hs, "H2D copy");
     std::string err;
-    rc = n->net->forward(n->planes_dev, nullptr, B, n->logits_dev, n->value_dev, nullptr, n->stream, err);
+    rc = n->net->forward(n->planes_dev, nullptr, B, n->logits_dev, n->value_dev, nullptr, nullptr, n->stream, err);
     if (rc != M0_OK) { m0_set_error(err); return rc; }
     M0_HIP(hs, launch_score_rows(n->logits_dev, n->value_dev, n->score_pi_dev, n->score_z_dev, masked ? n->score_mask_dev : nullptr,
                                  B, *opts, n->score_rows_dev, n->stream));
@@ -312,7 +336,7 @@
         if (!M0_HIP(hs, hipMemcpy(n->planes_dev, h.data(), h.size() * 4, hipMemcpyHostToDevice))) return m0_hip_error(hs, "H2D copy");
     }
     float* ssl = ((with_ssl & 1) && n->net->ssl_channels_total() > 0) ? n->ssl_dev : nullptr;
-    rc = n->net->forward(n->planes_dev, nullptr, B, n->logits_dev, n->value_dev, ssl, n->stream, err);
+    rc = n->net->forward(n->planes_dev, nullptr, B, n->logits_dev, n->value_dev, ssl, n->row_bad_dev, n->stream, err);
     if (rc != M0_OK) { m0_set_error(err); return rc; }
     struct Events {
         hipEvent_t e0 = nullptr, e1 = nullptr;
@@ -321,7 +345,7 @@
     M0_HIP(hs, hipEventCreate(&ev.e0)); M0_HIP(hs, hipEventCreate(&ev.e1));
     M0_HIP(hs, hipEventRecord(ev.e0, n->stream));
     for (int i = 0; i < iters && hs.ok(); ++i) {
-        rc = n->net->forward(n->planes_dev, nullptr, B, n->logits_dev, n->value_dev, ssl, n->stream, err);
+        rc = n->net->forward(n->planes_dev, nullptr, B, n->logits_dev, n->value_dev, ssl, n->row_bad_dev, n->stream, err);
         if (rc != M0_OK) { m0_set_error(err); return rc; }
     }
     M0_HIP(hs, hipEventRecord(ev.e1, n->stream));
diff --git a/matrix0_amd/csrc/capi_selfplay.hip b/matrix0_amd/csrc/capi_selfplay.hip
--- a/matrix0_amd/csrc/capi_selfplay.hip
+++ b/matrix0_amd/csrc/capi_selfplay.hip
@@ -1,3 +1,4 @@
+#include <stdlib.h>
 #include <string.h>
 #include <algorithm>
 #include <memory>
@@ -14,6 +15,8 @@
     t.virtual_loss_active = c.virtual_loss_active; t.leaves_per_step = c.inference_batch_size;
     t.tt_merge = c.tt_merge; t.raw_legal_priors = c.raw_legal_priors; t.max_children = c.max_children;
     t.min_child_prior = c.min_child_prior;
+    const char* e = getenv("M0_TREE_DPP");
+    t.tree_dpp = (e && e[0] == '0') ? 0 : 1;
     t.eval_cache = ((match ? c.arena_eval_cache : c.eval_cache) && c.legal_softmax && !c.raw_legal_priors && !c.tt_merge) ? 1 : 0;
 }
 
@@ -76,6 +79,8 @@
     sp->d.x0 = dalloc<_Float16>(sp, (size_t)(nreg * sp->rows_max + 4) * 64 * 32);
     sp->logits_dev = dalloc<float>(sp, (size_t)nreg * sp->rows_max * 4672);
     sp->values_dev = dalloc<float>(sp, (size_t)nreg * sp->rows_max + 4);
+    if (sp->net && sp->net->writes_row_flags() && (!sp->net_b || sp->net_b->writes_row_flags()))
+        sp->row_bad_dev = dalloc<uint8_t>(sp, (size_t)nreg * sp->rows_max + 4);
     sp->d.net_row_base = sp->rows_max;
     if (sp->cfg.ssl_in_forward && sp->net && sp->net->ssl_channels_total() > 0)
         sp->ssl_dev = dalloc<float>(sp, (size_t)sp->rows_max * sp->net->ssl_channels_total() * 64);
@@ -213,7 +218,7 @@
     upload_eval(sp, (size_t)sp->d.net_row_base, logits_b, values_b, rows_b);
     sp->ext_pending = false;
     M0_HIP(sp->hip, hipEventRecord(sp->ev0, sp->stream)); M0_HIP(sp->hip, hipEventRecord(sp->ev1, sp->stream));
-    return finish_step(sp, rows_a + rows_b, now_ms());
+    return finish_step(sp, rows_a + rows_b, now_ms(), false);
 }
 
 bool m0::kind_accepted(const m0_selfplay* sp, const char* what, unsigned kinds) {
diff --git a/matrix0_amd/csrc/conv_epilogue.h b/matrix0_amd/csrc/conv_epilogue.h
--- a/matrix0_amd/csrc/conv_epilogue.h
+++ b/matrix0_amd/csrc/conv_epilogue.h
@@ -78,7 +78,7 @@
     gn16_affine(mean, rstd, gamma[col], beta[col], scale, shift);
 }
 
-template <ConvEpi EPI, int ACT, int NT>
+template <ConvEpi EPI, int ACT, int NT, bool ROW_FLAGS = false>
 __device__ __forceinline__ void conv_tile_epilogue(float16v (&acc)[2][NT], const GemmArgs& a, char* lds_wave, int m0,
                                                    int n0, int wm, int wn, int lane, int out_col0 = 0) {
     const int half = lane >> 5;
@@ -144,10 +144,12 @@
         const bool want_stats = a.out_stats != nullptr;
         const bool has_mul = a.mul != nullptr;
         const bool f32out = a.out_f32 != 0;
+        uint32_t badrows = 0;
         static_for<0, NT>([&](auto ni_) __attribute__((always_inline)) {
             constexpr int ni = decltype(ni_)::value;
             const int col = colbase + ni * 32;
             const float bias = a.bias != nullptr ? a.bias[col] : 0.f;
+            const uint32_t counts = col < a.N ? 1u : 0u;
             float s = 0.f, ss = 0.f;
             static_for<0, 2>([&](auto mi_) __attribute__((always_inline)) {
                 constexpr int mi = decltype(mi_)::value;
@@ -160,6 +162,8 @@
                     if (has_mul) v *= (float)a.mul[(size_t)row * ldo + col];
                     v *= oscale;
                     s += v; ss += v * v;
+                    if constexpr (ROW_FLAGS)
+                        badrows |= (counts & (uint32_t)((__float_as_uint(v) & 0x7f800000u) == 0x7f800000u)) << (mi * 16 + r);
                     if (row < a.Mvalid) {
                         if (f32out) reinterpret_cast<float*>(a.out)[(size_t)row * ldo + col] = v;
                         else reinterpret_cast<_Float16*>(a.out)[(size_t)row * ldo + col] = (_Float16)v;
@@ -175,5 +179,14 @@
                 }
             }
         });
+        if constexpr (ROW_FLAGS) {
+            if (badrows != 0 && f32out && a.row_bad != nullptr) {
+                static_for<0, 32>([&](auto k_) __attribute__((always_inline)) {
+                    constexpr int k = decltype(k_)::value, mi = k / 16, r = k % 16;
+                    const int row = rowbase + mi * 32 + (r & 3) + 8 * (r >> 2);
+                    if (((badrows >> k) & 1u) && row < a.Mvalid) a.row_bad[row] = 1;
+                });
+            }
+        }
     }
 }
diff --git a/matrix0_amd/csrc/conv_gemm.hip b/matrix0_amd/csrc/conv_gemm.hip
--- a/matrix0_amd/csrc/conv_gemm.hip
+++ b/matrix0_amd/csrc/conv_gemm.hip
@@ -1,7 +1,7 @@
 #include "kernel_common.h"
 #include "conv_epilogue.h"
 
-template <int TAPS, int WN, int NT, int KC, ConvEpi EPI = EPI_ELEMENT, int ACT = ACT_NONE>
+template <int TAPS, int WN, int NT, int KC, ConvEpi EPI = EPI_ELEMENT, int ACT = ACT_NONE, bool ROW_FLAGS = false>
 __global__ __launch_bounds__(256 * WN) void conv_gemm_kernel(GemmArgs a) {
     constexpr int NB = WN * NT * 32;
     constexpr int NTHR = 256 * WN;
@@ -137,8 +137,99 @@
         if (a.out2 != nullptr && n0 + wn * NT * 32 >= a.nsplit) { o.out = a.out2; o.ldo = a.ldo2; out_col0 = a.nsplit; }
         conv_tile_epilogue<EPI_GN, ACT, NT>(acc, o, smem + wave * (64 * 64 * NT), m0, n0, wm, wn, lane, out_col0);
     } else {
-        conv_tile_epilogue<EPI_ELEMENT, ACT_NONE, NT>(acc, a, smem, m0, n0, wm, wn, lane);
-    }
+        conv_tile_epilogue<EPI_ELEMENT, ACT_NONE, NT, ROW_FLAGS>(acc, a, smem, m0, n0, wm, wn, lane);
+    }
+}
+
+template <int ACT>
+__global__ __launch_bounds__(256) __attribute__((amdgpu_waves_per_eu(2, 2))) void stem_loop_kernel(GemmArgs a) {
+    constexpr int NT = 2, KC = 32, NB = NT * 32, NTHR = 256, AST = KC + 8, K8 = KC / 8;
+    constexpr int A_ELEMS = 4 * 100 * AST, W_ELEMS = NB * AST;
+    constexpr int A_PER = 4 * 64 * K8 / NTHR;
+    static_assert(NB * K8 == NTHR, "one 16-byte weight piece per thread and tap");
+    static_assert(((A_ELEMS + 2 * W_ELEMS) * 2) % 16 == 0, "staging images are read in 16-byte pieces");
+
+    extern __shared__ __attribute__((aligned(16))) char smem[];
+    _Float16* A_lds = reinterpret_cast<_Float16*>(smem);
+    _Float16* W_lds = A_lds + A_ELEMS;
+    char* const stage = smem + (A_ELEMS + 2 * W_ELEMS) * 2;
+
+    const int tid = threadIdx.x;
+    const int lane = tid & 63;
+    const int wm = tid >> 6;
+    const int m0 = blockIdx.x * 256;
+    const int Npad = a.Npad;
+    const int nblocks = Npad / NB;
+
+    auto load_W = [&](int tap, int n0) { return *reinterpret_cast<const uint4*>(a.w + ((size_t)tap * Npad + n0) * KC + (size_t)tid * 8); };
+    uint4 wreg = load_W(0, 0);
+
+    for (int i = tid; i < A_ELEMS / 8; i += NTHR) reinterpret_cast<uint4*>(A_lds)[i] = make_uint4(0, 0, 0, 0);
+    __syncthreads();
+#pragma unroll
+    for (int i = 0; i < A_PER; ++i) {
+        const int p = tid + i * NTHR;
+        const int row = p / K8, b = row >> 6, px = row & 63;
+        const uint4 v = *reinterpret_cast<const uint4*>(a.in + (size_t)(m0 + row) * KC + (p % K8) * 8);
+        *reinterpret_cast<uint4*>(A_lds + (b * 100 + ((px >> 3) + 1) * 10 + (px & 7) + 1) * AST + (p % K8) * 8) = v;
+    }
+
+    int apix[2];
+#pragma unroll
+    for (int mi = 0; mi < 2; ++mi) {
+        const int px = mi * 32 + (lane & 31);
+        apix[mi] = wm * 100 + ((px >> 3) + 1) * 10 + (px & 7) + 1;
+    }
+    const int khalf = 8 * (lane >> 5);
+
+    int gs = 0;
+#pragma unroll 1
+    for (int nb = 0; nb < nblocks; ++nb) {
+        const int n0 = nb * NB;
+        float16v acc[2][NT];
+        static_for<0, 2>([&](auto mi) __attribute__((always_inline)) {
+            static_for<0, NT>([&](auto ni) __attribute__((always_inline)) {
+                acc[decltype(mi)::value][decltype(ni)::value] = float16v{0.f, 0.f, 0.f, 0.f, 0.f, 0.f, 0.f, 0.f,
+                                                                          0.f, 0.f, 0.f, 0.f, 0.f, 0.f, 0.f, 0.f};
+            });
+        });
+#pragma unroll 1
+        for (int tap = 0; tap < 9; ++tap, ++gs) {
+            *reinterpret_cast<uint4*>(W_lds + (gs & 1) * W_ELEMS + (tid / K8) * AST + (tid % K8) * 8) = wreg;
+            __syncthreads();
+            if (tap + 1 < 9) wreg = load_W(tap + 1, n0);
+            else if (nb + 1 < nblocks) wreg = load_W(0, n0 + NB);
+            const int tapoff = (tap / 3 - 1) * 10 + (tap % 3 - 1);
+            const _Float16* Wb = W_lds + (gs & 1) * W_ELEMS + (lane & 31) * AST + khalf;
+            static_for<0, KC / 16>([&](auto kk_) __attribute__((always_inline)) {
+                constexpr int kk = decltype(kk_)::value;
+                half8 af0 = *reinterpret_cast<const half8*>(A_lds + (apix[0] + tapoff) * AST + kk * 16 + khalf);
+                half8 af1 = *reinterpret_cast<const half8*>(A_lds + (apix[1] + tapoff) * AST + kk * 16 + khalf);
+                static_for<0, NT>([&](auto ni_) __attribute__((always_inline)) {
+                    constexpr int ni = decltype(ni_)::value;
+                    half8 bf = *reinterpret_cast<const half8*>(Wb + ni * 32 * AST + kk * 16);
+                    acc[0][ni] = __builtin_amdgcn_mfma_f32_32x32x16_f16(af0, bf, acc[0][ni], 0, 0, 0);
+                    acc[1][ni] = __builtin_amdgcn_mfma_f32_32x32x16_f16(af1, bf, acc[1][ni], 0, 0, 0);
+                });
+            });
+        }
+        int ln = lane;
+        asm volatile("" : "+v"(ln));
+        conv_tile_epilogue<EPI_GN, ACT, NT>(acc, a, stage + wm * (64 * 64 * NT), m0, n0, wm, 0, ln);
+    }
+}
+
+template <int ACT>
+static hipError_t launch_stem_loop(const GemmArgs& a, hipStream_t st) {
+    constexpr size_t lds = (size_t)(4 * 100 * 40 + 2 * 64 * 40) * 2 + 4 * 64 * 64 * 2;
+    static DeviceOnce once;
+    hipError_t e = once.run([] {
+        return hipFuncSetAttribute(reinterpret_cast<const void*>(&stem_loop_kernel<ACT>), hipFuncAttributeMaxDynamicSharedMemorySize,
+                                   160 * 1024);
+    });
+    if (e != hipSuccess) return e;
+    hipLaunchKernelGGL((stem_loop_kernel<ACT>), dim3(a.Mrows / 256), dim3(256), lds, st, a);
+    return hipGetLastError();
 }
 
 template <int TAPS, int WN, int NT, int KC>
@@ -151,25 +242,28 @@
     return main_loop > staging ? main_loop : staging;
 }
 
-template <int TAPS, int WN, int NT, int KC, ConvEpi EPI = EPI_ELEMENT, int ACT = ACT_NONE>
+template <int TAPS, int WN, int NT, int KC, ConvEpi EPI = EPI_ELEMENT, int ACT = ACT_NONE, bool ROW_FLAGS = false>
 static hipError_t launch_conv_gemm_t(const GemmArgs& a, hipStream_t st) {
     constexpr int NB = WN * NT * 32;
     size_t lds = conv_gemm_lds<TAPS, WN, NT, KC>();
     static DeviceOnce once;
     hipError_t e = once.run([] {
-        return hipFuncSetAttribute(reinterpret_cast<const void*>(&conv_gemm_kernel<TAPS, WN, NT, KC, EPI, ACT>),
+        return hipFuncSetAttribute(reinterpret_cast<const void*>(&conv_gemm_kernel<TAPS, WN, NT, KC, EPI, ACT, ROW_FLAGS>),
                                    hipFuncAttributeMaxDynamicSharedMemorySize, 160 * 1024);
     });
     if (e != hipSuccess) return e;
     dim3 grid(a.Mrows / 256, a.Npad / NB);
-    hipLaunchKernelGGL((conv_gemm_kernel<TAPS, WN, NT, KC, EPI, ACT>), grid, dim3(256 * WN), lds, st, a);
+    hipLaunchKernelGGL((conv_gemm_kernel<TAPS, WN, NT, KC, EPI, ACT, ROW_FLAGS>), grid, dim3(256 * WN), lds, st, a);
     return hipGetLastError();
 }
 template <int ACT>
 static hipError_t launch_conv_gemm_gn(const GemmArgs& a, int taps, hipStream_t st) {
     if (a.bias != nullptr || a.mul != nullptr || a.out_stats != nullptr || a.out_f32 || a.out_scale != 1.f || a.Npad != a.N)
         return hipErrorInvalidValue;
-    if (taps == 9) return a.Npad % 64 == 0 && a.out2 == nullptr ? launch_conv_gemm_t<9, 1, 2, 32, EPI_GN, ACT>(a, st) : hipErrorInvalidValue;
+    if (taps == 9) {
+        if (a.Npad % 64 != 0 || a.out2 != nullptr) return hipErrorInvalidValue;
+        return a.nloop && a.Cin == 32 ? launch_stem_loop<ACT>(a, st) : launch_conv_gemm_t<9, 1, 2, 32, EPI_GN, ACT>(a, st);
+    }
     if (a.posenc != nullptr) return hipErrorInvalidValue;
     if (a.out2 != nullptr) return a.Npad == 192 && a.nsplit == 64 ? launch_conv_gemm_t<1, 3, 2, 32, EPI_GN, ACT>(a, st) : hipErrorInvalidValue;
     if (a.Npad == 160) return launch_conv_gemm_t<1, 1, 5, 32, EPI_GN, ACT>(a, st);
@@ -192,6 +286,7 @@
 hipError_t launch_conv_gemm(const GemmArgs& a, int taps, hipStream_t st) {
     if (a.Mrows % 256 != 0 || a.Cin % 32 != 0 || a.Npad % 32 != 0) return hipErrorInvalidValue;
     const bool big = conv_gemm_tile_n(a.Cin, a.Npad) == 320;
+    if (a.row_bad != nullptr && !(taps == 1 && !big && a.gn_gamma == nullptr && a.out_f32)) return hipErrorInvalidValue;
     if (a.gn_gamma != nullptr && !big) {
         if (a.epi_act == ACT_SILU) return launch_conv_gemm_gn<ACT_SILU>(a, taps, st);
         if (a.epi_act == ACT_RELU) return launch_conv_gemm_gn<ACT_RELU>(a, taps, st);
@@ -205,7 +300,11 @@
         return launch_conv_gemm_t<9, 1, 1, 32>(a, st);
     } else if (taps == 1) {
         if (big) return a.w_pp ? hipErrorInvalidValue : launch_conv_big(a, 1, st);
-        if (a.Mrows / 256 >= 256 && a.Npad % 64 == 0) return launch_conv_gemm_t<1, 1, 2, 32>(a, st);
+        const bool wide = a.Mrows / 256 >= 256 && a.Npad % 64 == 0;
+        if (a.row_bad != nullptr)
+            return wide ? launch_conv_gemm_t<1, 1, 2, 32, EPI_ELEMENT, ACT_NONE, true>(a, st)
+                        : launch_conv_gemm_t<1, 1, 1, 32, EPI_ELEMENT, ACT_NONE, true>(a, st);
+        if (wide) return launch_conv_gemm_t<1, 1, 2, 32>(a, st);
         return launch_conv_gemm_t<1, 1, 1, 32>(a, st);
     }
     return hipErrorInvalidValue;
diff --git a/matrix0_amd/csrc/net.h b/matrix0_amd/csrc/net.h
--- a/matrix0_amd/csrc/net.h
+++ b/matrix0_amd/csrc/net.h
@@ -80,7 +80,8 @@
     const std::vector<size_t>& device_buffer_bytes() const { return dev_sizes_; }
 
     int forward(const float* planes_dev, const _Float16* nhwc_dev, int B, float* logits_dev, float* value_dev,
-                float* ssl_dev, hipStream_t st, std::string& err);
+                float* ssl_dev, uint8_t* row_bad, hipStream_t st, std::string& err);
+    bool writes_row_flags() const { return sw_.row_flags; }
     int ensure_workspace(int B, std::string& err);
     int ssl_channels_total() const;
     const m0_net_cfg& cfg() const { return cfg_; }
@@ -107,7 +108,7 @@
     int device_;
     hipStream_t stream_ = nullptr;
     HipStatus own_hip_, *hip_ = &own_hip_;
-    struct Switches { bool fuse_tail = true, fuse_attn = true; int attn_grid = 0; } sw_;
+    struct Switches { bool fuse_tail = true, fuse_attn = true, row_flags = true, stem_loop = true; int attn_grid = 0; } sw_;
     struct Plan {
         bool fuse_tail = false;
         bool fuse_attn = false;
diff --git a/matrix0_amd/csrc/net.hip b/matrix0_amd/csrc/net.hip
--- a/matrix0_amd/csrc/net.hip
+++ b/matrix0_amd/csrc/net.hip
@@ -23,6 +23,8 @@
     auto off = [](const char* name) { const char* e = getenv(name); return e && e[0] == '0'; };
     sw_.fuse_tail = !off("M0_FUSE_TAIL");
     sw_.fuse_attn = !off("M0_FUSE_ATTN");
+    sw_.stem_loop = !off("M0_STEM_LOOP");
+    sw_.row_flags = !off("M0_ROW_FLAGS");
     if (const char* e = getenv("M0_ATTN_GRID")) sw_.attn_grid = std::max(0, atoi(e));
     C_ = cfg.channels;
     Cp_ = (C_ > 256 && C_ < 320) ? 320 : C_;
@@ -207,6 +209,7 @@
                               : plan_.gn_small && (g.taps == 9 ? g.Cin == 32 : g.N == 32 || g.N == 64 || g.N == 128 || g.N == 160);
     if (epilogue && !o.res && !o.next_bn1) {
         a.gn_gamma = n.gamma; a.gn_beta = n.beta; a.epi_act = plan_.act; a.posenc = o.posenc;
+        a.nloop = !big && g.taps == 9 && sw_.stem_loop && Mrows / 256 >= 512;
         return run_gemm(g, a, st);
     }
     a.out = scratch; a.out_stats = S1_;
@@ -232,7 +235,7 @@
 }
 
 int Net::forward(const float* planes_dev, const _Float16* nhwc_dev, int B, float* logits_dev, float* value_dev,
-                 float* ssl_dev, hipStream_t st, std::string& err) {
+                 float* ssl_dev, uint8_t* row_bad, hipStream_t st, std::string& err) {
     if (!finalized_) { err = "weights not finalized"; return M0_ERR_STATE; }
     if (B <= 0) { err = "batch must be positive"; return M0_ERR_INVALID; }
     if (int rc = ensure_workspace(B, err)) return rc;
@@ -346,6 +349,10 @@
     const PackedGemm& plast = factored ? pfc2_ : pfc1_;
     GemmArgs pl = gemm_args(plast, factored ? F1_ : PH2_, logits_dev, Mfc);
     pl.Mvalid = B; pl.out_f32 = 1; pl.out_scale = logit_scale_;
+    if (row_bad && sw_.row_flags) {
+        M0_HIP(hs, hipMemsetAsync(row_bad, 0, (size_t)B, st));
+        pl.row_bad = row_bad;
+    }
     M0_HIP(hs, run_gemm(plast, pl, st));
     if (!joint) M0_HIP(hs, conv_norm_act(vh0_, vh1_n_, xa, VH2_, VH_, Mc, st));
     _Float16* vflat = joint ? VH_ : VH2_;
diff --git a/matrix0_amd/csrc/net_kernels.h b/matrix0_amd/csrc/net_kernels.h
--- a/matrix0_amd/csrc/net_kernels.h
+++ b/matrix0_amd/csrc/net_kernels.h
@@ -48,6 +48,8 @@
     void* out2;
     int ldo2;
     int nsplit;
+    uint8_t* row_bad;
+    int nloop;
 };
 
 struct EwArgs {
diff --git a/matrix0_amd/csrc/selfplay.hip b/matrix0_amd/csrc/selfplay.hip
--- a/matrix0_amd/csrc/selfplay.hip
+++ b/matrix0_amd/csrc/selfplay.hip
@@ -385,9 +385,11 @@
     if (sp->counted) g_engines_with_net[sp->device].fetch_sub(1);
 }
 
-int finish_step(m0_selfplay* sp, int rows, double t0) {
+int finish_step(m0_selfplay* sp, int rows, double t0, bool net_flags) {
     M0_HIP(sp->hip, hipEventRecord(sp->ev2, sp->stream));
-    M0_HIP(sp->hip, launch_expand(sp->d, sp->tc, sp->stream));
+    TreeDev d = sp->d;
+    if (net_flags) d.row_bad = sp->row_bad_dev;
+    M0_HIP(sp->hip, launch_expand(d, sp->tc, sp->stream));
     M0_HIP(sp->hip, hipEventRecord(sp->ev3, sp->stream));
     if (!sync_games_d2h(sp)) return m0_hip_error(sp->hip, "step failed");
     if (sp->net) sp->net->harvest_profile();
@@ -443,11 +445,13 @@
         if (tail_rows > 0 && !M0_HIP(sp->hip, hipEventRecord(sp->ev_sel, sp->stream)))
             return m0_hip_error(sp->hip, "step failed");
         m0_net_lock(sp->nethandle);
-        int rc = sp->net->forward(nullptr, sp->d.x0, main_rows, sp->logits_dev, sp->values_dev, ssl, sp->stream, err);
+        uint8_t* const bad = sp->row_bad_dev;
+        int rc = sp->net->forward(nullptr, sp->d.x0, main_rows, sp->logits_dev, sp->values_dev, ssl, bad, sp->stream, err);
         if (rc == M0_OK && tail_rows > 0 && M0_HIP(sp->hip, hipStreamWaitEvent(sp->stream_tail, sp->ev_sel, 0))) {
             const size_t sslw = ssl ? (size_t)sp->net->ssl_channels_total() * 64 : 0;
             rc = sp->net_tail->forward(nullptr, sp->d.x0 + (size_t)main_rows * 64 * 32, tail_rows, sp->logits_dev + (size_t)main_rows * 4672,
-                                       sp->values_dev + main_rows, ssl ? ssl + (size_t)main_rows * sslw : nullptr, sp->stream_tail, err);
+                                       sp->values_dev + main_rows, ssl ? ssl + (size_t)main_rows * sslw : nullptr,
+                                       bad ? bad + main_rows : nullptr, sp->stream_tail, err);
             M0_HIP(sp->hip, hipEventRecord(sp->ev_tail, sp->stream_tail));
             M0_HIP(sp->hip, hipStreamWaitEvent(sp->stream, sp->ev_tail, 0));
         }
@@ -461,13 +465,13 @@
         const size_t b = (size_t)sp->d.net_row_base;
         m0_net_lock(sp->nethandle_b);
         int rc = sp->net_b->forward(nullptr, sp->d.x0 + b * 64 * 32, sp->rows2[1], sp->logits_dev + b * 4672,
-                                    sp->values_dev + b, nullptr, sp->stream, err);
+                                    sp->values_dev + b, nullptr, sp->row_bad_dev ? sp->row_bad_dev + b : nullptr, sp->stream, err);
         m0_net_unlock(sp->nethandle_b);
         if (rc != M0_OK) { sp->hip.check(sp->net_b->hip()); m0_set_error(err); return rc; }
         rows += sp->rows2[1];
     }
     gate.release();
-    return finish_step(sp, rows, t0);
-}
-
-}
+    return finish_step(sp, rows, t0, true);
+}
+
+}
diff --git a/matrix0_amd/csrc/selfplay_engine.h b/matrix0_amd/csrc/selfplay_engine.h
--- a/matrix0_amd/csrc/selfplay_engine.h
+++ b/matrix0_amd/csrc/selfplay_engine.h
@@ -114,6 +114,7 @@
     std::vector<RootResult> hres;
     float* logits_dev = nullptr;
     float* values_dev = nullptr;
+    uint8_t* row_bad_dev = nullptr;
     float* ssl_dev = nullptr;
     m0::Pos* ssl_pos_dev = nullptr;
     float* ssl_out_dev = nullptr;
@@ -178,7 +179,7 @@
 int run_select(m0_selfplay* sp, int* rows_out);
 int refill(m0_selfplay* sp);
 int one_step(m0_selfplay* sp);
-int finish_step(m0_selfplay* sp, int rows, double t0);
+int finish_step(m0_selfplay* sp, int rows, double t0, bool net_flags);
 
 m0_selfplay* engine_create(m0_net* nh, m0_net* nh_b, const m0_selfplay_cfg* cfg, EngineKind kind);
 int ext_select_impl(m0_selfplay* sp, int* rows_a, int* rows_b, float* planes_a, float* planes_b, int max_rows);
diff --git a/matrix0_amd/csrc/tree.h b/matrix0_amd/csrc/tree.h
--- a/matrix0_amd/csrc/tree.h
+++ b/matrix0_amd/csrc/tree.h
@@ -31,6 +31,7 @@
     int max_children;
     double min_child_prior;
     int eval_cache;
+    int tree_dpp;
 };
 
 #define M0_EC_MAXLEGAL 64
@@ -143,6 +144,7 @@
     _Float16* x0;
     const float* logits;
     const float* values;
+    const uint8_t* row_bad;
     int G;
     int L;
     const m0::TbSet* tb_set;
diff --git a/matrix0_amd/csrc/tree_device.h b/matrix0_amd/csrc/tree_device.h
--- a/matrix0_amd/csrc/tree_device.h
+++ b/matrix0_amd/csrc/tree_device.h
@@ -2,6 +2,7 @@
 #include <hip/hip_runtime.h>
 #include <math.h>
 #include "tree.h"
+#include "argmax_rule.h"
 
 using namespace m0;
 
@@ -65,6 +66,29 @@
 __device__ __forceinline__ double wave_sum_d(double v) {
     for (int o = 32; o > 0; o >>= 1) v += __shfl_xor(v, o);
     return v;
+}
+
+template <int CTRL, int ROW_MASK>
+__device__ __forceinline__ void argmax_dpp_step(double& best, int& bi) {
+    const int oi = __builtin_amdgcn_update_dpp(-1, bi, CTRL, ROW_MASK, 0xF, false);
+    const int lo = __builtin_amdgcn_update_dpp(0, __double2loint(best), CTRL, ROW_MASK, 0xF, false);
+    const int hi = __builtin_amdgcn_update_dpp(0, __double2hiint(best), CTRL, ROW_MASK, 0xF, false);
+    argmax_combine(best, bi, __hiloint2double(hi, lo), oi);
+}
+__device__ __forceinline__ void wave_argmax_first(double& best, int& bi) {
+    argmax_dpp_step<0xB1, 0xF>(best, bi);
+    argmax_dpp_step<0x4E, 0xF>(best, bi);
+    argmax_dpp_step<0x141, 0xF>(best, bi);
+    argmax_dpp_step<0x140, 0xF>(best, bi);
+    argmax_dpp_step<0x142, 0xA>(best, bi);
+    argmax_dpp_step<0x143, 0xC>(best, bi);
+    bi = __builtin_amdgcn_readlane(bi, 63);
+    best = __hiloint2double(__builtin_amdgcn_readlane(__double2hiint(best), 63), __builtin_amdgcn_readlane(__double2loint(best), 63));
+}
+__device__ __forceinline__ int wave_read_i(int v, int src) { return __builtin_amdgcn_readlane(v, __builtin_amdgcn_readfirstlane(src)); }
+__device__ __forceinline__ double wave_read_d(double v, int src) {
+    const int s = __builtin_amdgcn_readfirstlane(src);
+    return __hiloint2double(__builtin_amdgcn_readlane(__double2hiint(v), s), __builtin_amdgcn_readlane(__double2loint(v), s));
 }
 
 constexpr int CPL = M0_MAX_CHILDREN / 64;
diff --git a/matrix0_amd/csrc/tree_expand.hip b/matrix0_amd/csrc/tree_expand.hip
--- a/matrix0_amd/csrc/tree_expand.hip
+++ b/matrix0_amd/csrc/tree_expand.hip
@@ -20,9 +20,14 @@
     const float* row;
     const float* legal;
     float* store;
+    const uint8_t* bad;
 };
-__device__ __forceinline__ LeafLogits logits_of_row(const float* row, float* store) { return LeafLogits{row, nullptr, store}; }
-__device__ __forceinline__ LeafLogits logits_of_cache(const float* payload) { return LeafLogits{nullptr, payload + EC_LOGITS, nullptr}; }
+__device__ __forceinline__ LeafLogits logits_of_row(const float* row, float* store, const uint8_t* bad) {
+    return LeafLogits{row, nullptr, store, bad};
+}
+__device__ __forceinline__ LeafLogits logits_of_cache(const float* payload) {
+    return LeafLogits{nullptr, payload + EC_LOGITS, nullptr, nullptr};
+}
 
 static __device__ float np_sum_f32_dev(const float* a, int n) {
     auto block = [&](const float* b, int m) -> float {
@@ -212,7 +217,7 @@
     const int lane = E.lane;
     if (n <= 0) return true;
     bool bad = false;
-    if (!src.legal) bad = row_nonfinite(src.row, lane);
+    if (!src.legal) bad = src.bad ? *src.bad != 0 : row_nonfinite(src.row, lane);
     bad = __any(bad);
     if (lane == 0) E.X->bad = bad ? 1 : 0;
     float pr[CPL];
@@ -250,7 +255,8 @@
         cw = ec_payload(d.ec, ce);
         ec_invalidate(d.ec, ce, lane);
     }
-    const bool ok = expand_node(E, c, leaf, pos, moves, smp.nlegal, logits_of_row(lg, cw), kind == SK_ROOT_INIT,
+    const bool ok = expand_node(E, c, leaf, pos, moves, smp.nlegal, logits_of_row(lg, cw, d.row_bad ? d.row_bad + smp.row : nullptr),
+                                kind == SK_ROOT_INIT,
                                 !(kind == SK_ROOT_INIT && gd->root_fresh), q0);
     if (c.eval_cache && kind == SK_EVAL && lane == 0 && A.nch[leaf] < 0) A.cbase[leaf] = -1;
     const int sig = cw ? legal_sig(moves, smp.nlegal, lane) : 0;
diff --git a/matrix0_amd/csrc/tree_select.hip b/matrix0_amd/csrc/tree_select.hip
--- a/matrix0_amd/csrc/tree_select.hip
+++ b/matrix0_amd/csrc/tree_select.hip
@@ -220,22 +220,30 @@
                 sc += (u01(seedj, ctrj + (uint64_t)i) - 0.5) * jit;
                 if (sc > best) { best = sc; bi = i; b_nch = c_nch; b_cb = c_cb; b_n = cn; b_q = cq; b_mv = m; b_vl = cvl; }
             }
-            for (int off = 32; off > 0; off >>= 1) {
-                const double ob = __shfl_xor(best, off);
-                const int oi = __shfl_xor(bi, off);
-                if (oi >= 0 && (bi < 0 || ob > best || (ob == best && oi < bi))) { best = ob; bi = oi; }
-            }
+            if (c.tree_dpp) wave_argmax_first(best, bi);
+            else
+                for (int off = 32; off > 0; off >>= 1) {
+                    const double ob = __shfl_xor(best, off);
+                    const int oi = __shfl_xor(bi, off);
+                    argmax_combine(best, bi, ob, oi);
+                }
             ctrj += (uint64_t)nc;
             if (bi < 0) bi = 0;
             const int child = cb + bi;
             const int wl = bi & 63;
-            nc = __shfl(b_nch, wl); cb = __shfl(b_cb, wl); nn = __shfl(b_n, wl); nq = __shfl(b_q, wl);
-            const Move m = (Move)__shfl((int)b_mv, wl);
+            Move m;
+            int vlw;
+            if (c.tree_dpp) {
+                nc = wave_read_i(b_nch, wl); cb = wave_read_i(b_cb, wl); nn = wave_read_i(b_n, wl); nq = wave_read_d(b_q, wl);
+                m = (Move)wave_read_i((int)b_mv, wl); vlw = wave_read_i(b_vl, wl);
+            } else {
+                nc = __shfl(b_nch, wl); cb = __shfl(b_cb, wl); nn = __shfl(b_n, wl); nq = __shfl(b_q, wl);
+                m = (Move)__shfl((int)b_mv, wl); vlw = __shfl(b_vl, wl);
+            }
             const uint64_t k = tkey(pos);
             const bool irr = irreversible(pos, m);
             if (lane == 0) { pkey[depth] = k; pirr[depth] = irr ? 1 : 0; }
             make_move(pos, m);
-            const int vlw = __shfl(b_vl, wl);
             if (lane == 0 && c.virtual_loss_active) { A.vl[child] = vlw + 1; if (child < ncached) TC->vl[child] = vlw + 1; }
             prev_from = mv_from(m); prev_to = mv_to(m);
             node = child; ++depth;
```

Result: no change. 1.173 (median of 3 runs) (+0.3%).
